# deeplearning-wisc/MCM

Hardware: AMD Instinct MI355X
Metric: images/sec MCM-scored (CLIP-B/16, 1000 prompts) (higher is better)
Workload: dtype fp16; 1 GPU; MCM scoring, CLIP-ViT-B/16 (12L vision tower, random-init weights), K=1000 prompts pre-encoded, batch 512/GPU, fp32 NCHW pixels resident in HBM -> [B] scores; batch_per_gpu=512, prompts=1000, parallelism=image-sharded x1

## Files before the change

include/mcm.h:

```cpp
#ifndef MCM_H_
#define MCM_H_

#include <stdint.h>

#ifdef __cplusplus
extern "C" {
#endif

#define MCM_ABI_VERSION 5

#define MCM_OK 0
#define MCM_EINVAL (-1)
#define MCM_ENOMEM (-2)
#define MCM_EHIP (-3)
#define MCM_ENOWEIGHT (-4)
#define MCM_ENAME (-5)
#define MCM_ESHAPE (-6)
#define MCM_ERANGE (-7)

#define MCM_PREC_BF16 0
#define MCM_PREC_F32 1
#define MCM_PREC_F16 2

#define MCM_DT_F32 0
#define MCM_DT_F16 1
#define MCM_DT_BF16 2

#define MCM_WEIGHTS_AUTO 0
#define MCM_WEIGHTS_SINGLE 1
#define MCM_WEIGHTS_SPLIT 2

#define MCM_ACT_QUICK_GELU 0
#define MCM_ACT_GELU 1

#define MCM_SCORE_MCM 0
#define MCM_SCORE_MAX_LOGIT 1
#define MCM_SCORE_ENERGY 2
#define MCM_SCORE_ENTROPY 3
#define MCM_SCORE_VAR 4

typedef struct mcm_handle mcm_handle;

typedef struct mcm_config {
  int32_t abi_version;
  int32_t device;
  int32_t precision;
  int32_t image_size;
  int32_t patch_size;
  int32_t v_width;
  int32_t v_heads;
  int32_t v_layers;
  int32_t v_mlp;
  int32_t vocab_size;
  int32_t max_positions;
  int32_t t_width;
  int32_t t_heads;
  int32_t t_layers;
  int32_t t_mlp;
  int32_t proj_dim;
  float ln_eps;
  int32_t max_batch;
  int32_t max_prompt_tokens;
  int32_t weight_operands;
  int32_t x2_max_batch;
  int32_t v_hidden_act;
  int32_t t_hidden_act;
} mcm_config;

int mcm_abi_version(void);

int mcm_create(const mcm_config* cfg, mcm_handle** out);
void mcm_destroy(mcm_handle* h);
const char* mcm_last_error(const mcm_handle* h);

int mcm_set_weight(mcm_handle* h, const char* hf_name, const void* host_ptr, int32_t dtype,
                   const int64_t* shape, int32_t ndim);
int mcm_finalize_weights(mcm_handle* h);
int mcm_weights_operand_exact(mcm_handle* h, uint64_t* inexact_host, int32_t* split_host);

int mcm_encode_text(mcm_handle* h, const int32_t* ids_host, int32_t K, int32_t S,
                    float* out_dev, void* stream);

int mcm_encode_image(mcm_handle* h, const float* pixels_dev, int32_t B, float* out_dev,
                     void* stream);

#define MCM_PIXELS_F32_NCHW 0
#define MCM_PIXELS_U8_NHWC 1
int mcm_encode_image_ex(mcm_handle* h, const void* pixels_dev, int32_t pixel_format, int32_t B,
                        int32_t normalize, float* out_dev, void* stream);
int mcm_encode_text_ex(mcm_handle* h, const int32_t* ids_host, int32_t K, int32_t S, int32_t normalize,
                       float* out_dev, void* stream);

int mcm_score_features(mcm_handle* h, const float* img_feat_dev, int32_t B,
                       const float* text_feat_dev, int32_t K, float T, int32_t kind,
                       float* scores_dev, void* stream);

int mcm_score(mcm_handle* h, const float* pixels_dev, int32_t B, const float* text_feat_dev,
              int32_t K, float T, int32_t kind, float* scores_dev, void* stream);

#define MCM_TOPK_MAX 8
int mcm_score_features_topk(mcm_handle* h, const float* img_feat_dev, int32_t B, const float* text_feat_dev,
                            int32_t K, float T, int32_t kind, int32_t topk, float* scores_dev,
                            int32_t* idx_dev , float* prob_dev , void* stream);
int mcm_score_topk(mcm_handle* h, const void* pixels_dev, int32_t pixel_format, int32_t x2, int32_t B,
                   const float* text_feat_dev, int32_t K, float T, int32_t kind, int32_t topk, float* scores_dev,
                   int32_t* idx_dev, float* prob_dev, void* stream);

int mcm_encode_image_u8(mcm_handle* h, const uint8_t* pixels_dev, int32_t B, float* out_dev,
                        void* stream);
int mcm_score_u8(mcm_handle* h, const uint8_t* pixels_dev, int32_t B, const float* text_feat_dev,
                 int32_t K, float T, int32_t kind, float* scores_dev, void* stream);

int mcm_x2_max_batch(const mcm_handle* h);
int mcm_encode_image_x2(mcm_handle* h, const void* pixels_dev, int32_t pixel_format, int32_t B, int32_t normalize,
                        float* out_dev, void* stream);
int mcm_score_x2(mcm_handle* h, const void* pixels_dev, int32_t pixel_format, int32_t B, const float* text_feat_dev,
                 int32_t K, float T, int32_t kind, float* scores_dev, void* stream);

int mcm_resize_crop_u8(mcm_handle* h, const uint8_t* const* src_dev_ptrs, const int32_t* heights,
                       const int32_t* widths, int32_t B, uint8_t* dst_dev, void* stream);

int mcm_pack_u8(const uint8_t* const* srcs, const int64_t* sizes, const int64_t* offsets, int32_t n, uint8_t* dst,
                int64_t dst_bytes, int32_t threads);

typedef struct mcm_jpeg_image {
  int32_t status;
  int32_t width, height, ncomp;
  int32_t hs[3], vs[3];
  int32_t wb[3], hb[3];
  int64_t coef_off[3];
} mcm_jpeg_image;
int mcm_jpeg_entropy_decode(const char* const* paths, int32_t n, void* dst, int64_t dst_bytes, mcm_jpeg_image* meta,
                            uint16_t* quant, int32_t threads, int64_t* bytes_used);

int mcm_jpeg_reconstruct(mcm_handle* h, const void* coef_dev, const mcm_jpeg_image* meta, const uint16_t* quant, int32_t n,
                         uint8_t* rgb_dev, const int64_t* rgb_offsets, void* stream);

int mcm_reduce_bank(mcm_handle* h, const float* feats_dev, int32_t K, int32_t T, float* bank_dev,
                    void* stream);

int mcm_measures(mcm_handle* h, const float* pos_dev, int64_t n_pos, const float* neg_dev,
                 int64_t n_neg, int32_t negate, double recall_level, double* out_host, void* stream);

int mcm_score_histogram(mcm_handle* h, const float* scores_dev, int64_t n, const float* edges_dev,
                        int32_t n_bins, int64_t* counts_dev, void* stream);

int mcm_encode_image_raw(mcm_handle* h, const float* pixels_dev, int32_t B, float* out_dev, void* stream);
int mcm_maha_prepare(mcm_handle* h, const float* means_dev, const float* prec_dev, int32_t C,
                     double* w_dev, double* k_dev, void* stream);
int mcm_maha_score_features(mcm_handle* h, const float* feats_dev, int32_t B, const float* prec_dev,
                            const double* w_dev, const double* k_dev, int32_t C, float* scores_dev,
                            void* stream);
int mcm_maha_fit_accumulate(mcm_handle* h, const float* feats_dev , int32_t B,
                            const float* shift_dev , double* gram_dev, double* sum_dev,
                            void* stream);

#define MCM_KNN_MAX_K 1024
#define MCM_KNN_MAX_SPLITS 32
int mcm_knn_workspace_bytes(const mcm_handle* h, int32_t B, int64_t N, int32_t k, int32_t splits, int64_t* bytes_out);
int mcm_knn_score_features(mcm_handle* h, const float* feats_dev , int32_t B,
                           const float* bank_dev , int64_t N, int32_t k, int32_t splits,
                           void* work_dev, int64_t work_bytes, float* scores_dev ,
                           float* topv_dev , void* stream);

#define MCM_NEG_MAX_GROUPS 1024
int mcm_neglabel_workspace_bytes(const mcm_handle* h, int32_t B, int32_t K, int32_t G, int32_t gs, int32_t splits,
                                 int64_t* bytes_out);
int mcm_neglabel_score_features(mcm_handle* h, const float* feats_dev , int32_t B,
                                const float* bank_dev , int32_t K, int32_t G, int32_t gs,
                                float T, int32_t splits, void* work_dev, int64_t work_bytes,
                                float* scores_dev , float* group_dev , void* stream);

int mcm_local_workspace_bytes(const mcm_handle* h, int32_t B, int32_t R, int32_t K, int64_t* bytes_out);
int mcm_local_score_features(mcm_handle* h, const float* local_dev , int32_t B, int32_t R,
                             const float* text_dev , int32_t K, float T, void* work_dev,
                             int64_t work_bytes, float* local_scores_dev ,
                             float* patch_dev , void* stream);
int mcm_encode_image_local(mcm_handle* h, const void* pixels_dev, int32_t pixel_format, int32_t B,
                           float* global_dev ,
                           float* local_dev , void* stream);
int mcm_score_glmcm(mcm_handle* h, const void* pixels_dev, int32_t pixel_format, int32_t B, const float* text_dev ,
                    int32_t K, float T, float lambda, float* scores_dev ,
                    float* global_scores_dev , float* local_scores_dev ,
                    float* patch_dev , void* stream);

typedef struct mcm_tokenizer mcm_tokenizer;
int mcm_tokenizer_create(const char* vocab_json_path, const char* merges_txt_path, mcm_tokenizer** out);
void mcm_tokenizer_destroy(mcm_tokenizer* t);
const char* mcm_tokenizer_last_error(const mcm_tokenizer* t);
int32_t mcm_tokenizer_vocab_size(const mcm_tokenizer* t);
int mcm_tokenizer_encode(mcm_tokenizer* t, const char* const* texts, int32_t n, int32_t capacity,
                         int32_t* ids_out, int32_t* mask_out, int32_t* seq_len_out);

#define MCM_KC_PATCHIFY 0
#define MCM_KC_GEMM 1
#define MCM_KC_LAYERNORM 2
#define MCM_KC_ATTENTION 3
#define MCM_KC_POOL_PROJECT 4
#define MCM_KC_SCORE 5
#define MCM_KC_EMBED 6
#define MCM_KC_GEMM_QKV 7
#define MCM_KC_GEMM_OUTPROJ 8
#define MCM_KC_GEMM_FC1 9
#define MCM_KC_GEMM_FC2 10
#define MCM_KC_COUNT 11
int mcm_profile_enable(mcm_handle* h, int32_t on);
int mcm_profile_read(mcm_handle* h, double* ms_out, int64_t* launches_out, double* flops_out);


int mcm_op_linear(mcm_handle* h, int32_t prec, const void* x_dev, const void* w_dev,
                  const float* bias_dev, void* y_dev, float* resid_dev, int32_t M, int32_t N,
                  int32_t K, int32_t epi, void* stream);
#define MCM_LINEAR_SPLIT_W 1
#define MCM_LINEAR_SPLIT_X 2
#define MCM_LINEAR_SPLIT_OUT 4
#define MCM_LINEAR_ACT_GELU 8
int mcm_op_linear_ex(mcm_handle* h, int32_t prec, const void* x_dev, const void* w_dev,
                     const float* bias_dev, void* y_dev, float* resid_dev, int32_t M, int32_t N,
                     int32_t K, int32_t epi, int32_t flags, void* stream);
int mcm_op_split_weight(mcm_handle* h, int32_t prec, const float* w_dev, int32_t N, int32_t K,
                        void* out_dev, void* stream);
int mcm_op_layernorm(mcm_handle* h, int32_t prec, const float* x_dev, const float* gamma_dev,
                     const float* beta_dev, void* y_dev, int32_t M, int32_t D, float eps,
                     int32_t out_f32, void* stream);
int mcm_op_layernorm_split(mcm_handle* h, const float* x_dev, const float* gamma_dev, const float* beta_dev,
                           void* y_dev, int32_t M, int32_t D, float eps, void* stream);
int mcm_op_attention_split(mcm_handle* h, const void* qkv_dev, void* out_dev, int32_t nseq, int32_t seq_len,
                           int32_t heads, void* stream);
int mcm_op_attention(mcm_handle* h, int32_t prec, const void* qkv_dev, void* out_dev,
                     int32_t nseq, int32_t seq_len, int32_t heads, int32_t causal,
                     void* stream);

int mcm_saturation_check(mcm_handle* h, int32_t on);
int mcm_saturation_count(mcm_handle* h, int32_t reset, uint64_t* count_host, void* stream);

int mcm_kernel_faults(const mcm_handle* h);

#ifdef MCM_HARNESS
int mcm_debug_gemm_variant(int32_t variant);
int mcm_debug_op_act(mcm_handle* h, int32_t act, const float* x_dev, float* y_dev, int64_t n, void* stream);
int mcm_debug_attention_variant(int32_t variant);
int mcm_debug_attn_spin_budget(int64_t polls);
int mcm_debug_clear_faults(mcm_handle* h);
int mcm_debug_op_attention(mcm_handle* h, int32_t prec, const void* qkv_dev, void* out_dev, int32_t nseq, int32_t seq_len,
                           int32_t heads, int32_t causal, int32_t qrows, int32_t reverse, void* stream);
int mcm_debug_op_attention_split(mcm_handle* h, const void* qkv_dev, void* out_dev, int32_t nseq, int32_t seq_len,
                                 int32_t heads, int32_t qrows, int32_t reverse, void* stream);
int mcm_debug_op_attention_hd(mcm_handle* h, int32_t prec, const void* qkv_dev, void* out_dev, int32_t nseq, int32_t seq_len,
                              int32_t heads, int32_t head_dim, int32_t causal, int32_t qrows, int32_t reverse, void* stream);
int mcm_debug_op_attention_split_hd(mcm_handle* h, const void* qkv_dev, void* out_dev, int32_t nseq, int32_t seq_len,
                                    int32_t heads, int32_t head_dim, int32_t qrows, int32_t reverse, void* stream);
int mcm_debug_vision_front(mcm_handle* h, const void* pixels_dev, int32_t pixel_format, int32_t x2, int32_t B, int32_t stage,
                           int32_t poison, float* resid_out_dev, void* ln_out_dev, void* stream);
int mcm_debug_op_pool_project(mcm_handle* h, const float* x_dev, int64_t x_rows, const int32_t* row_idx_host, int32_t row_stride,
                              int32_t n, int32_t D, const float* gamma_dev, const float* beta_dev, float eps,
                              const float* proj_dev, int32_t P, float* out_dev, int32_t normalize, void* stream);
int mcm_debug_op_text_embed(mcm_handle* h, const int32_t* ids_host, int32_t vocab, const float* tok_dev, const float* pos_dev,
                            float* x_dev, int32_t K, int32_t S, int32_t D, void* stream);
int mcm_debug_gemm_dbg(int32_t bits);
int mcm_debug_qkv_chunks(int32_t n);
int mcm_debug_nsplit(int32_t n);
int mcm_debug_gemm_group_n(int32_t gn);
int mcm_debug_patch_fold(int32_t on);
int mcm_debug_resize_fused_only(int32_t on);
int mcm_debug_persistent_grid(int32_t n);
int mcm_debug_ln_fold(int32_t on);
int mcm_debug_qkv_head_major(int32_t on);
int mcm_debug_ln_tail(int32_t on);
int mcm_debug_ln_cluster(int32_t on);
int mcm_debug_ln_cluster_spin(int32_t polls);
int mcm_debug_ln_row(int32_t on);
int mcm_debug_ln_cluster_deferred(mcm_handle* h, uint64_t* count_host);
int mcm_debug_ln_tail_timeouts(mcm_handle* h, uint64_t* count_host);
#endif

#ifdef __cplusplus
}
#endif
#endif
```

mcm_amd/csrc/common.hpp:

```cpp
#pragma once
#include <hip/hip_runtime.h>
#include <stdint.h>

#include "../../include/mcm.h"

struct PerDeviceFlag {
  bool done[64] = {};
  static int dev() { int d = 0; return hipGetDevice(&d) == hipSuccess && d >= 0 && d < 64 ? d : -1; }
  bool get() const { const int d = dev(); return d >= 0 && done[d]; }
  void set() { const int d = dev(); if (d >= 0) done[d] = true; }
};

inline int device_cu_count() {
  static int cus[64] = {};
  int dev = 0;
  if (hipGetDevice(&dev) != hipSuccess || dev < 0) return 0;
  if (dev < 64 && cus[dev] > 0) return cus[dev];
  int n = 0;
  if (hipDeviceGetAttribute(&n, hipDeviceAttributeMultiprocessorCount, dev) != hipSuccess) return 0;
  if (dev < 64) cus[dev] = n;
  return n;
}

typedef __attribute__((ext_vector_type(8))) __bf16 bf16x8_t;
typedef __attribute__((ext_vector_type(8))) _Float16 f16x8_t;
typedef __attribute__((ext_vector_type(4))) float f32x4_t;
typedef __attribute__((address_space(1))) const void* gptr_t;
typedef __attribute__((address_space(3))) void* lptr_t;

__device__ __forceinline__ uint16_t f2bf(float f) {
  uint32_t u = __builtin_bit_cast(uint32_t, f);
  if ((u & 0x7fffffffu) > 0x7f800000u) return (uint16_t)((u >> 16) | 0x40u);
  u += 0x7fffu + ((u >> 16) & 1u);
  return (uint16_t)(u >> 16);
}
__device__ __forceinline__ float bf2f(uint16_t h) {
  return __builtin_bit_cast(float, (uint32_t)h << 16);
}
__device__ __forceinline__ uint32_t pack_bf2(float lo, float hi) {
  typedef __bf16 bf2_t __attribute__((ext_vector_type(2)));
  typedef float f2_t __attribute__((ext_vector_type(2)));
  const f2_t v = {lo, hi};
  return __builtin_bit_cast(uint32_t, __builtin_convertvector(v, bf2_t));
}

__device__ __forceinline__ void glds16(const void* gsrc, uint32_t lds_base) {
  uint32_t keep;
  asm volatile(
      "s_mov_b32 %0, m0\n\ts_mov_b32 m0, %2\n\ts_nop 0\n\tglobal_load_lds_dwordx4 %1, off\n\t"
      "s_mov_b32 m0, %0"
      : "=&s"(keep)
      : "v"(gsrc), "s"(lds_base)
      : "memory");
}
__device__ __forceinline__ uint32_t lds_addr(const void* p) {
  return (uint32_t)(uintptr_t)(__attribute__((address_space(3))) const void*)p;
}

__device__ __forceinline__ uint32_t pack_h2(float lo, float hi) {
  typedef _Float16 h2_t __attribute__((ext_vector_type(2)));
  typedef float f2_t __attribute__((ext_vector_type(2)));
  const f2_t v = {lo, hi};
  return __builtin_bit_cast(uint32_t, __builtin_convertvector(v, h2_t));
}
template <int PREC>
__device__ __forceinline__ void enter_precision_mode() {
  if constexpr (PREC == MCM_PREC_F16) asm volatile("s_setreg_imm32_b32 hwreg(HW_REG_MODE, 23, 1), 1");
}

template <int PREC>
__device__ __forceinline__ void sat_track(float& amax, float a, float b) {
#ifndef MCM_NO_SAT_TRACK
  if constexpr (PREC == MCM_PREC_F16) amax = fmaxf(fmaxf(__builtin_fabsf(a), __builtin_fabsf(b)), amax);
#endif
}
template <int PREC>
__device__ __forceinline__ void sat_report(float amax, unsigned int* counter) {
  if constexpr (PREC == MCM_PREC_F16) {
    if (counter != nullptr && __builtin_amdgcn_ballot_w64(amax >= 65520.0f) != 0) {
      if ((threadIdx.x & 63) == 0) {
        const unsigned int one = 1u;
        asm volatile("global_atomic_add %0, %1, off" ::"v"(counter), "v"(one) : "memory");
      }
    }
  }
}

template <int PREC>
__device__ __forceinline__ uint32_t pack2(float lo, float hi) {
  if constexpr (PREC == MCM_PREC_F16) return pack_h2(lo, hi);
  else return pack_bf2(lo, hi);
}
template <int PREC>
__device__ __forceinline__ f32x4_t mfma16(uint4 a, uint4 b, f32x4_t c) {
  if constexpr (PREC == MCM_PREC_F16)
    return __builtin_amdgcn_mfma_f32_16x16x32_f16(__builtin_bit_cast(f16x8_t, a),
                                                  __builtin_bit_cast(f16x8_t, b), c, 0, 0, 0);
  else
    return __builtin_amdgcn_mfma_f32_16x16x32_bf16(__builtin_bit_cast(bf16x8_t, a),
                                                   __builtin_bit_cast(bf16x8_t, b), c, 0, 0, 0);
}

__device__ __forceinline__ float quick_gelu(float x) { return x / (1.0f + __expf(-1.702f * x)); }
__device__ __forceinline__ float quick_gelu_fast(float x) {
  return x * __builtin_amdgcn_rcpf(1.0f + __builtin_amdgcn_exp2f(-1.702f * 1.4426950408889634f * x));
}
__device__ __forceinline__ float gelu_erf(float x) {
#pragma clang fp contract(off)
  const float ax = __builtin_fabsf(x);
  const float t = __builtin_amdgcn_rcpf(__builtin_fmaf(ax, 0.2757716477f, 1.0f));
  const float e = __builtin_amdgcn_exp2f((ax * ax) * -0.7213475204f);
  float h = -0.11376846582f;
  h = __builtin_fmaf(h, t, 0.44333177805f);
  h = __builtin_fmaf(h, t, -0.31769949198f);
  h = __builtin_fmaf(h, t, 0.32477918267f);
  h = __builtin_fmaf(h, t, 0.045694414526f);
  h = __builtin_fmaf(h, t, 0.11766257882f);
  h = (h * t) * e;
  return x * (x >= 0.0f ? 1.0f - h : h);
}

__device__ __forceinline__ float wave_sum(float v) {
#pragma unroll
  for (int o = 32; o > 0; o >>= 1) v += __shfl_xor(v, o, 64);
  return v;
}
__device__ __forceinline__ float wave_max(float v) {
#pragma unroll
  for (int o = 32; o > 0; o >>= 1) v = fmaxf(v, __shfl_xor(v, o, 64));
  return v;
}

template <int CTRL>
__device__ __forceinline__ float dpp_move(float x) {
  return __builtin_bit_cast(float, __builtin_amdgcn_update_dpp(0, __builtin_bit_cast(int, x), CTRL, 0xf, 0xf, true));
}
__device__ __forceinline__ float row16_sum(float v) {
#pragma clang fp contract(off)
  v = v + dpp_move<0xB1>(v);
  v = v + dpp_move<0x4E>(v);
  v = v + dpp_move<0x141>(v);
  v = v + dpp_move<0x140>(v);
  return v;
}
__device__ __forceinline__ void slot_moments(const f32x4_t& v, float& sum, float& m2) {
#pragma clang fp contract(off)
  sum = row16_sum((v[0] + v[1]) + (v[2] + v[3]));
  const float mean = sum * (1.0f / 64.0f);
  const float d0 = v[0] - mean, d1 = v[1] - mean, d2 = v[2] - mean, d3 = v[3] - mean;
  m2 = row16_sum((d0 * d0 + d1 * d1) + (d2 * d2 + d3 * d3));
}
__device__ __forceinline__ f32x4_t fold_scale(const f32x4_t& v, const f32x4_t& gamma) {
#pragma clang fp contract(off)
  return v * gamma;
}
__device__ __forceinline__ float fold_apply(float acc, float rstd, float mrstd, float c, float b) {
  return __builtin_fmaf(acc, rstd, __builtin_fmaf(-mrstd, c, b));
}

template <int PREC>
__device__ __forceinline__ void split2(float a, float b, uint32_t& hi, uint32_t& lo) {
  hi = pack2<PREC>(a, b);
  float ha, hb;
  if constexpr (PREC == MCM_PREC_F16) {
    typedef _Float16 h2_t __attribute__((ext_vector_type(2)));
    const h2_t h = __builtin_bit_cast(h2_t, hi);
    ha = (float)h[0];
    hb = (float)h[1];
  } else {
    ha = __builtin_bit_cast(float, hi << 16);
    hb = __builtin_bit_cast(float, hi & 0xffff0000u);
  }
  lo = pack2<PREC>(a - ha, b - hb);
}
__host__ __device__ constexpr size_t split_col(int n) { return (size_t)(n >> 6) * 128 + (n & 63); }

__host__ __device__ constexpr int prec_esize(int prec) { return prec == MCM_PREC_F32 ? 4 : 2; }


enum GemmEpi : int {
  EPI_STORE = 0,
  EPI_GELU = 1,
  EPI_RESID = 2,
  EPI_PATCH = 3,
  EPI_STORE_X2 = 4,
  EPI_GELU_X2 = 5,
  EPI_GELU_ERF = 6,
  EPI_GELU_ERF_X2 = 7,
};
__host__ __device__ constexpr bool epi_x2(int e) { return e == EPI_STORE_X2 || e == EPI_GELU_X2 || e == EPI_GELU_ERF_X2; }
__host__ __device__ constexpr bool epi_erf(int e) { return e == EPI_GELU_ERF || e == EPI_GELU_ERF_X2; }
__host__ __device__ constexpr bool epi_gelu(int e) { return e == EPI_GELU || e == EPI_GELU_X2 || epi_erf(e); }
__host__ __device__ constexpr bool epi_plain16(int e) { return e == EPI_STORE || e == EPI_GELU || e == EPI_GELU_ERF; }
__host__ __device__ constexpr bool epi_store16(int e) { return epi_plain16(e) || epi_x2(e); }

struct GemmArgs {
  const void* x;
  const void* w;
  const float* bias;
  void* out;
  float* resid;
  const float* pos;
  int M, N, K;
  int ldx;
  int ldo;
  int np;
  const float* px;
  int img, patch;
  int gn;
  int rev;
  int dbg;
  unsigned int* sat;
  int ksplit;
  int xsplit;
  void* fold_z;
  const float* fold_g;
  float2* fold_part;
  const float2* fold_rs;
  const float* fold_c;
  int hm;
  const float* ln_g;
  const float* ln_b;
  void* ln_y;
  float ln_eps;
  unsigned int* ln_state;
  int ln_rs, ln_cap8;
  int lnc;
  int lnc_spin;
  int wblk;
};
#ifdef MCM_HARNESS
#define MCM_HM(hm) (hm)
#else
#define MCM_HM(hm) 0
#endif
__device__ __forceinline__ size_t out16_off(const GemmArgs& a, int m, int n) {
  return MCM_HM(a.hm) ? ((size_t)(n >> 6) * a.hm + m) * 64 + (n & 63) : (size_t)m * a.ldo + n;
}
hipError_t launch_gemm(int prec, int epi, const GemmArgs& a, hipStream_t s);
int gemm_fold_kind(int epi, int M, int N);
bool gemm_patch_takes_pixels(int prec, int M, int N, int kpad, int patch, int image);
bool gemm_ln_tail_ok(int prec, int M, int N);
int gemm_persistent_grid();
#ifdef MCM_HARNESS
void gemm_set_persistent_grid(int n);
#endif
hipError_t launch_fold_prep(int prec, const void* w, const float* gamma, const float* beta, const float* bias,
                            float* c, float* bfold, int N, int K, hipStream_t s);
hipError_t launch_fold_rows(int prec, const float* x, const float* gamma, void* z, float2* part, int M, int D,
                            hipStream_t s, unsigned int* sat = nullptr);
hipError_t launch_fold_stats(const float2* part, int slots, int M, int D, float eps, float2* rs, hipStream_t s);
#ifdef MCM_HARNESS
hipError_t launch_lnc_cleanup(int prec, const float* x, const float* g, const float* b, void* y, const float2* part, int M, int D,
                              float eps, unsigned int* ln_state, int ln_rs, int ln_cap8, hipStream_t s, unsigned int* sat);
hipError_t launch_gemm_row64_ln(int prec, const GemmArgs& a, hipStream_t s, int stages);
hipError_t launch_row64_block_w(const void* w, void* blocked, int N, int K, hipStream_t s);
void gemm_set_group_n(int gn);
void gemm_set_dbg(int d);
void gemm_set_variant(int v);
void attention_set_variant(int v);
void attention_set_spin_budget(unsigned int polls);
#endif

hipError_t launch_layernorm(int prec, const float* x, const float* g, const float* b, void* y,
                            int M, int D, float eps, bool out_f32, hipStream_t s,
                            size_t x_stride = 0, size_t y_stride = 0, bool reverse = false,
                            unsigned int* sat = nullptr, bool split = false);

hipError_t launch_layernorm_pre(int prec, float* x, const float* g0, const float* b0, const float* g1,
                                const float* b1, void* y, int M, int D, float eps, hipStream_t s,
                                bool reverse = false, unsigned int* sat = nullptr, const float* cls = nullptr,
                                const float* pos0 = nullptr, int ntok = 0, bool split = false);

hipError_t launch_attention(int prec, const void* qkv, void* out, int nseq, int L, int heads, int head_dim,
                            bool causal, int qrows, hipStream_t s, bool reverse = false, int hm = 0, bool split = false,
                            unsigned int* fault = nullptr);

hipError_t launch_patchify(int prec, const float* pixels, void* patches, int B, int image,
                           int patch, int kpad, hipStream_t s, bool split = false);
hipError_t launch_patchify_u8(int prec, const uint8_t* pixels, void* patches, int B, int image,
                              int patch, int kpad, const float* mean, const float* stdv,
                              hipStream_t s, bool split = false);
hipError_t launch_bank_reduce(const float* feats, int K, int T, int P, float* bank, hipStream_t s);
hipError_t launch_text_embed(const int32_t* ids, const float* tok, const float* pos, float* x,
                             int K, int S, int D, hipStream_t s);
hipError_t launch_cvt_weight(int prec, const float* src, void* dst, int rows, int cols,
                             int cols_pad, hipStream_t s);
hipError_t launch_cvt_weight_split(int prec, const float* src, void* dst, int rows, int cols,
                                   int cols_pad, hipStream_t s);
hipError_t launch_count_inexact(int prec, const float* src, size_t n, unsigned long long* count, hipStream_t s);

hipError_t launch_pool_project(const float* x, const int32_t* row_idx, int row_stride, int n,
                               int D, const float* g, const float* b, float eps,
                               const float* proj, int P, float* out, hipStream_t s,
                               bool normalize = true);
hipError_t launch_maha_prepare(const float* means, const float* prec, int C, int P, double* w, double* c,
                               hipStream_t s);
hipError_t launch_maha_score(const float* feats, int B, const float* prec, const double* w, const double* c,
                             int C, int P, float* scores, hipStream_t s);
hipError_t launch_maha_fit(const float* feats, int B, int P, const float* shift, double* gram, double* sum,
                           hipStream_t s);

hipError_t launch_knn(const float* feats, int B, const float* bank, int64_t N, int P, int k, int S, float* work,
                      float* scores, float* topv, hipStream_t s);

int64_t neglabel_work_bytes(int B, int G, int S);
hipError_t launch_neglabel(const float* feats, int B, const float* bank, int K, int G, int gs, int P, float T, int S,
                           void* work, float* scores, float* group, hipStream_t s);

int64_t local_work_bytes(int B, int R);
hipError_t launch_local_score(const float* rows, int B, int R, const float* bank, int K, int P, float T, void* work,
                              float* scores, float* patch, hipStream_t s);
hipError_t launch_local_compact(const float* y, float* out, int B, int ntok, int P, hipStream_t s);
hipError_t launch_local_combine(const float* g, const float* l, float lambda, float* out, int B, hipStream_t s);

hipError_t launch_score(const float* img, int B, const float* text, int K, int P, float T,
                        int kind, float* scores, hipStream_t s);
bool score_shape_ok(int K, int P);
hipError_t launch_score_topk(const float* img, int B, const float* text, int K, int P, float T, int kind,
                             int topk, float* scores, int* idx, float* prob, hipStream_t s);

size_t measures_workspace_bytes(long n);
hipError_t launch_measures(const float* pos, long n_pos, const float* neg, long n_neg, int negate,
                           double level, void* workspace, double** out_dev, hipStream_t s);

hipError_t launch_histogram(const float* x, long n, const float* edges, int nb, unsigned long long* counts,
                            hipStream_t s);

struct PrepImage {
  const uint8_t* src;
  int32_t H, W;
  int32_t nh, nw;
  int32_t top, left;
};
struct JpegImageDev {
  int32_t width, height, ncomp;
  int32_t H, V;
  int32_t wb[3], hb[3];
  int64_t coef_off[3];
  int64_t plane_off[3];
  int64_t rgb_off;
};
hipError_t launch_jpeg_reconstruct(const JpegImageDev* meta_dev, const uint16_t* quant_dev, const void* coef_dev,
                                   uint8_t* planes_dev, uint8_t* rgb_dev, int n, int max_blocks, int max_pixels, hipStream_t s);
int prep_max_taps();
size_t prep_coef_bytes(int max_batch, int S);
hipError_t launch_resize_crop(const PrepImage* meta_dev, int32_t* coef_dev, int B, int S, uint8_t* dst, hipStream_t s,
                              bool fused_only = false);
```

mcm_amd/csrc/embed.hip:

```cpp
#include "common.hpp"

namespace {

template <int OUT, bool X2 = false>
__global__ __launch_bounds__(256) void patchify_kernel(const float* __restrict__ px, void* out,
                                                       int B, int S, int P, int kpad) {
  const int g = S / P, np = g * g, kreal = 3 * P * P;
  const size_t total = (size_t)B * np * kpad;
  for (size_t i = (size_t)blockIdx.x * 256 + threadIdx.x; i < total;
       i += (size_t)gridDim.x * 256) {
    const int k = (int)(i % kpad);
    const size_t m = i / kpad;
    float v = 0.f;
    if (k < kreal) {
      const int b = (int)(m / np), p = (int)(m % np);
      const int gy = p / g, gx = p % g;
      const int c = k / (P * P), rem = k % (P * P), py = rem / P, pxx = rem % P;
      v = px[(((size_t)b * 3 + c) * S + gy * P + py) * S + gx * P + pxx];
    }
    if constexpr (X2) {
      const _Float16 hi = (_Float16)v;
      _Float16* dst = (_Float16*)out + m * 2 * kpad + split_col(k);
      dst[0] = hi;
      dst[64] = (_Float16)(v - (float)hi);
    } else
    if constexpr (OUT == MCM_PREC_BF16) ((uint16_t*)out)[i] = f2bf(v);
    else if constexpr (OUT == MCM_PREC_F16) ((_Float16*)out)[i] = (_Float16)v;
    else ((float*)out)[i] = v;
  }
}

template <int OUT>
__global__ __launch_bounds__(256) void patchify8_kernel(const float* __restrict__ px, void* out,
                                                        int B, int S, int P, int kpad) {
  const int g = S / P, np = g * g, k8 = kpad / 8, p8 = P / 8;
  const size_t total = (size_t)B * np * k8;
  for (size_t i = (size_t)blockIdx.x * 256 + threadIdx.x; i < total;
       i += (size_t)gridDim.x * 256) {
    const int kq = (int)(i % k8);
    const size_t m = i / k8;
    const int b = (int)(m / np), p = (int)(m % np);
    const int gy = p / g, gx = p - gy * g;
    const int rowi = kq / p8, xq = kq - rowi * p8;
    const int c = rowi / P, py = rowi - c * P;
    const float* src = px + (((size_t)b * 3 + c) * S + gy * P + py) * S + gx * P + xq * 8;
    const float4 a = *(const float4*)src, d = *(const float4*)(src + 4);
    if constexpr (OUT != MCM_PREC_F32) {
      *(uint4*)((uint16_t*)out + i * 8) =
          make_uint4(pack2<OUT>(a.x, a.y), pack2<OUT>(a.z, a.w), pack2<OUT>(d.x, d.y), pack2<OUT>(d.z, d.w));
    } else {
      *(float4*)((float*)out + i * 8) = a;
      *(float4*)((float*)out + i * 8 + 4) = d;
    }
  }
}

template <int OUT, bool X2 = false>
__global__ __launch_bounds__(256) void patchify_u8_kernel(const uint8_t* __restrict__ px, void* out,
                                                          int B, int S, int P, int kpad, float m0,
                                                          float m1, float m2, float s0, float s1,
                                                          float s2) {
  const int g = S / P, np = g * g;
  const size_t total = (size_t)B * S * S;
  const float mean[3] = {m0, m1, m2}, stdv[3] = {s0, s1, s2};
  for (size_t i = (size_t)blockIdx.x * 256 + threadIdx.x; i < total; i += (size_t)gridDim.x * 256) {
    const int x = (int)(i % S), y = (int)((i / S) % S), b = (int)(i / ((size_t)S * S));
    const int gy = y / P, py = y - gy * P, gx = x / P, pxx = x - gx * P;
    const size_t row = ((size_t)b * np + gy * g + gx) * kpad;
#pragma unroll
    for (int c = 0; c < 3; ++c) {
      const float v = ((float)px[i * 3 + c] / 255.0f - mean[c]) / stdv[c];
      const size_t o = row + (size_t)(c * P + py) * P + pxx;
      if constexpr (X2) {
        const _Float16 hi = (_Float16)v;
        _Float16* dst = (_Float16*)out + 2 * row + split_col((c * P + py) * P + pxx);
        dst[0] = hi;
        dst[64] = (_Float16)(v - (float)hi);
      } else
      if constexpr (OUT == MCM_PREC_BF16) ((uint16_t*)out)[o] = f2bf(v);
      else if constexpr (OUT == MCM_PREC_F16) ((_Float16*)out)[o] = (_Float16)v;
      else ((float*)out)[o] = v;
    }
  }
}

__global__ __launch_bounds__(256) void bank_reduce_kernel(const float* __restrict__ feats, int K,
                                                          int T, int P, float* __restrict__ bank) {
  const int k = blockIdx.x * 4 + (threadIdx.x >> 6), lane = threadIdx.x & 63;
  if (k >= K) return;
  float sq = 0.f;
  for (int d = lane; d < P; d += 64) {
    float a = 0.f;
    for (int t = 0; t < T; ++t) a += feats[((size_t)k * T + t) * P + d];
    a /= (float)T;
    bank[(size_t)k * P + d] = a;
    sq += a * a;
  }
  const float rn = 1.0f / sqrtf(wave_sum(sq));
  for (int d = lane; d < P; d += 64) bank[(size_t)k * P + d] *= rn;
}

__global__ __launch_bounds__(256) void text_embed_kernel(const int32_t* __restrict__ ids,
                                                         const float* __restrict__ tok,
                                                         const float* __restrict__ pos, float* x,
                                                         int K, int S, int D) {
  const int row = blockIdx.x;
  const int s = row % S;
  const int id = ids[row];
  for (int d = threadIdx.x * 4; d < D; d += 1024) {
    const float4 a = *(const float4*)(tok + (size_t)id * D + d);
    const float4 p = *(const float4*)(pos + (size_t)s * D + d);
    *(float4*)(x + (size_t)row * D + d) = make_float4(a.x + p.x, a.y + p.y, a.z + p.z, a.w + p.w);
  }
}

template <int OUT>
__global__ __launch_bounds__(256) void cvt_weight_kernel(const float* __restrict__ src, void* dst,
                                                         int rows, int cols, int cols_pad) {
  const size_t total = (size_t)rows * cols_pad;
  for (size_t i = (size_t)blockIdx.x * 256 + threadIdx.x; i < total;
       i += (size_t)gridDim.x * 256) {
    const int c = (int)(i % cols_pad);
    const size_t r = i / cols_pad;
    const float v = c < cols ? src[r * cols + c] : 0.f;
    if constexpr (OUT == MCM_PREC_BF16) ((uint16_t*)dst)[i] = f2bf(v);
    else if constexpr (OUT == MCM_PREC_F16) ((_Float16*)dst)[i] = (_Float16)v;
    else ((float*)dst)[i] = v;
  }
}

template <int OUT>
__global__ __launch_bounds__(256) void cvt_weight_split_kernel(const float* __restrict__ src, void* dst,
                                                               int rows, int cols, int cols_pad) {
  const size_t total = (size_t)rows * cols_pad;
  for (size_t i = (size_t)blockIdx.x * 256 + threadIdx.x; i < total;
       i += (size_t)gridDim.x * 256) {
    const int c = (int)(i % cols_pad);
    const size_t r = i / cols_pad;
    const float v = c < cols ? src[r * cols + c] : 0.f;
    const size_t o = r * 2 * cols_pad + (size_t)(c >> 6) * 128 + (c & 63);
    if constexpr (OUT == MCM_PREC_BF16) {
      const uint16_t hi = f2bf(v);
      ((uint16_t*)dst)[o] = hi;
      ((uint16_t*)dst)[o + 64] = f2bf(v - bf2f(hi));
    } else {
      const float vc = fminf(fmaxf(v, -65504.0f), 65504.0f);
      const _Float16 hi = (_Float16)vc;
      ((_Float16*)dst)[o] = hi;
      ((_Float16*)dst)[o + 64] = (_Float16)fminf(fmaxf(v - (float)hi, -65504.0f), 65504.0f);
    }
  }
}

template <int OUT>
__global__ __launch_bounds__(256) void count_inexact_kernel(const float* __restrict__ src, size_t n,
                                                            unsigned long long* count) {
  unsigned int mine = 0;
  for (size_t i = (size_t)blockIdx.x * 256 + threadIdx.x; i < n; i += (size_t)gridDim.x * 256) {
    const float v = src[i];
    float back;
    if constexpr (OUT == MCM_PREC_BF16) back = bf2f(f2bf(v));
    else back = (float)(_Float16)v;
    mine += (back != v && v == v) ? 1u : 0u;
  }
#pragma unroll
  for (int o = 32; o > 0; o >>= 1) mine += __shfl_xor(mine, o, 64);
  if ((threadIdx.x & 63) == 0 && mine) atomicAdd(count, (unsigned long long)mine);
}

constexpr int NWP = 16;
constexpr int POOL_MAXD = 1280;
template <bool WIDE>
__global__ __launch_bounds__(NWP * 64) void pool_project_kernel(
    const float* __restrict__ x, const int32_t* __restrict__ row_idx, int row_stride, int D,
    const float* __restrict__ g, const float* __restrict__ b, float eps,
    const float* __restrict__ proj, int P, float* __restrict__ out, int normalize) {
  __shared__ float y[WIDE ? POOL_MAXD : 1024];
  __shared__ float o[1024];
  __shared__ float red[2 * NWP];
  const int n = blockIdx.x, tid = threadIdx.x, lane = tid & 63, wave = tid >> 6;
  const size_t row = row_idx ? (size_t)row_idx[n] : (size_t)n * row_stride;
  const float* xr = x + row * D;
  const int t2 = tid + NWP * 64;
  const float xv = tid < D ? xr[tid] : 0.f;
  float xw = 0.f;
  float s;
  if constexpr (WIDE) {
    if (t2 < D) xw = xr[t2];
    s = wave_sum(xv + xw);
  } else {
    s = wave_sum(xv);
  }
  if (lane == 0) red[wave] = s;
  __syncthreads();
  float tot = 0.f;
#pragma unroll
  for (int i = 0; i < NWP; ++i) tot += red[i];
  const float mean = tot / (float)D;
  const float c = tid < D ? xv - mean : 0.f;
  float cw = 0.f;
  float q;
  if constexpr (WIDE) {
    if (t2 < D) cw = xw - mean;
    q = wave_sum(fmaf(cw, cw, c * c));
  } else {
    q = wave_sum(c * c);
  }
  if (lane == 0) red[NWP + wave] = q;
  __syncthreads();
  tot = 0.f;
#pragma unroll
  for (int i = 0; i < NWP; ++i) tot += red[NWP + i];
  const float rstd = 1.0f / sqrtf(tot / (float)D + eps);
  if (tid < D) y[tid] = c * rstd * g[tid] + b[tid];
  if constexpr (WIDE) {
    if (t2 < D) y[t2] = cw * rstd * g[t2] + b[t2];
  }
  __syncthreads();
  float sq = 0.f;
  for (int p = wave; p < P; p += NWP) {
    const float* w = proj + (size_t)p * D;
    float a = 0.f;
    for (int d = lane * 4; d < D; d += 256) {
      const float4 wv = *(const float4*)(w + d);
      a = fmaf(wv.x, y[d], a);
      a = fmaf(wv.y, y[d + 1], a);
      a = fmaf(wv.z, y[d + 2], a);
      a = fmaf(wv.w, y[d + 3], a);
    }
    a = wave_sum(a);
    if (lane == 0) {
      o[p] = a;
      sq += a * a;
    }
  }
  __syncthreads();
  if (lane == 0) red[wave] = sq;
  __syncthreads();
  tot = 0.f;
#pragma unroll
  for (int i = 0; i < NWP; ++i) tot += red[i];
  const float rn = normalize ? 1.0f / sqrtf(tot) : 1.0f;
  for (int p = tid; p < P; p += NWP * 64) out[(size_t)n * P + p] = o[p] * rn;
}

inline int grid_for(size_t total) {
  size_t g = (total + 255) / 256;
  return (int)(g > 4096 ? 4096 : (g ? g : 1));
}

}

hipError_t launch_patchify(int prec, const float* pixels, void* patches, int B, int image,
                           int patch, int kpad, hipStream_t s, bool split) {
  const int g = image / patch;
  if (split) {
    if (prec != MCM_PREC_F16 || kpad % 64) return hipErrorInvalidValue;
    const size_t n = (size_t)B * g * g * kpad;
    hipLaunchKernelGGL((patchify_kernel<MCM_PREC_F16, true>), dim3(grid_for(n)), dim3(256), 0, s, pixels, patches, B, image, patch, kpad);
    return hipGetLastError();
  }
  const bool vec = patch % 8 == 0 && kpad == 3 * patch * patch && image % 4 == 0;
  const size_t total = (size_t)B * g * g * (vec ? kpad / 8 : kpad);
  const dim3 grid(grid_for(total)), block(256);
#define MCM_LAUNCH_BY_PREC(KERNEL, ...)                                                         \
  do {                                                                                           \
    if (prec == MCM_PREC_BF16) hipLaunchKernelGGL(KERNEL<MCM_PREC_BF16>, grid, block, 0, s, __VA_ARGS__); \
    else if (prec == MCM_PREC_F16) hipLaunchKernelGGL(KERNEL<MCM_PREC_F16>, grid, block, 0, s, __VA_ARGS__); \
    else hipLaunchKernelGGL(KERNEL<MCM_PREC_F32>, grid, block, 0, s, __VA_ARGS__);               \
  } while (0)
  if (vec) MCM_LAUNCH_BY_PREC(patchify8_kernel, pixels, patches, B, image, patch, kpad);
  else MCM_LAUNCH_BY_PREC(patchify_kernel, pixels, patches, B, image, patch, kpad);
  return hipGetLastError();
}

hipError_t launch_patchify_u8(int prec, const uint8_t* pixels, void* patches, int B, int image,
                              int patch, int kpad, const float* mean, const float* stdv,
                              hipStream_t s, bool split) {
  const size_t total = (size_t)B * image * image;
  const dim3 grid(grid_for(total)), block(256);
  if (split && (prec != MCM_PREC_F16 || kpad % 64)) return hipErrorInvalidValue;
  if (kpad != 3 * patch * patch) {
    hipError_t e = hipMemsetAsync(patches, 0, (size_t)B * (image / patch) * (image / patch) * kpad *
                                                   prec_esize(prec) * (split ? 2 : 1), s);
    if (e != hipSuccess) return e;
  }
  if (split) {
    hipLaunchKernelGGL((patchify_u8_kernel<MCM_PREC_F16, true>), grid, block, 0, s, pixels, patches, B, image, patch, kpad,
                       mean[0], mean[1], mean[2], stdv[0], stdv[1], stdv[2]);
    return hipGetLastError();
  }
  MCM_LAUNCH_BY_PREC(patchify_u8_kernel, pixels, patches, B, image, patch, kpad, mean[0], mean[1],
                     mean[2], stdv[0], stdv[1], stdv[2]);
  return hipGetLastError();
}

hipError_t launch_bank_reduce(const float* feats, int K, int T, int P, float* bank, hipStream_t s) {
  if (K <= 0 || T <= 0 || P <= 0) return hipErrorInvalidValue;
  hipLaunchKernelGGL(bank_reduce_kernel, dim3((K + 3) / 4), dim3(256), 0, s, feats, K, T, P, bank);
  return hipGetLastError();
}

hipError_t launch_text_embed(const int32_t* ids, const float* tok, const float* pos, float* x,
                             int K, int S, int D, hipStream_t s) {
  if (D % 4) return hipErrorInvalidValue;
  hipLaunchKernelGGL(text_embed_kernel, dim3(K * S), dim3(256), 0, s, ids, tok, pos, x, K, S, D);
  return hipGetLastError();
}

hipError_t launch_cvt_weight(int prec, const float* src, void* dst, int rows, int cols,
                             int cols_pad, hipStream_t s) {
  const size_t total = (size_t)rows * cols_pad;
  const dim3 grid(grid_for(total)), block(256);
  MCM_LAUNCH_BY_PREC(cvt_weight_kernel, src, dst, rows, cols, cols_pad);
  return hipGetLastError();
}

hipError_t launch_cvt_weight_split(int prec, const float* src, void* dst, int rows, int cols,
                                   int cols_pad, hipStream_t s) {
  if (prec == MCM_PREC_F32 || cols_pad % 64) return hipErrorInvalidValue;
  const size_t total = (size_t)rows * cols_pad;
  const dim3 grid(grid_for(total)), block(256);
  if (prec == MCM_PREC_BF16) hipLaunchKernelGGL(cvt_weight_split_kernel<MCM_PREC_BF16>, grid, block, 0, s, src, dst, rows, cols, cols_pad);
  else hipLaunchKernelGGL(cvt_weight_split_kernel<MCM_PREC_F16>, grid, block, 0, s, src, dst, rows, cols, cols_pad);
  return hipGetLastError();
}

hipError_t launch_count_inexact(int prec, const float* src, size_t n, unsigned long long* count, hipStream_t s) {
  if (prec == MCM_PREC_F32 || n == 0) return hipSuccess;
  const dim3 grid(grid_for(n)), block(256);
  if (prec == MCM_PREC_BF16) hipLaunchKernelGGL(count_inexact_kernel<MCM_PREC_BF16>, grid, block, 0, s, src, n, count);
  else hipLaunchKernelGGL(count_inexact_kernel<MCM_PREC_F16>, grid, block, 0, s, src, n, count);
  return hipGetLastError();
}

hipError_t launch_pool_project(const float* x, const int32_t* row_idx, int row_stride, int n,
                               int D, const float* g, const float* b, float eps,
                               const float* proj, int P, float* out, hipStream_t s, bool normalize) {
  if (n <= 0 || D > POOL_MAXD || D % 4 || P > 1024) return hipErrorInvalidValue;
  if (D > 1024 && D % 64) return hipErrorInvalidValue;
  if (D > 1024)
    hipLaunchKernelGGL(pool_project_kernel<true>, dim3(n), dim3(NWP * 64), 0, s, x, row_idx, row_stride, D, g, b,
                       eps, proj, P, out, normalize ? 1 : 0);
  else
    hipLaunchKernelGGL(pool_project_kernel<false>, dim3(n), dim3(NWP * 64), 0, s, x, row_idx, row_stride, D, g, b,
                       eps, proj, P, out, normalize ? 1 : 0);
  return hipGetLastError();
}
```

mcm_amd/csrc/gemm.hip:

```cpp
#include <type_traits>

#include "common.hpp"
#include "ln_row.hpp"

namespace {

constexpr int ROWB = 128;

__device__ __forceinline__ void kstep_off(const GemmArgs& a, int kt, size_t& kox, size_t& kow) {
  const int t = kt >> (a.ksplit + a.xsplit);
  kox = (size_t)((t << a.xsplit) | (kt & a.xsplit)) * ROWB;
  kow = (size_t)((t << a.ksplit) | ((kt >> a.xsplit) & a.ksplit)) * ROWB;
}
__device__ __forceinline__ int ksteps(const GemmArgs& a, int es) { return ((a.K * es) / ROWB) << a.xsplit; }

#if defined(MCM_HARNESS) || defined(MCM_LN_FOLD) || defined(MCM_LN_TAIL)
#define MCM_ARMS 1
#endif

__device__ __forceinline__ int frag_off(int fr, int g, int kk) {
  return (fr >> 1) * 256 + ((((fr & 1) << 3) | (((kk * 4 + g) ^ (fr >> 1)) & 7)) << 4);
}

template <int PREC, int MF>
// ... 179 lines not shown
                     pack2<PREC>(v[1][0], v[1][1]), pack2<PREC>(v[1][2], v[1][3]));
      *(uint4*)(w + (((g * 2 + 1) ^ sw) << 4)) =
          make_uint4(pack2<PREC>(v[2][0], v[2][1]), pack2<PREC>(v[2][2], v[2][3]),
                     pack2<PREC>(v[3][0], v[3][1]), pack2<PREC>(v[3][2], v[3][3]));
    };
    auto read_unit = [&](int u, uint4 (&r)[2]) {
#pragma unroll
      for (int t = 0; t < 2; ++t) {
        const int row = t * 8 + rrow;
        r[t] = *(const uint4*)(scratch + (u & 1) * 2048 + row * 128 + ((c8 ^ (row & 7)) << 4));
      }
    };
    const int ldo_e = MCM_HM(a.hm) ? 64 : a.ldo;
    const int lane_off = rrow * ldo_e + c8 * 8;
    const char* sp = (const char*)a.out + out16_off(a, mw, nw) * 2;
    const size_t sp_step = (size_t)ldo_e * 16;
    auto store_unit = [&](int u, const uint4 (&r)[2]) {
#pragma unroll
      for (int t = 0; t < 2; ++t) {
        if constexpr (INTERIOR) {
          store16_stream_s(sp, (uint32_t)lane_off * 2u, r[t]);
          sp += sp_step;
        } else {
          const int m = mw + u * 16 + t * 8 + rrow;
          if (m < a.M && n < a.N) store16_stream((uint16_t*)a.out + out16_off(a, m, n), r[t]);
        }
      }
    };
    write_unit(0);
#pragma unroll
    for (int u = 1; u < MF; ++u) {
      uint4 r[2];
      read_unit(u - 1, r);
      write_unit(u);
      store_unit(u - 1, r);
    }
    {
      uint4 r[2];
      read_unit(MF - 1, r);
      store_unit(MF - 1, r);
    }
  } else {
    const int rrow = lane >> 4, c16 = lane & 15;
    const int n = nw + c16 * 4;
    const bool ncol = n < a.N;
    f32x4_t rnext[4];
    auto row_ptr = [&](int c, int t, bool& ok) -> float* {
      const int m = mw + c * 16 + t * 4 + rrow;
      ok = ncol && m < a.M;
      if constexpr (EPI == EPI_PATCH) {
        const int mm = min(m, a.M - 1), b = mm / a.np, p = mm - b * a.np;
        return (float*)a.out + (size_t)(b * (a.np + 1) + 1 + p) * a.ldo + n;
      } else if constexpr (EPI == EPI_RESID) {
        return a.resid + (size_t)m * a.ldo + n;
      } else {
        return (float*)a.out + (size_t)m * a.ldo + n;
      }
    };
    auto prefetch = [&](int c) {
#pragma unroll
      for (int t = 0; t < 4; ++t) {
        bool ok;
        const float* ptr;
        if constexpr (EPI == EPI_PATCH) {
          const int m = min(mw + c * 16 + t * 4 + rrow, a.M - 1);
          const int p = m - (m / a.np) * a.np;
          ok = ncol;
          ptr = a.pos + (size_t)(1 + p) * a.N + n;
        } else {
          ptr = row_ptr(c, t, ok);
        }
        rnext[t] = ok ? *(const f32x4_t*)ptr : (f32x4_t){0.f, 0.f, 0.f, 0.f};
      }
    };
    constexpr bool ADD = (EPI == EPI_RESID || EPI == EPI_PATCH);
    if constexpr (ADD) prefetch(0);
#pragma unroll
    for (int c = 0; c < MF; ++c) {
      f32x4_t r[4];
      if constexpr (ADD) {
#pragma unroll
        for (int t = 0; t < 4; ++t) r[t] = rnext[t];
        if (c + 1 < MF) prefetch(c + 1);
      }
      const int sw = fr;
#pragma unroll
      for (int fj = 0; fj < 4; ++fj) {
        f32x4_t v = acc[fj][c] + bv[fj];
        if constexpr (epi_gelu(EPI)) {
#pragma unroll
          for (int t = 0; t < 4; ++t) v[t] = epi_erf(EPI) ? gelu_erf(v[t]) : quick_gelu(v[t]);
        }
        *(f32x4_t*)(scratch + fr * 256 + (((g * 4 + fj) ^ sw) << 4)) = v;
      }
#pragma unroll
      for (int t = 0; t < 4; ++t) {
        const int row = t * 4 + rrow;
        f32x4_t v = *(const f32x4_t*)(scratch + row * 256 + ((c16 ^ row) << 4));
        if constexpr (ADD) v += r[t];
        bool ok;
        float* dst = row_ptr(c, t, ok);
        if (ok) *(f32x4_t*)dst = v;
      }
    }
  }
}

__device__ __forceinline__ void load_bias(const GemmArgs& a, int n, f32x4_t (&bv)[4]) {
  const int nc = min(n, a.N - 16);
#pragma unroll
  for (int fj = 0; fj < 4; ++fj) {
    bv[fj] = a.bias ? *(const f32x4_t*)(a.bias + nc + fj * 4) : (f32x4_t){0.f, 0.f, 0.f, 0.f};
  }
#pragma unroll
  for (int fj = 0; fj < 4; ++fj) asm volatile("" : "+v"(bv[fj]));
}
__device__ __forceinline__ void load_bias_async(const GemmArgs& a, int n, f32x4_t (&bv)[4]) {
  const float* p = a.bias + min(n, a.N - 16);
#pragma unroll
  for (int fj = 0; fj < 4; ++fj)
    asm volatile("global_load_dwordx4 %0, %1, off" : "=v"(bv[fj]) : "v"(p + fj * 4) : "memory");
}

template <int MF>
__device__ __forceinline__ void zero_acc(f32x4_t (&acc)[4][MF]) {
#pragma unroll
  for (int i = 0; i < 4; ++i)
#pragma unroll
    for (int j = 0; j < MF; ++j) acc[i][j] = (f32x4_t){0.f, 0.f, 0.f, 0.f};
}

namespace tile {
constexpr int BM = 128, BN = 128;
constexpr int TILE_BYTES = BM * ROWB;
constexpr int STAGE_BYTES = 2 * TILE_BYTES;
constexpr int LDS_BYTES = 2 * STAGE_BYTES;
}

template <int PREC, int EPI>
__global__ __launch_bounds__(256, 2) void gemm_tile_kernel(const GemmArgs a) {
  using namespace tile;
  enter_precision_mode<PREC>();
  extern __shared__ __attribute__((aligned(16))) char smem[];
  constexpr int ES = prec_esize(PREC);
  const int lane = threadIdx.x & 63;
  const int wave = __builtin_amdgcn_readfirstlane(threadIdx.x >> 6);

  const int nbn = (a.N + BN - 1) / BN;
  const int nbm = (a.M + BM - 1) / BM;
  const int nwg = nbn * nbm;
  int lid;
  {
    const int bid = blockIdx.x, q = nwg >> 3, r = nwg & 7, xcd = bid & 7;
    lid = (xcd < r ? xcd * (q + 1) : r * (q + 1) + (xcd - r) * q) + (bid >> 3);
  }
  const int m0 = (lid / nbn) * BM;
  const int n0 = (lid % nbn) * BN;

  const char* gx[4];
  const char* gw[4];
#pragma unroll
  for (int i = 0; i < 4; ++i) {
    const int blk = i * 4 + wave;
    const int p = blk * 4 + (lane >> 4);
    const int s = lane & 15;
    const int row = 2 * p + (s >> 3);
    const int chunk = (s & 7) ^ (p & 7);
    const int mr = min(m0 + row, a.M - 1);
    const int nr = min(n0 + (row & 64) + perm_n(row & 63), a.N - 1);
    gx[i] = (const char*)a.x + ((size_t)mr * a.ldx) * ES + chunk * 16;
    gw[i] = (const char*)a.w + ((size_t)nr * a.K) * ES + chunk * 16;
  }
  const uint32_t lds0 = lds_addr(smem);
  auto stage = [&](int st, int kt) {
    const uint32_t base = lds0 + st * STAGE_BYTES;
    size_t kox, kow;
    kstep_off(a, kt, kox, kow);
#pragma unroll
    for (int i = 0; i < 4; ++i) {
      const int blk = i * 4 + wave;
      glds16(gx[i] + kox, __builtin_amdgcn_readfirstlane(base + blk * 1024));
      glds16(gw[i] + kow, __builtin_amdgcn_readfirstlane(base + TILE_BYTES + blk * 1024));
    }
  };

  const int wr = wave >> 1, wc = wave & 1;
  const int fr = lane & 15, g = lane >> 4;
  const int foff[2] = {frag_off(fr, g, 0), frag_off(fr, g, 1)};
  const int xbase = wr * 64 * ROWB;
  const int wbase = TILE_BYTES + wc * 64 * ROWB;

  f32x4_t acc[4][4];
  zero_acc(acc);
  const int nk = ksteps(a, ES);
  stage(0, 0);
  for (int kt = 0; kt < nk; ++kt) {
    asm volatile("s_waitcnt vmcnt(0)" ::: "memory");
    __syncthreads();
    if (kt + 1 < nk) stage((kt + 1) & 1, kt + 1);
    const char* sb = smem + (kt & 1) * STAGE_BYTES;
    wave_kstep<PREC, 4>(sb + xbase, sb + wbase, foff, acc);
  }
  f32x4_t bv[4];
  load_bias(a, n0 + wc * 64 + g * 16, bv);
  float amax = 0.f;
  wave_epilogue<PREC, EPI, 4>(a, acc, bv, m0 + wr * 64, n0 + wc * 64, fr, g, amax);
  sat_report<PREC>(amax, a.sat);
}

namespace tile64 {
constexpr int BM = 64, BN = 128;
constexpr int X_BYTES = BM * ROWB, W_BYTES = BN * ROWB;
constexpr int STAGE_BYTES = X_BYTES + W_BYTES;
constexpr int LDS_BYTES = 2 * STAGE_BYTES;
}

template <int PREC, int EPI>
__global__ __launch_bounds__(256, 2) void gemm_tile64_kernel(const GemmArgs a) {
  using namespace tile64;
  enter_precision_mode<PREC>();
  extern __shared__ __attribute__((aligned(16))) char smem[];
  constexpr int ES = prec_esize(PREC);
  const int lane = threadIdx.x & 63;
  const int wave = __builtin_amdgcn_readfirstlane(threadIdx.x >> 6);
  const int nbn = (a.N + BN - 1) / BN;
  const int nbm = (a.M + BM - 1) / BM;
  const int nwg = nbn * nbm;
  int lid;
  {
    const int bid = blockIdx.x, q = nwg >> 3, r = nwg & 7, xcd = bid & 7;
    lid = (xcd < r ? xcd * (q + 1) : r * (q + 1) + (xcd - r) * q) + (bid >> 3);
  }
  const int m0 = (lid / nbn) * BM;
  const int n0 = (lid % nbn) * BN;
  const char* gx[2];
  const char* gw[4];
#pragma unroll
  for (int i = 0; i < 4; ++i) {
    const int blk = i * 4 + wave;
    const int p = blk * 4 + (lane >> 4);
    const int sl = lane & 15;
    const int row = 2 * p + (sl >> 3);
    const int chunk = (sl & 7) ^ (p & 7);
    if (i < 2) gx[i] = (const char*)a.x + ((size_t)min(m0 + row, a.M - 1) * a.ldx) * ES + chunk * 16;
    const int nr = min(n0 + (row & 64) + perm_n(row & 63), a.N - 1);
    gw[i] = (const char*)a.w + ((size_t)nr * a.K) * ES + chunk * 16;
  }
  const uint32_t lds0 = lds_addr(smem);
  auto stage = [&](int st, int kt) {
    const uint32_t base = lds0 + st * STAGE_BYTES;
    size_t kox, kow;
    kstep_off(a, kt, kox, kow);
#pragma unroll
    for (int i = 0; i < 4; ++i) {
      const int blk = i * 4 + wave;
      if (i < 2) glds16(gx[i] + kox, __builtin_amdgcn_readfirstlane(base + blk * 1024));
      glds16(gw[i] + kow, __builtin_amdgcn_readfirstlane(base + X_BYTES + blk * 1024));
    }
  };
  const int wr = wave >> 1, wc = wave & 1;
  const int fr = lane & 15, g = lane >> 4;
  const int foff[2] = {frag_off(fr, g, 0), frag_off(fr, g, 1)};
  const int xbase = wr * 32 * ROWB;
  const int wbase = X_BYTES + wc * 64 * ROWB;
  f32x4_t acc[4][2];
  zero_acc(acc);
  const int nk = ksteps(a, ES);
  stage(0, 0);
  for (int kt = 0; kt < nk; ++kt) {
    asm volatile("s_waitcnt vmcnt(0)" ::: "memory");
    __syncthreads();
    if (kt + 1 < nk) stage((kt + 1) & 1, kt + 1);
    const char* sb = smem + (kt & 1) * STAGE_BYTES;
#pragma unroll
    for (int kk = 0; kk < 2; ++kk) {
      uint4 wf[4], xf[2];
#pragma unroll
      for (int f = 0; f < 4; ++f) wf[f] = *(const uint4*)(sb + wbase + f * 2048 + foff[kk]);
#pragma unroll
      for (int f = 0; f < 2; ++f) xf[f] = *(const uint4*)(sb + xbase + f * 2048 + foff[kk]);
#pragma unroll
      for (int fj = 0; fj < 4; ++fj)
#pragma unroll
        for (int fi = 0; fi < 2; ++fi) {
          if constexpr (PREC != MCM_PREC_F32) {
            acc[fj][fi] = mfma16<PREC>(wf[fj], xf[fi], acc[fj][fi]);
          } else {
            const f32x4_t wv = __builtin_bit_cast(f32x4_t, wf[fj]);
            const f32x4_t xv = __builtin_bit_cast(f32x4_t, xf[fi]);
#pragma unroll
            for (int t = 0; t < 4; ++t)
              acc[fj][fi] = __builtin_amdgcn_mfma_f32_16x16x4f32(wv[t], xv[t], acc[fj][fi], 0, 0, 0);
          }
        }
    }
  }
  f32x4_t bv[4];
  load_bias(a, n0 + wc * 64 + g * 16, bv);
  float amax = 0.f;
  wave_epilogue<PREC, EPI, 2>(a, acc, bv, m0 + wr * 32, n0 + wc * 64, fr, g, amax);
  sat_report<PREC>(amax, a.sat);
}

__device__ __forceinline__ void tile_of(int q, int nmt_x, int nbn, int gn, int& mtl, int& nt) {
  int start = 0, g0 = 0;
  for (;;) {
    const int gw = min(gn, nbn - g0), cnt = nmt_x * gw;
    if (q < start + cnt || g0 + gw >= nbn) {
      const int r = q - start;
      mtl = r / gw;
      nt = g0 + (r - mtl * gw);
      return;
    }
    start += cnt;
    g0 += gw;
  }
}

template <int N>
__device__ __forceinline__ void wait_vmcnt() {
  asm volatile("s_waitcnt vmcnt(%0)" ::"n"(N) : "memory");
}

namespace p256 {
constexpr int BM = 256, BN = 256;
constexpr int A_BYTES = BM * ROWB;
constexpr int W_BYTES = BN * ROWB;
constexpr int STAGE_BYTES = A_BYTES + W_BYTES;
constexpr int LDS_BYTES = 2 * STAGE_BYTES + 8 * 4096;
}

__device__ __forceinline__ void gload16(f32x4_t& dst, const void* sbase, uint32_t voff) {
  asm volatile("global_load_dwordx4 %0, %1, %2" : "=v"(dst) : "v"(voff), "s"(sbase) : "memory");
}
__device__ __forceinline__ void gstore16(const void* sbase, uint32_t voff, const f32x4_t& v) {
  asm volatile("global_store_dwordx4 %0, %1, %2\n\ts_nop 1" ::"v"(voff), "v"(v), "s"(sbase) : "memory");
}

template <int PREC, int EPI, bool COUNT_STORES, bool PXF = false>
__global__ __launch_bounds__(512, 2) void gemm_p256_kernel(const GemmArgs a) {
  static_assert(!PXF || EPI == EPI_PATCH, "pixel gathering: the patch embedding only");
  using namespace p256;
  enter_precision_mode<PREC>();
  extern __shared__ __attribute__((aligned(16))) char smem[];
  constexpr int ES = prec_esize(PREC);
  constexpr int STORES_PER_EPI = (PREC != MCM_PREC_F32 && epi_plain16(EPI)) ? 16 : 32;
  const int lane = threadIdx.x & 63;
  const int wave = __builtin_amdgcn_readfirstlane(threadIdx.x >> 6);

  const int nbn = (a.N + BN - 1) / BN;
  const int nbm = (a.M + BM - 1) / BM;
  const int G8 = gridDim.x >> 3;
  const int xcd = blockIdx.x & 7, jx = blockIdx.x >> 3;
  const int nmt_x = (nbm - xcd + 7) >> 3;
  const int ntl_x = nmt_x * nbn;
  const int ntl = jx < ntl_x ? (ntl_x - jx + G8 - 1) / G8 : 0;
  if (ntl == 0) return;
  const int nk = ksteps(a, ES);
  const int total = ntl * nk;

  const int r0 = wave * 8 + (lane >> 4) * 2 + ((lane & 15) >> 3);
  const int chunk = (lane & 7) ^ (((wave & 1) << 2) | (lane >> 4));
  const char* gx[4];
  const char* gw[4];
  int ji = 0, kti = 0;
  constexpr int EC = 16 / ES, KS = ROWB / ES;
  uint32_t pxoff[4] = {0u, 0u, 0u, 0u};
  f32x4_t xr[4][2];
  int xst = 0;
  const bool plain = a.gn >= nbn;
  const int dmt = G8 / nbn, dnt = G8 - dmt * nbn;
  struct Cursor { int mtl, nt; };
  auto cursor_init = [&](Cursor& c) { tile_of(jx, nmt_x, nbn, a.gn, c.mtl, c.nt); };
  auto cursor_next = [&](Cursor& c, int i) {
    if (plain) {
      c.mtl += dmt;
      c.nt += dnt;
      if (c.nt >= nbn) { c.nt -= nbn; ++c.mtl; }
    } else {
      tile_of(jx + i * G8, nmt_x, nbn, a.gn, c.mtl, c.nt);
    }
  };
  const size_t sx = (size_t)a.ldx * ES, sw = (size_t)a.K * ES;
  const char* xlane = (const char*)a.x + (size_t)r0 * sx + chunk * 16;
  const char* wlane = (const char*)a.w + (size_t)perm_n(r0) * sw + chunk * 16;
  auto mt_of = [&](int mtl) { return a.rev ? nmt_x - 1 - mtl : mtl; };
  Cursor ci;
  auto set_issue_tile = [&]() {
    const int m0 = (mt_of(ci.mtl) * 8 + xcd) * BM, n0 = ci.nt * BN;
    if (m0 + BM <= a.M && n0 + BN <= a.N) {
      const char* xb = xlane + (size_t)m0 * sx;
      const char* wb = wlane + (size_t)n0 * sw;
#pragma unroll
      for (int p = 0; p < 4; ++p) {
        if constexpr (!PXF) gx[p] = xb + (size_t)(p * 64) * sx;
        gw[p] = wb + (size_t)(p * 64) * sw;
      }
    } else {
#pragma unroll
      for (int p = 0; p < 4; ++p) {
        if constexpr (!PXF) gx[p] = (const char*)a.x + (size_t)min(m0 + p * 64 + r0, a.M - 1) * sx + chunk * 16;
        gw[p] = (const char*)a.w + (size_t)min(n0 + p * 64 + perm_n(r0), a.N - 1) * sw + chunk * 16;
      }
    }
    if constexpr (PXF) {
      {
        const int P = a.patch, S = a.img, gsz = S / P;
        const int e = chunk * EC, dpy = e / P, pxl = e - dpy * P;
#pragma unroll
        for (int p = 0; p < 4; ++p) {
          const int m = min(m0 + p * 64 + r0, a.M - 1);
          const int b = m / a.np, pp = m - b * a.np, gy = pp / gsz, gxx = pp - gy * gsz;
          pxoff[p] = (uint32_t)((((size_t)b * 3 * S + (size_t)gy * P + dpy) * S + (size_t)gxx * P + pxl) * 4);
        }
      }
    }
  };
  const uint32_t lds0 = lds_addr(smem);
  auto issue_px = [&](int st) {
    const int r = (kti >> a.ksplit) * (KS / a.patch), c = r / a.patch, py0 = r - c * a.patch;
    const char* kb = (const char*)a.px + ((size_t)c * a.img + py0) * a.img * 4;
#pragma unroll
    for (int p = 0; p < 4; ++p) {
      gload16(xr[p][0], kb, pxoff[p]);
      if constexpr (ES == 2) gload16(xr[p][1], kb, pxoff[p] + 16u);
    }
    xst = st;
  };
  auto issue = [&](int st) {
    const uint32_t base = lds0 + st * STAGE_BYTES;
    size_t ko, kox;
    kstep_off(a, kti, kox, ko);
    if constexpr (PXF) {
#pragma unroll
      for (int p = 0; p < 4; ++p)
        glds16(gw[p] + ko, __builtin_amdgcn_readfirstlane(base + A_BYTES + (p * 8 + wave) * 1024));
    } else {
#pragma unroll
      for (int p = 0; p < 4; ++p) {
        glds16(gx[p] + kox, __builtin_amdgcn_readfirstlane(base + (p * 8 + wave) * 1024));
        glds16(gw[p] + ko, __builtin_amdgcn_readfirstlane(base + A_BYTES + (p * 8 + wave) * 1024));
      }
    }
    if (++kti == nk) {
      kti = 0;
      if (++ji < ntl) {
        cursor_next(ci, ji);
        set_issue_tile();
      }
    }
  };

  const int wr = wave >> 2, wc = wave & 3;
  const bool late = wave >= 4;
  const int fr = lane & 15, g = lane >> 4;
  const int foff[2] = {frag_off(fr, g, 0), frag_off(fr, g, 1)};
  const int xbase = wr * 128 * ROWB;
  const int wbase = A_BYTES + wc * 64 * ROWB;

  f32x4_t acc[4][8];
  zero_acc<8>(acc);
  float amax = 0.f;
  f32x4_t bv[4];
#pragma unroll
  for (int fj = 0; fj < 4; ++fj) bv[fj] = (f32x4_t){0.f, 0.f, 0.f, 0.f};

  auto commit_x = [&]() {
    wait_vmcnt<0>();
#pragma unroll
    for (int p = 0; p < 4; ++p) {
      asm volatile("" : "+v"(xr[p][0]));
      if constexpr (ES == 2) asm volatile("" : "+v"(xr[p][1]));
    }
#pragma unroll
    for (int p = 0; p < 4; ++p) {
      char* dst = smem + xst * STAGE_BYTES + (p * 8 + wave) * 1024 + lane * 16;
      if constexpr (PREC != MCM_PREC_F32) {
        *(uint4*)dst = make_uint4(pack2<PREC>(xr[p][0][0], xr[p][0][1]), pack2<PREC>(xr[p][0][2], xr[p][0][3]),
                                  pack2<PREC>(xr[p][1][0], xr[p][1][1]), pack2<PREC>(xr[p][1][2], xr[p][1][3]));
      } else {
        *(f32x4_t*)dst = xr[p][0];
      }
    }
    asm volatile("s_waitcnt lgkmcnt(0)" ::: "memory");
  };

  cursor_init(ci);
  set_issue_tile();
  if constexpr (PXF) issue_px(0);
  issue(0);
  if constexpr (PXF) commit_x();
  int issued = 1;
  int jc = 0, ktc = 0;
  Cursor cc;
  cursor_init(cc);
  int cm0 = (mt_of(cc.mtl) * 8 + xcd) * BM, cn0 = cc.nt * BN;
  bool stores_pending = false;
  if (late) __builtin_amdgcn_s_setprio(1);
  for (int s = 0; s < total; ++s) {
    if (COUNT_STORES && stores_pending) wait_vmcnt<STORES_PER_EPI>();
    else wait_vmcnt<0>();
    stores_pending = false;
    __builtin_amdgcn_s_barrier();
    asm volatile("" ::: "memory");
    if constexpr (!PXF) {
      if (ktc == 0 && a.bias) load_bias_async(a, cn0 + wc * 64 + g * 16, bv);
    }
    const bool refill = issued < total;
    if constexpr (PXF) {
      if (refill) issue_px(issued & 1);
    }
    if (refill && !late) issue(issued & 1);
    const char* sb = smem + (s & 1) * STAGE_BYTES;
    wave_khalf<PREC, 8>(sb + xbase, sb + wbase, foff[0], acc);
    if (refill && late) issue(issued & 1);
    if (refill) ++issued;
    wave_khalf<PREC, 8>(sb + xbase, sb + wbase, foff[1], acc);
    if (++ktc == nk) {
      if constexpr (!PXF) {
        if (nk < 2) wait_vmcnt<0>();
#pragma unroll
        for (int fj = 0; fj < 4; ++fj) asm volatile("" : "+v"(bv[fj]));
      }
      wave_epilogue_lds<PREC, EPI, 8>(a, acc, bv, cm0 + wr * 128, cn0 + wc * 64, lane,
                                      smem + 2 * STAGE_BYTES + wave * 4096, amax);
      zero_acc<8>(acc);
      stores_pending = (cm0 + BM <= a.M && cn0 + BN <= a.N);
      ktc = 0;
      if (++jc < ntl) {
        cursor_next(cc, jc);
        cm0 = (mt_of(cc.mtl) * 8 + xcd) * BM;
        cn0 = cc.nt * BN;
      }
    }
    if constexpr (PXF) {
      if (refill) commit_x();
    }
  }
  sat_report<PREC>(amax, a.sat);
}

template <int N>
__device__ __forceinline__ void wait_vmcnt_pin(f32x4_t (&b)[4]) {
  asm volatile("s_waitcnt vmcnt(%4)" : "+v"(b[0]), "+v"(b[1]), "+v"(b[2]), "+v"(b[3]) : "n"(N) : "memory");
}
template <int EPI, int MF>
__device__ __forceinline__ void wave_epilogue_f32_interior(const GemmArgs& a, const f32x4_t (&acc)[4][MF],
                                                           const f32x4_t (&bv)[4], int mw, int nw, int lane,
                                                           char* scratch) {
  static_assert(EPI != EPI_PATCH, "patch rows are remapped: not an interior form");
  const int fr = lane & 15, g = lane >> 4;
  const int rrow = lane >> 4, c16 = lane & 15;
  const uint32_t voff = (uint32_t)(rrow * a.ldo + c16 * 4) * 4u;
  const char* base = (const char*)(EPI == EPI_RESID ? a.resid : (float*)a.out) + ((size_t)mw * a.ldo + nw) * 4;
  const size_t step = (size_t)a.ldo * 16;
  const char* lp = base;
  const char* sp = base;
  f32x4_t buf[2][4];
  f32x4_t bia = {0.f, 0.f, 0.f, 0.f};
  if constexpr (EPI == EPI_RESID) {
    if (a.bias) gload16(bia, a.bias + nw, (uint32_t)c16 * 16u);
#pragma unroll
    for (int t = 0; t < 4; ++t) {
      gload16(buf[0][t], lp, voff);
      lp += step;
    }
  }
#pragma unroll
  for (int c = 0; c < MF; ++c) {
    if constexpr (EPI == EPI_RESID) {
      if (c + 1 < MF) {
#pragma unroll
        for (int t = 0; t < 4; ++t) {
          gload16(buf[(c + 1) & 1][t], lp, voff);
          lp += step;
        }
      }
    }
#pragma unroll
    for (int fj = 0; fj < 4; ++fj) {
      f32x4_t v = acc[fj][c];
      if constexpr (EPI != EPI_RESID) v += bv[fj];
      if constexpr (epi_gelu(EPI)) {
#pragma unroll
        for (int t = 0; t < 4; ++t) v[t] = epi_erf(EPI) ? gelu_erf(v[t]) : quick_gelu(v[t]);
      }
      *(f32x4_t*)(scratch + fr * 256 + (((g * 4 + fj) ^ fr) << 4)) = v;
    }
    f32x4_t v[4];
#pragma unroll
    for (int t = 0; t < 4; ++t) {
      const int row = t * 4 + rrow;
      v[t] = *(const f32x4_t*)(scratch + row * 256 + ((c16 ^ row) << 4));
    }
    if constexpr (EPI == EPI_RESID) {
      if (c == 0 || c + 1 == MF) wait_vmcnt_pin<4>(buf[c & 1]);
      else wait_vmcnt_pin<8>(buf[c & 1]);
      if (c == 0) asm volatile("" : "+v"(bia));
#pragma unroll
      for (int t = 0; t < 4; ++t) v[t] = (v[t] + bia) + buf[c & 1][t];
    }
#pragma unroll
    for (int t = 0; t < 4; ++t) {
      gstore16(sp, voff, v[t]);
      sp += step;
    }
  }
}

__device__ __forceinline__ void glds16s(const void* sbase, uint32_t voff, uint32_t lds_base) {
  uint32_t keep;
  asm volatile(
      "s_mov_b32 %0, m0\n\ts_mov_b32 m0, %3\n\ts_nop 0\n\tglobal_load_lds_dwordx4 %1, %2\n\t"
      "s_mov_b32 m0, %0"
      : "=&s"(keep)
      : "v"(voff), "s"(sbase), "s"(lds_base)
      : "memory");
}

template <int PREC, int EPI>
__global__ __launch_bounds__(512, 2) void gemm_pp_kernel(const GemmArgs a) {
  using namespace p256;
  enter_precision_mode<PREC>();
  extern __shared__ __attribute__((aligned(16))) char smem[];
  constexpr int ES = prec_esize(PREC);
  const int lane = threadIdx.x & 63;
  const int wave = __builtin_amdgcn_readfirstlane(threadIdx.x >> 6);
  const int grp = wave >> 2, w4 = wave & 3;

  const int nbn = a.N / BN, nbm = a.M / BM;
  const int G8 = gridDim.x >> 3;
  const int xcd = blockIdx.x & 7, jx = blockIdx.x >> 3;
  const int nmt_x = (nbm - xcd + 7) >> 3;
  const int ntl_x = nmt_x * nbn;
  const int ntl = jx < ntl_x ? (ntl_x - jx + G8 - 1) / G8 : 0;
  if (ntl == 0) return;
  const int nk = ksteps(a, ES);
  const int total = ntl * nk;

  const int dmt = G8 / nbn, dnt = G8 - dmt * nbn;
  struct Cursor { int mtl, nt; };
  auto cursor_next = [&](Cursor& c) {
    c.mtl += dmt;
    c.nt += dnt;
    if (c.nt >= nbn) { c.nt -= nbn; ++c.mtl; }
  };
  auto mt_of = [&](int mtl) { return a.rev ? nmt_x - 1 - mtl : mtl; };
  const size_t sx = (size_t)a.ldx * ES, sw = (size_t)a.K * ES;

  struct LaneK { uint32_t voff_x, voff_w; int fo0, fo1; };
  auto lane_consts = [&]() {
    int l = lane;
    asm volatile("" : "+v"(l));
    const int rr = (l >> 4) * 2 + ((l & 15) >> 3);
    const int chunk = (l & 7) ^ (((w4 & 1) << 2) | (l >> 4));
    LaneK c;
    c.voff_x = (uint32_t)(rr * (uint32_t)sx + chunk * 16);
    c.voff_w = (uint32_t)(perm_n(w4 * 8 + rr) * (uint32_t)sw + chunk * 16);
    c.fo0 = frag_off(l & 15, l >> 4, 0);
    c.fo1 = frag_off(l & 15, l >> 4, 1);
    return c;
  };
  Cursor ci{jx / nbn, jx % nbn};
  int ji = 0, kti = 0;
  const char *tx, *tw;
  auto set_issue_tile = [&]() {
    const int m0 = (mt_of(ci.mtl) * 8 + xcd) * BM, n0 = ci.nt * BN;
    tx = (const char*)a.x + (size_t)(m0 + grp * 128 + w4 * 8) * sx;
    tw = (const char*)a.w + (size_t)n0 * sw;
  };
  const uint32_t lds0 = lds_addr(smem);
  auto piece = [&](const LaneK& lk, int st, int i) {
    const uint32_t base = lds0 + st * STAGE_BYTES + w4 * 1024;
    size_t ko, kox;
    kstep_off(a, kti, kox, ko);
    if (i < 4) {
      glds16s(tx + kox + (size_t)(i * 32) * sx, lk.voff_x, base + (grp * 16 + i * 4) * 1024);
    } else {
      const int q = i - 4;
      glds16s(tw + ko + (size_t)((q >> 1) * 64 + (q & 1) * 8) * sw, lk.voff_w, base + A_BYTES + q * 4096);
    }
  };
  constexpr int NP0 = 12;
  auto issue_done = [&]() {
    if (++kti == nk) {
      kti = 0;
      if (++ji < ntl) {
        cursor_next(ci);
        set_issue_tile();
      }
    }
  };

  const int wr = wave >> 2, wc = wave & 3;
  const int xbase = wr * 128 * ROWB;
  const int wbase = A_BYTES + wc * 64 * ROWB;
  typedef uint32_t u32x4_t __attribute__((ext_vector_type(4)));
  u32x4_t xf[8], wf[2][4];
  auto readf = [&](const LaneK& lk, int st, int i) {
    const char* sb = smem + st * STAGE_BYTES;
    if (i < 4) wf[0][i] = *(const u32x4_t*)(sb + wbase + i * 2048 + lk.fo0);
    else if (i < 12) xf[i - 4] = *(const u32x4_t*)(sb + xbase + (i - 4) * 2048 + lk.fo0);
    else wf[1][i - 12] = *(const u32x4_t*)(sb + wbase + (i - 12) * 2048 + lk.fo1);
  };
  auto pin_frags = [&]() {
    asm volatile("s_waitcnt lgkmcnt(0)" ::: "memory");
#pragma unroll
    for (int f = 0; f < 4; ++f) asm volatile("" : "+v"(wf[0][f]));
#pragma unroll
    for (int f = 0; f < 4; ++f) asm volatile("" : "+v"(wf[1][f]));
#pragma unroll
    for (int f = 0; f < 8; ++f) asm volatile("" : "+v"(xf[f]));
  };
  f32x4_t acc[4][8];
  zero_acc<8>(acc);
  float amax = 0.f;
  auto mfma_pair = [&](const u32x4_t& wv4, const u32x4_t& xv4, f32x4_t& c) {
    if constexpr (PREC != MCM_PREC_F32) {
      c = mfma16<PREC>(__builtin_bit_cast(uint4, wv4), __builtin_bit_cast(uint4, xv4), c);
    } else {
      const f32x4_t wv = __builtin_bit_cast(f32x4_t, wv4);
      const f32x4_t xv = __builtin_bit_cast(f32x4_t, xv4);
#pragma unroll
      for (int t = 0; t < 4; ++t) c = __builtin_amdgcn_mfma_f32_16x16x4f32(wv[t], xv[t], c, 0, 0, 0);
    }
  };
  auto compute = [&](int fo1, int st) {
    const char* sb = smem + st * STAGE_BYTES;
#pragma unroll
    for (int fi = 0; fi < 8; ++fi) {
#pragma unroll
      for (int fj = 0; fj < 4; ++fj) mfma_pair(wf[0][fj], xf[fi], acc[fj][fi]);
      xf[fi] = *(const u32x4_t*)(sb + xbase + fi * 2048 + fo1);
    }
#pragma unroll
    for (int fi = 0; fi < 8; ++fi)
#pragma unroll
      for (int fj = 0; fj < 4; ++fj) mfma_pair(wf[1][fj], xf[fi], acc[fj][fi]);
  };

  Cursor cc{jx / nbn, jx % nbn};
  int em0 = 0, en0 = 0;
  f32x4_t bv[4];
#pragma unroll
  for (int fj = 0; fj < 4; ++fj) bv[fj] = (f32x4_t){0.f, 0.f, 0.f, 0.f};
  auto epilogue = [&]() {
    int le = lane;
    asm volatile("" : "+v"(le));
    if constexpr (EPI != EPI_RESID) {
#pragma unroll
      for (int fj = 0; fj < 4; ++fj) asm volatile("" : "+v"(bv[fj]));
    }
    char* win = smem + 2 * STAGE_BYTES + wave * 4096;
    if constexpr (PREC != MCM_PREC_F32 && epi_store16(EPI))
      wave_epilogue_lds<PREC, EPI, 8, true>(a, acc, bv, em0 + wr * 128, en0 + wc * 64, le, win, amax);
    else
      wave_epilogue_f32_interior<EPI, 8>(a, acc, bv, em0 + wr * 128, en0 + wc * 64, le, win);
    zero_acc<8>(acc);
  };
  set_issue_tile();
  {
    const LaneK lk = lane_consts();
#pragma unroll
    for (int i = 0; i < NP0; ++i)
      if (i < 4 || !grp) piece(lk, 0, i);
  }
  issue_done();
  wait_vmcnt<0>();
  __builtin_amdgcn_s_barrier();
  asm volatile("" ::: "memory");
  if (grp) {
    __builtin_amdgcn_s_barrier();
    asm volatile("" ::: "memory");
  }
  int ktc = 0;
  bool pend = false;
  auto phase_barrier = [&]() {
    __builtin_amdgcn_sched_barrier(0);
    __builtin_amdgcn_s_barrier();
    asm volatile("" ::: "memory");
    __builtin_amdgcn_sched_barrier(0);
  };
  for (int s = 0; s < total; ++s) {
    const int sr = s & 1, si = sr ^ 1;
    const bool split = pend && !grp;
    int fo1;
    if (pend) {
      if (!grp) {
        const LaneK lk = lane_consts();
#pragma unroll
        for (int i = 0; i < NP0; ++i) piece(lk, si, i);
        issue_done();
        phase_barrier();
      }
      epilogue();
      if (!grp) {
        const LaneK lk = lane_consts();
        fo1 = lk.fo1;
#pragma unroll
        for (int i = 0; i < 16; ++i) readf(lk, sr, i);
      }
    }
    if (!split) {
      const LaneK lk = lane_consts();
      fo1 = lk.fo1;
      if (!grp) {
#pragma unroll
        for (int i = 0; i < NP0; ++i) {
          if (i < 8) {
            readf(lk, sr, 2 * i);
            readf(lk, sr, 2 * i + 1);
          }
          piece(lk, si, i);
        }
      } else {
#pragma unroll
        for (int i = 0; i < 4; ++i) {
#pragma unroll
          for (int j = 0; j < 4; ++j) readf(lk, sr, 4 * i + j);
          piece(lk, si, i);
        }
      }
      issue_done();
    }
    pin_frags();
    if (!split) phase_barrier();
    if (EPI == EPI_RESID) {
    } else if (ktc == nk - 1 && a.bias) {
      int le = lane;
      asm volatile("" : "+v"(le));
      load_bias_async(a, cc.nt * BN + wc * 64 + (le >> 4) * 16, bv);
    }
    __builtin_amdgcn_s_setprio(1);
    compute(fo1, sr);
    __builtin_amdgcn_s_setprio(0);
    wait_vmcnt<0>();
    phase_barrier();
    pend = false;
    if (++ktc == nk) {
      ktc = 0;
      pend = true;
      em0 = (mt_of(cc.mtl) * 8 + xcd) * BM;
      en0 = cc.nt * BN;
      cursor_next(cc);
    }
  }
  if (!grp) {
    __builtin_amdgcn_s_barrier();
    asm volatile("" ::: "memory");
  }
  if (pend) epilogue();
  if constexpr (epi_store16(EPI)) sat_report<PREC>(amax, a.sat);
}

#ifdef MCM_ARMS
int persistent_grid();
#include "gemm_arms.hpp"
#endif


#ifdef MCM_HARNESS
int g_variant = -1;
int variant() { return g_variant; }
#else
constexpr int variant() { return -1; }
#endif

#ifdef MCM_HARNESS
int g_grid_override = 0;
#endif
int persistent_grid() {
#ifdef MCM_HARNESS
  if (g_grid_override > 0) return g_grid_override;
#endif
  return device_cu_count() / 8 * 8;
}

template <int PREC, int EPI>
hipError_t launch_tile(const GemmArgs& a, hipStream_t s) {
  static PerDeviceFlag attr_set;
  if (!attr_set.get()) {
    hipError_t e = hipFuncSetAttribute((const void*)gemm_tile_kernel<PREC, EPI>,
                                       hipFuncAttributeMaxDynamicSharedMemorySize, tile::LDS_BYTES);
    if (e != hipSuccess) return e;
    attr_set.set();
  }
  const int nbn = (a.N + tile::BN - 1) / tile::BN, nbm = (a.M + tile::BM - 1) / tile::BM;
  hipLaunchKernelGGL((gemm_tile_kernel<PREC, EPI>), dim3(nbn * nbm), dim3(256), tile::LDS_BYTES, s, a);
  return hipGetLastError();
}

template <int PREC, int EPI>
hipError_t launch_tile64(const GemmArgs& a, hipStream_t s) {
  static PerDeviceFlag attr_set;
  if (!attr_set.get()) {
    hipError_t e = hipFuncSetAttribute((const void*)gemm_tile64_kernel<PREC, EPI>,
                                       hipFuncAttributeMaxDynamicSharedMemorySize, tile64::LDS_BYTES);
    if (e != hipSuccess) return e;
    attr_set.set();
  }
  const int nbn = (a.N + tile64::BN - 1) / tile64::BN, nbm = (a.M + tile64::BM - 1) / tile64::BM;
  hipLaunchKernelGGL((gemm_tile64_kernel<PREC, EPI>), dim3(nbn * nbm), dim3(256), tile64::LDS_BYTES, s, a);
  return hipGetLastError();
}

template <int PREC, int EPI, bool CS, bool PXF = false>
hipError_t launch_p256(const GemmArgs& a, hipStream_t s) {
  static PerDeviceFlag attr_set;
  if (!attr_set.get()) {
    hipError_t e = hipFuncSetAttribute((const void*)gemm_p256_kernel<PREC, EPI, CS, PXF>,
                                       hipFuncAttributeMaxDynamicSharedMemorySize, p256::LDS_BYTES);
    if (e != hipSuccess) return e;
    attr_set.set();
  }
  hipLaunchKernelGGL((gemm_p256_kernel<PREC, EPI, CS, PXF>), dim3(persistent_grid()), dim3(512), p256::LDS_BYTES, s, a);
  return hipGetLastError();
}

template <int PREC, int EPI>
hipError_t launch_pp(const GemmArgs& a, hipStream_t s) {
  static PerDeviceFlag attr_set;
  if (!attr_set.get()) {
    hipError_t e = hipFuncSetAttribute((const void*)gemm_pp_kernel<PREC, EPI>,
                                       hipFuncAttributeMaxDynamicSharedMemorySize, p256::LDS_BYTES);
    if (e != hipSuccess) return e;
    attr_set.set();
  }
  hipLaunchKernelGGL((gemm_pp_kernel<PREC, EPI>), dim3(persistent_grid()), dim3(512), p256::LDS_BYTES, s, a);
  return hipGetLastError();
}

int size_policy(int M, int N) {
  int v = variant();
  if (v < 0) {
    const long tiles = (long)((M + p256::BM - 1) / p256::BM) * ((N + p256::BN - 1) / p256::BN);
    v = 2 * tiles > persistent_grid() ? 5 : 0;
  }
  if (v != 0 && v != 11 && persistent_grid() < 8) v = 0;
  return v;
}

template <int PREC, int EPI>
hipError_t launch_one(const GemmArgs& a, hipStream_t s) {
  int v = size_policy(a.M, a.N);
#ifdef MCM_ARMS
  if constexpr (epi_erf(EPI)) {
    if (a.fold_z || a.fold_rs || a.ln_y || a.lnc || a.wblk || v == 9) return hipErrorInvalidValue;
  } else {
    hipError_t e;
    if (arms::route<PREC, EPI>(v, a, s, &e)) return e;
  }
#else
  if (a.fold_z || a.fold_rs || a.ln_y || a.lnc || a.wblk) return hipErrorInvalidValue;
#endif
  if constexpr (EPI == EPI_PATCH) {
    if (a.px) return launch_p256<PREC, EPI, false, true>(a, s);
  }
  if (v == 0 || v == 11) {
    const bool few = (long)((a.M + 127) / 128) * ((a.N + 127) / 128) < 2L * persistent_grid();
    if (v == 11 || (variant() < 0 && few && !MCM_HM(a.hm))) return launch_tile64<PREC, EPI>(a, s);
    return launch_tile<PREC, EPI>(a, s);
  }
#ifdef MCM_HARNESS
  if (v == 4) return launch_p256<PREC, EPI, true>(a, s);
#endif
  if (v == 5) {
    if constexpr (EPI != EPI_PATCH) {
      if (a.M % p256::BM == 0 && a.N % p256::BN == 0) return launch_pp<PREC, EPI>(a, s);
    }
  }
  return launch_p256<PREC, EPI, false>(a, s);
}

template <int PREC, int EPI>
hipError_t launch_one_x2(const GemmArgs& a, hipStream_t s) {
  if constexpr (PREC != MCM_PREC_F16) {
    return hipErrorInvalidValue;
  } else {
    const int v = size_policy(a.M, a.N);
    if (v == 0 || v == 11) {
      const bool few = (long)((a.M + 127) / 128) * ((a.N + 127) / 128) < 2L * persistent_grid();
      return few ? launch_tile64<PREC, EPI>(a, s) : launch_tile<PREC, EPI>(a, s);
    }
    if (a.M % p256::BM == 0 && a.N % p256::BN == 0) return launch_pp<PREC, EPI>(a, s);
    return launch_p256<PREC, EPI, false>(a, s);
  }
}

template <int PREC>
hipError_t launch_prec(int epi, const GemmArgs& a, hipStream_t s) {
  switch (epi) {
    case EPI_STORE_X2: return launch_one_x2<PREC, EPI_STORE_X2>(a, s);
    case EPI_GELU_X2: return launch_one_x2<PREC, EPI_GELU_X2>(a, s);
    case EPI_GELU_ERF_X2: return launch_one_x2<PREC, EPI_GELU_ERF_X2>(a, s);
    case EPI_STORE: return launch_one<PREC, EPI_STORE>(a, s);
    case EPI_GELU: return launch_one<PREC, EPI_GELU>(a, s);
    case EPI_GELU_ERF: return launch_one<PREC, EPI_GELU_ERF>(a, s);
    case EPI_RESID: return launch_one<PREC, EPI_RESID>(a, s);
    case EPI_PATCH: return launch_one<PREC, EPI_PATCH>(a, s);
  }
  return hipErrorInvalidValue;
}

}

#ifdef MCM_HARNESS
void gemm_set_variant(int v) { g_variant = v; }
int g_group_n = 0;
int g_dbg = 0;
void gemm_set_dbg(int d) { g_dbg = d; }
void gemm_set_group_n(int gn) { g_group_n = gn > 0 ? gn : 0; }
#else
constexpr int g_group_n = 0, g_dbg = 0;
#endif

#ifdef MCM_HARNESS
void gemm_set_persistent_grid(int n) { g_grid_override = n; }
hipError_t launch_lnc_cleanup(int prec, const float* x, const float* g, const float* b, void* y, const float2* part, int M, int D,
                              float eps, unsigned int* ln_state, int ln_rs, int ln_cap8, hipStream_t s, unsigned int* sat) {
  if (prec == MCM_PREC_F16) return arms::launch_lnc_cleanup_p<MCM_PREC_F16>(x, g, b, y, part, M, D, eps, ln_state, ln_rs, ln_cap8, s, sat);
  if (prec == MCM_PREC_BF16) return arms::launch_lnc_cleanup_p<MCM_PREC_BF16>(x, g, b, y, part, M, D, eps, ln_state, ln_rs, ln_cap8, s, sat);
  return hipErrorInvalidValue;
}
hipError_t launch_row64_block_w(const void* w, void* blocked, int N, int K, hipStream_t s) {
  if (N % 16 || K % 32) return hipErrorInvalidValue;
  const size_t nchunks = (size_t)N * K / 8;
  hipLaunchKernelGGL(arms::row64_block_w_kernel, dim3((unsigned)((nchunks + 255) / 256)), dim3(256), 0, s, (const uint4*)w, (uint4*)blocked, N, K);
  return hipGetLastError();
}
hipError_t launch_gemm_row64_ln(int prec, const GemmArgs& a, hipStream_t s, int stages) {
  if (prec == MCM_PREC_F16) return arms::launch_row64_ln_p<MCM_PREC_F16>(a, s, stages);
  if (prec == MCM_PREC_BF16) return arms::launch_row64_ln_p<MCM_PREC_BF16>(a, s, stages);
  return hipErrorInvalidValue;
}
#endif
int gemm_persistent_grid() { return persistent_grid(); }
bool gemm_ln_tail_ok(int prec, int M, int N) {
#if !defined(MCM_HARNESS) && !defined(MCM_LN_TAIL)
  return false;
#endif
  if (prec == MCM_PREC_F32 || M <= 0 || M % p256::BM || (N != 768 && N != 1024)) return false;
  return size_policy(M, N) == 5 && persistent_grid() >= 8;
}

bool gemm_patch_takes_pixels(int prec, int M, int N, int kpad, int patch, int image) {
  const int es = prec_esize(prec), ks = ROWB / es, ec = 16 / es;
  if (patch <= 0 || image % patch || patch % ec || ks % patch || kpad != 3 * patch * patch) return false;
  if ((size_t)M / ((size_t)(image / patch) * (image / patch)) * 3 * image * image * 4 >= (1ull << 32)) return false;
  return size_policy(M, N) != 0 && persistent_grid() >= 8;
}

int gemm_fold_kind(int epi, int M, int N) {
  if (epi == EPI_PATCH || epi_erf(epi) || M <= 0 || N <= 0) return 0;
  const int v = size_policy(M, N);
  if (v == 5 && M % p256::BM == 0 && N % p256::BN == 0) return 1;
  if (v == 0) return 2;
  return 0;
}

static hipError_t launch_gemm_one(int prec, int epi, const GemmArgs& a, hipStream_t s) {
  switch (prec) {
    case MCM_PREC_BF16: return launch_prec<MCM_PREC_BF16>(epi, a, s);
    case MCM_PREC_F16: return launch_prec<MCM_PREC_F16>(epi, a, s);
    case MCM_PREC_F32: return launch_prec<MCM_PREC_F32>(epi, a, s);
  }
  return hipErrorInvalidValue;
}

hipError_t launch_gemm(int prec, int epi, const GemmArgs& a_in, hipStream_t s) {
  GemmArgs a = a_in;
  const int es = prec_esize(prec);
  if (a.gn <= 0) {
    const int nbn = (a.N + 255) / 256;
    a.gn = g_group_n > 0 ? g_group_n : nbn;
  }
  a.dbg = g_dbg;
  if (a.M <= 0 || a.N <= 0 || a.K <= 0 || (a.K * es) % ROWB || a.N % 16 || (a.ldx * es) % 16 ||
      a.ldo % 4)
    return hipErrorInvalidValue;
  if (a.ksplit && (a.ksplit != 1 || prec == MCM_PREC_F32 || ((a.K * es) / ROWB) % 2 || a.fold_z || a.fold_rs || a.ln_y))
    return hipErrorInvalidValue;
  if ((a.xsplit || epi_x2(epi)) && (prec != MCM_PREC_F16 || (a.xsplit != 0 && a.xsplit != 1) || a.fold_z || a.fold_rs || a.ln_y ||
                                    a.hm || a.px || variant() >= 0))
    return hipErrorInvalidValue;
  if (a.xsplit && a.ldx % 128) return hipErrorInvalidValue;
  if (epi_x2(epi) && (a.N % 64 || a.ldo % 128)) return hipErrorInvalidValue;
  if (a.hm && (a.hm < a.M || a.N % 64 || !(epi == EPI_STORE || epi == EPI_GELU) || prec == MCM_PREC_F32)) return hipErrorInvalidValue;
#ifndef MCM_HARNESS
  if (a.hm) return hipErrorInvalidValue;
#endif
#ifndef MCM_NO_SLIVER_SPLIT
  {
    const int G = persistent_grid();
    const bool fold = a.fold_z != nullptr || a.fold_rs != nullptr;
    if (epi != EPI_PATCH && !fold && !a.ln_y && variant() < 0 && G >= 8 && a.M % p256::BM == 0 && a.N % p256::BN == 0 &&
        size_policy(a.M, a.N) == 5) {
      const long nbn = a.N / p256::BN, rt = a.M / p256::BM, T = rt * nbn, R = T / G, left = T - R * G;
      const long rt1 = 8 * ((R * (G / 8)) / nbn);
      const long rest_wgs = (rt - rt1) * 2 * (a.N / 128);
      if (R >= 1 && left > 0 && left * 4 <= G && rt1 >= 1 && rt1 < rt && rest_wgs * 2 >= G &&
          size_policy((int)(rt1 * p256::BM), a.N) == 5 && size_policy((int)((rt - rt1) * p256::BM), a.N) == 0) {
        GemmArgs m = a, r = a;
        const size_t row0 = (size_t)rt1 * p256::BM;
        m.M = (int)row0;
        r.M = a.M - (int)row0;
        r.x = (const char*)a.x + row0 * a.ldx * es;
        if (a.out) r.out = (char*)a.out + (a.hm ? row0 * 64 : row0 * a.ldo) * es;
        if (a.resid) r.resid = a.resid + row0 * a.ldo;
        hipError_t e = launch_gemm_one(prec, epi, m, s);
        return e != hipSuccess ? e : launch_gemm_one(prec, epi, r, s);
      }
    }
  }
#endif
  return launch_gemm_one(prec, epi, a, s);
}
```

mcm_amd/csrc/mcm_api.hip:

```cpp
#include <algorithm>
#include <map>
#include <string>
#include <vector>

#include <math.h>
#include <stdlib.h>
#include <string.h>

#include "bank_sim.hpp"
#include "common.hpp"

namespace {

thread_local std::string g_create_err;

struct Param {
  std::vector<int64_t> shape;
  int64_t numel = 0;
  float* dev = nullptr;
  bool set = false;
};

struct LayerW {
  void *wqkv = nullptr, *wo = nullptr, *w1 = nullptr, *w2 = nullptr;
// ... 1248 lines not shown
    h->ms_acc[k] = 0;
    h->launches[k] = 0;
    h->flops[k] = 0;
  }
  return MCM_OK;
}


int mcm_op_linear(mcm_handle* h, int32_t prec, const void* x_dev, const void* w_dev, const float* bias_dev,
                  void* y_dev, float* resid_dev, int32_t M, int32_t N, int32_t K, int32_t epi,
                  void* stream) {
  return mcm_op_linear_ex(h, prec, x_dev, w_dev, bias_dev, y_dev, resid_dev, M, N, K, epi, 0, stream);
}

int mcm_op_linear_ex(mcm_handle* h, int32_t prec, const void* x_dev, const void* w_dev, const float* bias_dev,
                     void* y_dev, float* resid_dev, int32_t M, int32_t N, int32_t K, int32_t epi, int32_t flags,
                     void* stream) {
  if (!h) return MCM_EINVAL;
  if (epi < EPI_STORE || epi > EPI_RESID) return fail(h, MCM_EINVAL, "bad epilogue");
  const bool split = (flags & MCM_LINEAR_SPLIT_W) != 0, xs = (flags & MCM_LINEAR_SPLIT_X) != 0, os = (flags & MCM_LINEAR_SPLIT_OUT) != 0;
  const bool erf = (flags & MCM_LINEAR_ACT_GELU) != 0;
  if ((flags & ~(MCM_LINEAR_SPLIT_W | MCM_LINEAR_SPLIT_X | MCM_LINEAR_SPLIT_OUT | MCM_LINEAR_ACT_GELU)) ||
      (split && (prec == MCM_PREC_F32 || K % 64)))
    return fail(h, MCM_EINVAL, "bad flags (split weights: 16-bit modes, K % 64 == 0)");
  if (erf && epi != EPI_GELU) return fail(h, MCM_EINVAL, "bad flags (MCM_LINEAR_ACT_GELU: epilogue 1 only)");
  if ((xs || os) && (prec != MCM_PREC_F16 || K % 64 || (os && (epi == EPI_RESID || N % 64))))
    return fail(h, MCM_EINVAL, "bad flags (split activations / outputs: fp16 mode, K % 64 == 0; outputs: epilogues 0 / 1, N % 64 == 0)");
  GemmArgs a{};
  a.x = x_dev; a.w = w_dev; a.bias = bias_dev; a.out = y_dev; a.resid = resid_dev;
  a.M = M; a.N = N; a.K = split ? 2 * K : K; a.ldx = xs ? 2 * K : K; a.ldo = os ? 2 * N : N; a.ksplit = split ? 1 : 0;
  a.xsplit = xs ? 1 : 0;
  if (os) epi = epi == EPI_STORE ? EPI_STORE_X2 : erf ? EPI_GELU_ERF_X2 : EPI_GELU_X2;
  else if (erf) epi = EPI_GELU_ERF;
  a.sat = h->sat_on ? h->sat_dev : nullptr;
  HIP_TRY(h, launch_gemm(prec, epi, a, (hipStream_t)stream));
  return MCM_OK;
}

int mcm_op_split_weight(mcm_handle* h, int32_t prec, const float* w_dev, int32_t N, int32_t K, void* out_dev,
                        void* stream) {
  if (!h) return MCM_EINVAL;
  if (!w_dev || !out_dev || N <= 0 || K <= 0 || K % 64 || prec == MCM_PREC_F32)
    return fail(h, MCM_EINVAL, "split weights: 16-bit modes, K % 64 == 0");
  HIP_TRY(h, launch_cvt_weight_split(prec, w_dev, out_dev, N, K, K, (hipStream_t)stream));
  return MCM_OK;
}

int mcm_op_layernorm(mcm_handle* h, int32_t prec, const float* x_dev, const float* gamma_dev,
                     const float* beta_dev, void* y_dev, int32_t M, int32_t D, float eps, int32_t out_f32,
                     void* stream) {
  if (!h) return MCM_EINVAL;
  HIP_TRY(h, launch_layernorm(prec, x_dev, gamma_dev, beta_dev, y_dev, M, D, eps, out_f32 != 0,
                              (hipStream_t)stream, 0, 0, false, h->sat_on ? h->sat_dev : nullptr));
  return MCM_OK;
}

int mcm_op_layernorm_split(mcm_handle* h, const float* x_dev, const float* gamma_dev, const float* beta_dev,
                           void* y_dev, int32_t M, int32_t D, float eps, void* stream) {
  if (!h) return MCM_EINVAL;
  HIP_TRY(h, launch_layernorm(MCM_PREC_F16, x_dev, gamma_dev, beta_dev, y_dev, M, D, eps, false, (hipStream_t)stream, 0, 0,
                              false, h->sat_on ? h->sat_dev : nullptr, true));
  return MCM_OK;
}

int mcm_op_attention_split(mcm_handle* h, const void* qkv_dev, void* out_dev, int32_t nseq, int32_t seq_len,
                           int32_t heads, void* stream) {
  if (!h) return MCM_EINVAL;
  HIP_TRY(h, launch_attention(MCM_PREC_F16, qkv_dev, out_dev, nseq, seq_len, heads, 64, false, 0, (hipStream_t)stream, false, 0, true));
  return MCM_OK;
}

int mcm_op_attention(mcm_handle* h, int32_t prec, const void* qkv_dev, void* out_dev, int32_t nseq,
                     int32_t seq_len, int32_t heads, int32_t causal, void* stream) {
  if (!h) return MCM_EINVAL;
  HIP_TRY(h, launch_attention(prec, qkv_dev, out_dev, nseq, seq_len, heads, 64, causal != 0, 0,
                              (hipStream_t)stream, false, 0, false, h->fault_dev));
  return MCM_OK;
}

#ifdef MCM_HARNESS
__global__ void act_kernel(const float* __restrict__ x, float* __restrict__ y, size_t n, int act) {
  const size_t stride = (size_t)gridDim.x * blockDim.x;
  for (size_t i = (size_t)blockIdx.x * blockDim.x + threadIdx.x; i < n; i += stride)
    y[i] = act == 2 ? gelu_erf(x[i]) : act == 1 ? quick_gelu_fast(x[i]) : quick_gelu(x[i]);
}
int mcm_debug_op_act(mcm_handle* h, int32_t act, const float* x_dev, float* y_dev, int64_t n, void* stream) {
  if (!h) return MCM_EINVAL;
  if (act < 0 || act > 2 || !x_dev || !y_dev || n <= 0) return fail(h, MCM_EINVAL, "act 0 ... 2, n > 0, device pointers");
  const size_t blocks = ((size_t)n + 255) / 256;
  hipLaunchKernelGGL(act_kernel, dim3((unsigned)(blocks < 4096 ? blocks : 4096)), dim3(256), 0, (hipStream_t)stream, x_dev, y_dev,
                     (size_t)n, (int)act);
  HIP_TRY(h, hipGetLastError());
  return MCM_OK;
}

int mcm_debug_attention_variant(int32_t variant) {
  if (variant != 0 && variant != 1 && variant != 10 && variant != 11 && variant != 21 && variant != 36) return MCM_EINVAL;
  attention_set_variant(variant);
  return MCM_OK;
}

int mcm_debug_attn_spin_budget(int64_t polls) {
  if (polls < 0 || polls > 0xffffffffLL) return MCM_EINVAL;
  attention_set_spin_budget((unsigned int)polls);
  return MCM_OK;
}

int mcm_debug_clear_faults(mcm_handle* h) {
  if (!h || !h->fault_pin) return MCM_EINVAL;
  (void)hipDeviceSynchronize();
  *(volatile unsigned int*)h->fault_pin = 0u;
  return MCM_OK;
}

int mcm_debug_op_attention(mcm_handle* h, int32_t prec, const void* qkv_dev, void* out_dev, int32_t nseq, int32_t seq_len,
                           int32_t heads, int32_t causal, int32_t qrows, int32_t reverse, void* stream) {
  if (!h) return MCM_EINVAL;
  HIP_TRY(h, launch_attention(prec, qkv_dev, out_dev, nseq, seq_len, heads, 64, causal != 0, qrows, (hipStream_t)stream, reverse != 0, 0, false,
                              h->fault_dev));
  return MCM_OK;
}

int mcm_debug_op_attention_hd(mcm_handle* h, int32_t prec, const void* qkv_dev, void* out_dev, int32_t nseq, int32_t seq_len,
                              int32_t heads, int32_t head_dim, int32_t causal, int32_t qrows, int32_t reverse, void* stream) {
  if (!h) return MCM_EINVAL;
  HIP_TRY(h, launch_attention(prec, qkv_dev, out_dev, nseq, seq_len, heads, head_dim, causal != 0, qrows, (hipStream_t)stream,
                              reverse != 0, 0, false, h->fault_dev));
  return MCM_OK;
}

int mcm_debug_op_attention_split(mcm_handle* h, const void* qkv_dev, void* out_dev, int32_t nseq, int32_t seq_len,
                                 int32_t heads, int32_t qrows, int32_t reverse, void* stream) {
  if (!h) return MCM_EINVAL;
  HIP_TRY(h, launch_attention(MCM_PREC_F16, qkv_dev, out_dev, nseq, seq_len, heads, 64, false, qrows, (hipStream_t)stream,
                              reverse != 0, 0, true));
  return MCM_OK;
}

int mcm_debug_op_attention_split_hd(mcm_handle* h, const void* qkv_dev, void* out_dev, int32_t nseq, int32_t seq_len,
                                    int32_t heads, int32_t head_dim, int32_t qrows, int32_t reverse, void* stream) {
  if (!h) return MCM_EINVAL;
  HIP_TRY(h, launch_attention(MCM_PREC_F16, qkv_dev, out_dev, nseq, seq_len, heads, head_dim, false, qrows, (hipStream_t)stream,
                              reverse != 0, 0, true));
  return MCM_OK;
}

int mcm_debug_vision_front(mcm_handle* h, const void* pixels_dev, int32_t pixel_format, int32_t x2, int32_t B, int32_t stage,
                           int32_t poison, float* resid_out_dev, void* ln_out_dev, void* stream) {
  if (pixel_format != MCM_PIXELS_F32_NCHW && pixel_format != MCM_PIXELS_U8_NHWC) return fail(h, MCM_EINVAL, "unknown pixel_format");
  int rc = check_image_call(h, pixels_dev, resid_out_dev, B, x2 != 0);
  if (rc) return rc;
  if (stage < 0 || stage > 1 || (stage == 1 && !ln_out_dev)) return fail(h, MCM_EINVAL, "stage 0 or 1; stage 1 needs ln_out_dev");
  hipStream_t s = (hipStream_t)stream;
  const size_t es = (size_t)prec_esize(h->cfg.precision) * (x2 ? 2 : 1), rows = (size_t)B * h->ntok, D = (size_t)h->cfg.v_width;
  if (poison) {
    HIP_TRY(h, hipMemsetAsync(h->patches, 0xFF, (size_t)B * h->np * h->kpad * es, s));
    HIP_TRY(h, hipMemsetAsync(h->x, 0xFF, rows * D * sizeof(float), s));
  }
  if ((rc = vision_front(h, s, pixels_dev, pixel_format == MCM_PIXELS_U8_NHWC, B, x2 != 0, stage))) return rc;
  HIP_TRY(h, hipMemcpyAsync(resid_out_dev, h->x, rows * D * sizeof(float), hipMemcpyDeviceToDevice, s));
  if (stage == 1) HIP_TRY(h, hipMemcpyAsync(ln_out_dev, h->ln, rows * D * es, hipMemcpyDeviceToDevice, s));
  return MCM_OK;
}

int mcm_debug_op_pool_project(mcm_handle* h, const float* x_dev, int64_t x_rows, const int32_t* row_idx_host, int32_t row_stride,
                              int32_t n, int32_t D, const float* gamma_dev, const float* beta_dev, float eps,
                              const float* proj_dev, int32_t P, float* out_dev, int32_t normalize, void* stream) {
  if (!h) return MCM_EINVAL;
  if (!x_dev || !gamma_dev || !beta_dev || !proj_dev || !out_dev || n <= 0 || D <= 0 || P <= 0 || x_rows <= 0 || row_stride < 0)
    return fail(h, MCM_EINVAL, "bad argument");
  if (row_idx_host) {
    for (int32_t i = 0; i < n; ++i)
      if (row_idx_host[i] < 0 || row_idx_host[i] >= x_rows) return fail(h, MCM_EINVAL, "row index outside x");
  } else if ((int64_t)(n - 1) * row_stride >= x_rows) {
    return fail(h, MCM_EINVAL, "strided rows outside x");
  }
  hipStream_t s = (hipStream_t)stream;
  int32_t* idx_dev = nullptr;
  if (row_idx_host) {
    HIP_TRY(h, hipMalloc((void**)&idx_dev, (size_t)n * sizeof(int32_t)));
    hipError_t e = hipMemcpy(idx_dev, row_idx_host, (size_t)n * sizeof(int32_t), hipMemcpyHostToDevice);
    if (e != hipSuccess) {
      (void)hipFree(idx_dev);
      HIP_TRY(h, e);
    }
  }
  hipError_t e = launch_pool_project(x_dev, idx_dev, row_stride, n, D, gamma_dev, beta_dev, eps, proj_dev, P, out_dev, s,
                                     normalize != 0);
  const bool refused = e == hipErrorInvalidValue;
  if (e == hipSuccess) e = hipStreamSynchronize(s);
  if (idx_dev) (void)hipFree(idx_dev);
  if (refused) return fail(h, MCM_EINVAL, "launch_pool_project refused the shape (D <= 1280, D % 4 == 0 — D % 64 == 0 past 1024 —, P <= 1024)");
  HIP_TRY(h, e);
  return MCM_OK;
}

int mcm_debug_op_text_embed(mcm_handle* h, const int32_t* ids_host, int32_t vocab, const float* tok_dev, const float* pos_dev,
                            float* x_dev, int32_t K, int32_t S, int32_t D, void* stream) {
  if (!h) return MCM_EINVAL;
  if (!ids_host || !tok_dev || !pos_dev || !x_dev || K <= 0 || S <= 0 || D <= 0 || vocab <= 0) return fail(h, MCM_EINVAL, "bad argument");
  const size_t nid = (size_t)K * S;
  for (size_t i = 0; i < nid; ++i)
    if (ids_host[i] < 0 || ids_host[i] >= vocab) return fail(h, MCM_EINVAL, "token id out of range");
  hipStream_t s = (hipStream_t)stream;
  int32_t* ids_dev = nullptr;
  HIP_TRY(h, hipMalloc((void**)&ids_dev, nid * sizeof(int32_t)));
  hipError_t e = hipMemcpy(ids_dev, ids_host, nid * sizeof(int32_t), hipMemcpyHostToDevice);
  bool refused = false;
  if (e == hipSuccess) {
    e = launch_text_embed(ids_dev, tok_dev, pos_dev, x_dev, K, S, D, s);
    refused = e == hipErrorInvalidValue;
  }
  if (e == hipSuccess) e = hipStreamSynchronize(s);
  (void)hipFree(ids_dev);
  if (refused) return fail(h, MCM_EINVAL, "launch_text_embed refused the shape (D % 4 == 0)");
  HIP_TRY(h, e);
  return MCM_OK;
}

int mcm_debug_gemm_dbg(int32_t bits) {
  gemm_set_dbg(bits);
  return MCM_OK;
}

int mcm_debug_ln_fold(int32_t on) {
  g_ln_fold = on ? 1 : 0;
  return MCM_OK;
}

int mcm_debug_ln_tail(int32_t on) {
  g_ln_tail = on ? 1 : 0;
  return MCM_OK;
}
int mcm_debug_ln_cluster(int32_t on) {
  g_ln_cluster = on ? 1 : 0;
  return MCM_OK;
}
int mcm_debug_ln_row(int32_t on) {
  g_ln_row = (on >= 1 && on <= 4) ? on : 0;
  return MCM_OK;
}
int mcm_debug_ln_cluster_spin(int32_t polls) {
  g_lnc_spin = polls < 0 ? -1 : polls;
  return MCM_OK;
}
int mcm_debug_ln_cluster_deferred(mcm_handle* h, uint64_t* count_host) {
  if (!h || !count_host) return MCM_EINVAL;
  *count_host = 0;
  if (!h->ln_state) return MCM_OK;
  HIP_TRY(h, hipDeviceSynchronize());
  for (int x = 0; x < 8; ++x) {
    unsigned int v = 0;
    HIP_TRY(h, hipMemcpy(&v, h->ln_state + (size_t)x * h->ln_rs + 2 * h->ln_cap8 + 3, sizeof(v), hipMemcpyDeviceToHost));
    *count_host += v;
  }
  return MCM_OK;
}
int mcm_debug_ln_tail_timeouts(mcm_handle* h, uint64_t* count_host) {
  if (!h || !count_host) return MCM_EINVAL;
  *count_host = 0;
  if (!h->ln_state) return MCM_OK;
  HIP_TRY(h, hipDeviceSynchronize());
  for (int x = 0; x < 8; ++x) {
    unsigned int v = 0;
    HIP_TRY(h, hipMemcpy(&v, h->ln_state + (size_t)x * h->ln_rs + h->ln_cap8 + 2, sizeof(v), hipMemcpyDeviceToHost));
    *count_host += v;
  }
  return MCM_OK;
}
int mcm_debug_qkv_head_major(int32_t on) {
  g_qkv_head_major = on ? 1 : 0;
  return MCM_OK;
}
int mcm_debug_patch_fold(int32_t on) {
  g_patch_fold = on ? 1 : 0;
  return MCM_OK;
}
int mcm_debug_persistent_grid(int32_t n) {
  if (n < 0 || n % 8 != 0) return MCM_EINVAL;
  gemm_set_persistent_grid(n);
  return MCM_OK;
}
int mcm_debug_resize_fused_only(int32_t on) {
  g_resize_fused_only = on ? 1 : 0;
  return MCM_OK;
}
int mcm_debug_gemm_group_n(int32_t gn) {
  if (gn < 0 || gn > 64) return MCM_EINVAL;
  gemm_set_group_n(gn);
  return MCM_OK;
}
int mcm_debug_nsplit(int32_t n) {
  if (n < 1 || n > 4) return MCM_EINVAL;
  g_nsplit = n;
  return MCM_OK;
}
int mcm_debug_qkv_chunks(int32_t n) {
  if (n < 1 || n > 16) return MCM_EINVAL;
  g_qkv_chunks = n;
  return MCM_OK;
}

int mcm_debug_gemm_variant(int32_t variant) {
  if (variant != -1 && variant != 0 && variant != 3 && variant != 4 && variant != 5 && variant != 9 && variant != 11) return MCM_EINVAL;
  gemm_set_variant(variant);
  return MCM_OK;
}

#endif

}
```

mcm_amd/csrc/score.hip:

```cpp
#include "common.hpp"

namespace {

__device__ __forceinline__ double wave_sum_d(double v) {
#pragma unroll
  for (int o = 32; o > 0; o >>= 1) v += __shfl_xor(v, o, 64);
  return v;
}

constexpr int NWV = 16;

__device__ __forceinline__ double block_sum_d(double v, double* red, int lane, int wave) {
  v = wave_sum_d(v);
  __syncthreads();
  if (lane == 0) red[wave] = v;
  __syncthreads();
  double t = 0.0;
#pragma unroll
  for (int i = 0; i < NWV; ++i) t += red[i];
  return t;
}

__device__ __forceinline__ void pair_better(float& v, int& i, float ov, int oi) {
  if (oi >= 0 && (i < 0 || ov > v || (ov == v && oi < i))) {
    v = ov;
    i = oi;
  }
}

template <bool TOPK>
__global__ __launch_bounds__(NWV * 64) void score_kernel(const float* __restrict__ img,
                                                    const float* __restrict__ text, int K, int P,
                                                    float T, int kind, float* __restrict__ scores,
                                                    int topk, int* __restrict__ idx,
                                                    float* __restrict__ prob) {
  extern __shared__ __attribute__((aligned(16))) char smem[];
  float* f = (float*)smem;
  float* sim = f + P;
  __shared__ double red[NWV];
  __shared__ float redf[NWV];
  const int b = blockIdx.x, tid = threadIdx.x, lane = tid & 63, wave = tid >> 6;
  for (int d = tid; d < P; d += NWV * 64) f[d] = img[(size_t)b * P + d];
  __syncthreads();
  for (int k = wave; k < K; k += NWV) {
    const float* t = text + (size_t)k * P;
    float a = 0.f;
    for (int d = lane * 4; d < P; d += 256) {
      const float4 tv = *(const float4*)(t + d);
      const float4 fv = *(const float4*)(f + d);
      a = fmaf(tv.x, fv.x, a);
      a = fmaf(tv.y, fv.y, a);
      a = fmaf(tv.z, fv.z, a);
      a = fmaf(tv.w, fv.w, a);
    }
    a = wave_sum(a);
    if (lane == 0) sim[k] = a;
  }
  __syncthreads();
  float m = -INFINITY;
  for (int k = tid; k < K; k += NWV * 64) m = fmaxf(m, sim[k]);
  m = wave_max(m);
  if (lane == 0) redf[wave] = m;
  __syncthreads();
  m = redf[0];
#pragma unroll
  for (int i = 1; i < NWV; ++i) m = fmaxf(m, redf[i]);
  float selv = 0.f;
  int seli = -1;
  if constexpr (TOPK) {
    __shared__ float stv[2][NWV];
    __shared__ int sti[2][NWV];
    float pv = INFINITY;
    int pi = -1;
    for (int r = 0; r < topk; ++r) {
      float bv = 0.f;
      int bi = -1;
      for (int k = tid; k < K; k += NWV * 64) {
        const float v = sim[k];
        if ((v < pv || (v == pv && k > pi)) && (bi < 0 || v > bv)) {
          bv = v;
          bi = k;
        }
      }
#pragma unroll
      for (int o = 32; o > 0; o >>= 1) {
        const float ov = __shfl_xor(bv, o, 64);
        const int oi = __shfl_xor(bi, o, 64);
        pair_better(bv, bi, ov, oi);
      }
      if (lane == 0) {
        stv[r & 1][wave] = bv;
        sti[r & 1][wave] = bi;
      }
      __syncthreads();
      bv = stv[r & 1][0];
      bi = sti[r & 1][0];
#pragma unroll
      for (int i = 1; i < NWV; ++i) pair_better(bv, bi, stv[r & 1][i], sti[r & 1][i]);
      if (bi < 0) break;
      if (tid == r) {
        selv = bv;
        seli = bi;
      }
      pv = bv;
      pi = bi;
    }
    if (tid < topk) idx[(size_t)b * topk + tid] = seli;
  }
  if (kind == MCM_SCORE_MAX_LOGIT) {
    if (tid == 0) scores[b] = -m;
    if constexpr (TOPK) {
      if (!prob) return;
    } else {
      return;
    }
  }
  const float mt = m / T;
  double z = 0.0, ez = 0.0;
  for (int k = tid; k < K; k += NWV * 64) {
    const float u = sim[k] / T - mt;
    const float e = expf(u);
    sim[k] = e;
    z += (double)e;
    ez += (double)e * (double)u;
  }
  z = block_sum_d(z, red, lane, wave);
  if constexpr (TOPK) {
    if (prob && tid < topk)
      prob[(size_t)b * topk + tid] = seli < 0 ? NAN : (float)((double)expf(selv / T - mt) / z);
    if (kind == MCM_SCORE_MAX_LOGIT) return;
  }
  if (kind == MCM_SCORE_MCM) {
    if (tid == 0) scores[b] = -(float)(1.0 / z);
  } else if (kind == MCM_SCORE_ENERGY) {
    if (tid == 0) scores[b] = -(T * (mt + (float)log(z)));
  } else if (kind == MCM_SCORE_ENTROPY) {
    ez = block_sum_d(ez, red, lane, wave);
    if (tid == 0) scores[b] = (float)(log(z) - ez / z);
  } else {
    const float rz = (float)(1.0 / z);
    double s1 = 0.0;
    for (int k = tid; k < K; k += NWV * 64) {
      const float p = sim[k] * rz;
      sim[k] = p;
      s1 += (double)p;
    }
    const double mean = block_sum_d(s1, red, lane, wave) / (double)K;
    double s2 = 0.0;
    for (int k = tid; k < K; k += NWV * 64) {
      const double c = (double)sim[k] - mean;
      s2 += c * c;
    }
    s2 = block_sum_d(s2, red, lane, wave);
    if (tid == 0) scores[b] = (float)(-(s2 / (double)K));
  }
}

__global__ __launch_bounds__(256) void maha_prepare_kernel(const float* __restrict__ means,
                                                           const float* __restrict__ prec, int P,
                                                           double* __restrict__ w, double* __restrict__ k) {
  extern __shared__ __attribute__((aligned(16))) char smem[];
  double* mu = (double*)smem;
  __shared__ double red[4];
  const int c = blockIdx.x, tid = threadIdx.x;
  for (int j = tid; j < P; j += 256) mu[j] = (double)means[(size_t)c * P + j];
  __syncthreads();
  double kc = 0.0;
  for (int p = tid; p < P; p += 256) {
    double a = 0.0, b = 0.0;
    for (int j = 0; j < P; ++j) {
      a += (double)prec[(size_t)p * P + j] * mu[j];
      b += (double)prec[(size_t)j * P + p] * mu[j];
    }
    w[(size_t)c * P + p] = a + b;
    kc += mu[p] * a;
  }
  kc = wave_sum_d(kc);
  if ((tid & 63) == 0) red[tid >> 6] = kc;
  __syncthreads();
  if (tid == 0) k[c] = (red[0] + red[1]) + (red[2] + red[3]);
}

__global__ __launch_bounds__(NWV * 64) void maha_score_kernel(const float* __restrict__ feats,
                                                              const float* __restrict__ prec,
                                                              const double* __restrict__ w,
                                                              const double* __restrict__ k, int C, int P,
                                                              float* __restrict__ scores) {
  extern __shared__ __attribute__((aligned(16))) char smem[];
  double* f = (double*)smem;
  __shared__ double red[NWV];
  const int b = blockIdx.x, tid = threadIdx.x, lane = tid & 63, wave = tid >> 6;
  for (int j = tid; j < P; j += NWV * 64) f[j] = (double)feats[(size_t)b * P + j];
  __syncthreads();
  double qa = 0.0;
  for (int p = wave; p < P; p += NWV) {
    double a = 0.0;
    for (int j = lane; j < P; j += 64) a += (double)prec[(size_t)p * P + j] * f[j];
    a = wave_sum_d(a);
    if (lane == 0) qa += f[p] * a;
  }
  const double q = block_sum_d(lane == 0 ? qa : 0.0, red, lane, wave);
  double best = INFINITY;
  for (int c = wave; c < C; c += NWV) {
    double a = 0.0;
    for (int j = lane; j < P; j += 64) a += w[(size_t)c * P + j] * f[j];
    a = wave_sum_d(a);
    best = fmin(best, q - a + k[c]);
  }
  __syncthreads();
  if (lane == 0) red[wave] = best;
  __syncthreads();
  if (tid == 0) {
    double m = red[0];
    for (int i = 1; i < NWV; ++i) m = fmin(m, red[i]);
    scores[b] = (float)(0.5 * m);
  }
}

constexpr int FT = 64;
constexpr int FK = 32;

__global__ __launch_bounds__(256) void maha_fit_kernel(const float* __restrict__ feats, int B, int P,
                                                       const float* __restrict__ shift, double* __restrict__ gram,
                                                       double* __restrict__ sum) {
  __shared__ double xs[2][FK][FT];
  const int nt = (P + FT - 1) / FT;
  int idx = blockIdx.x, ti = 0;
  while (idx >= nt - ti) {
    idx -= nt - ti;
    ++ti;
  }
  const int tj = ti + idx;
  const bool diag = ti == tj;
  const int tid = threadIdx.x, tx = tid & 15, ty = tid >> 4;
  const int sc = tid & 63, sr = tid >> 6;
  const int ci = ti * FT + sc, cj = tj * FT + sc;
  const double shi = (shift && ci < P) ? (double)shift[ci] : 0.0;
  const double shj = (shift && cj < P) ? (double)shift[cj] : 0.0;
  const double(*xi)[FT] = xs[0];
  const double(*xj)[FT] = diag ? xs[0] : xs[1];

  double acc[4][4];
#pragma unroll
  for (int r = 0; r < 4; ++r)
#pragma unroll
    for (int c = 0; c < 4; ++c) {
      const int i = ti * FT + ty + 16 * r, j = tj * FT + tx + 16 * c;
      acc[r][c] = (i < P && j < P && i <= j) ? gram[(size_t)i * P + j] : 0.0;
    }
  const bool sums = diag && tid < FT;
  double s = (sums && ci < P) ? sum[ci] : 0.0;

  float ri[FK / 4], rj[FK / 4];
  auto fetch = [&](int b0) {
#pragma unroll
    for (int m = 0; m < FK / 4; ++m) {
      const int b = b0 + sr + 4 * m;
      ri[m] = (b < B && ci < P) ? feats[(size_t)b * P + ci] : 0.f;
      rj[m] = (!diag && b < B && cj < P) ? feats[(size_t)b * P + cj] : 0.f;
    }
  };
  fetch(0);
  for (int b0 = 0; b0 < B; b0 += FK) {
    __syncthreads();
#pragma unroll
    for (int m = 0; m < FK / 4; ++m) {
      xs[0][sr + 4 * m][sc] = ci < P ? (double)ri[m] - shi : 0.0;
      if (!diag) xs[1][sr + 4 * m][sc] = cj < P ? (double)rj[m] - shj : 0.0;
    }
    __syncthreads();
    if (b0 + FK < B) fetch(b0 + FK);
    const int kmax = min(FK, B - b0);
    for (int k = 0; k < kmax; ++k) {
      double a[4], b[4];
#pragma unroll
      for (int r = 0; r < 4; ++r) a[r] = xi[k][ty + 16 * r];
#pragma unroll
      for (int c = 0; c < 4; ++c) b[c] = xj[k][tx + 16 * c];
#pragma unroll
      for (int r = 0; r < 4; ++r)
#pragma unroll
        for (int c = 0; c < 4; ++c) acc[r][c] = fma(a[r], b[c], acc[r][c]);
    }
    if (sums)
      for (int k = 0; k < kmax; ++k) s += xi[k][sc];
  }
#pragma unroll
  for (int r = 0; r < 4; ++r)
#pragma unroll
    for (int c = 0; c < 4; ++c) {
      const int i = ti * FT + ty + 16 * r, j = tj * FT + tx + 16 * c;
      if (i < P && j < P && i <= j) {
        gram[(size_t)i * P + j] = acc[r][c];
        if (i != j) gram[(size_t)j * P + i] = acc[r][c];
      }
    }
  if (sums && ci < P) sum[ci] = s;
}

}

hipError_t launch_maha_fit(const float* feats, int B, int P, const float* shift, double* gram, double* sum,
                           hipStream_t s) {
  if (B <= 0 || P <= 0 || P > 4096 || !feats || !gram || !sum) return hipErrorInvalidValue;
  const int nt = (P + FT - 1) / FT;
  hipLaunchKernelGGL(maha_fit_kernel, dim3(nt * (nt + 1) / 2), dim3(256), 0, s, feats, B, P, shift, gram, sum);
  return hipGetLastError();
}

hipError_t launch_maha_prepare(const float* means, const float* prec, int C, int P, double* w, double* c,
                               hipStream_t s) {
  if (C <= 0 || P <= 0 || P > 4096) return hipErrorInvalidValue;
  hipLaunchKernelGGL(maha_prepare_kernel, dim3(C), dim3(256), P * sizeof(double), s, means, prec, P, w, c);
  return hipGetLastError();
}

hipError_t launch_maha_score(const float* feats, int B, const float* prec, const double* w, const double* c,
                             int C, int P, float* scores, hipStream_t s) {
  if (B <= 0 || C <= 0 || P <= 0 || P > 4096) return hipErrorInvalidValue;
  hipLaunchKernelGGL(maha_score_kernel, dim3(B), dim3(NWV * 64), P * sizeof(double), s, feats, prec, w, c, C,
                     P, scores);
  return hipGetLastError();
}

hipError_t launch_score(const float* img, int B, const float* text, int K, int P, float T, int kind,
                        float* scores, hipStream_t s) {
  if (B <= 0 || K <= 0 || P % 4 || kind < 0 || kind > MCM_SCORE_VAR || !(T > 0.f))
    return hipErrorInvalidValue;
  const int lds = (P + K) * (int)sizeof(float);
  if (lds > 150 * 1024) return hipErrorInvalidValue;
  static PerDeviceFlag attr_set;
  if (!attr_set.get()) {
    hipError_t e = hipFuncSetAttribute((const void*)score_kernel<false>,
                                       hipFuncAttributeMaxDynamicSharedMemorySize, 150 * 1024);
    if (e != hipSuccess) return e;
    attr_set.set();
  }
  hipLaunchKernelGGL(score_kernel<false>, dim3(B), dim3(NWV * 64), lds, s, img, text, K, P, T, kind, scores,
                     0, (int*)nullptr, (float*)nullptr);
  return hipGetLastError();
}

bool score_shape_ok(int K, int P) { return K > 0 && P > 0 && P % 4 == 0 && (int64_t)(P + (int64_t)K) * 4 <= 150 * 1024; }

hipError_t launch_score_topk(const float* img, int B, const float* text, int K, int P, float T, int kind,
                             int topk, float* scores, int* idx, float* prob, hipStream_t s) {
  if (B <= 0 || !score_shape_ok(K, P) || kind < 0 || kind > MCM_SCORE_VAR || !(T > 0.f) || topk < 1 ||
      topk > MCM_TOPK_MAX || !scores || !idx)
    return hipErrorInvalidValue;
  const int lds = (P + K) * (int)sizeof(float);
  static PerDeviceFlag attr_set;
  if (!attr_set.get()) {
    hipError_t e = hipFuncSetAttribute((const void*)score_kernel<true>,
                                       hipFuncAttributeMaxDynamicSharedMemorySize, 150 * 1024);
    if (e != hipSuccess) return e;
    attr_set.set();
  }
  hipLaunchKernelGGL(score_kernel<true>, dim3(B), dim3(NWV * 64), lds, s, img, text, K, P, T, kind, scores,
                     topk, idx, prob);
  return hipGetLastError();
}
```

mcm_amd/engine.py:

```python
from __future__ import annotations

import ctypes
import os
from typing import Dict, Optional

import numpy as np

from .config import (ABI_VERSION, CConfig, ClipGeometry, DT_BF16, DT_F16, DT_F32, PREC_BF16, PREC_F16, PREC_F32,
                     SCORE_KINDS, WEIGHT_OPERANDS, geometry)

_HERE = os.path.dirname(os.path.abspath(__file__))
LIB_PATH = os.path.join(_HERE, "libmcm_hip.so")
HARNESS_LIB_PATH = os.path.join(_HERE, "libmcm_hip_harness.so")
KERNEL_CLASSES = ["patchify", "gemm", "layernorm", "attention", "pool_project", "score", "embed",
                  "gemm_qkv", "gemm_outproj", "gemm_fc1", "gemm_fc2"]

TOPK_MAX = 8

_libs = {}


class NativeLibraryMissing(RuntimeError):
    pass


def load_library(harness: bool = False):
    if harness in _libs:
        return _libs[harness]
    path = HARNESS_LIB_PATH if harness else LIB_PATH
    if not os.path.exists(path):
        raise NativeLibraryMissing(
            f"{path} not found: build it with `python -c 'import __graft_entry__ as g; g.build()'` "
            "(make -C mcm_amd/csrc).  mcm_amd has no CPU fallback.")
    try:
        import torch
    except ImportError:
        pass
    L = ctypes.CDLL(path)
    vp, i32, f32 = ctypes.c_void_p, ctypes.c_int32, ctypes.c_float
    L.mcm_abi_version.restype = i32
    L.mcm_create.argtypes = [ctypes.POINTER(CConfig), ctypes.POINTER(vp)]
    L.mcm_destroy.argtypes = [vp]
    L.mcm_destroy.restype = None
    L.mcm_last_error.argtypes = [vp]
    L.mcm_last_error.restype = ctypes.c_char_p
    L.mcm_set_weight.argtypes = [vp, ctypes.c_char_p, vp, i32, ctypes.POINTER(ctypes.c_int64), i32]
    L.mcm_weights_operand_exact.argtypes = [vp, ctypes.POINTER(ctypes.c_uint64), ctypes.POINTER(i32)]
    L.mcm_finalize_weights.argtypes = [vp]
    L.mcm_encode_text.argtypes = [vp, vp, i32, i32, vp, vp]
    L.mcm_encode_image.argtypes = [vp, vp, i32, vp, vp]
    L.mcm_score_features.argtypes = [vp, vp, i32, vp, i32, f32, i32, vp, vp]
    L.mcm_score.argtypes = [vp, vp, i32, vp, i32, f32, i32, vp, vp]
    L.mcm_score_features_topk.argtypes = [vp, vp, i32, vp, i32, f32, i32, i32, vp, vp, vp, vp]
    L.mcm_score_topk.argtypes = [vp, vp, i32, i32, i32, vp, i32, f32, i32, i32, vp, vp, vp, vp]
    L.mcm_profile_enable.argtypes = [vp, i32]
    L.mcm_profile_read.argtypes = [vp, ctypes.POINTER(ctypes.c_double),
                                   ctypes.POINTER(ctypes.c_int64), ctypes.POINTER(ctypes.c_double)]
    L.mcm_op_linear.argtypes = [vp, i32, vp, vp, vp, vp, vp, i32, i32, i32, i32, vp]
    L.mcm_op_linear_ex.argtypes = [vp, i32, vp, vp, vp, vp, vp, i32, i32, i32, i32, i32, vp]
    L.mcm_op_split_weight.argtypes = [vp, i32, vp, i32, i32, vp, vp]
    L.mcm_op_layernorm.argtypes = [vp, i32, vp, vp, vp, vp, i32, i32, f32, i32, vp]
    L.mcm_op_attention.argtypes = [vp, i32, vp, vp, i32, i32, i32, i32, vp]
    L.mcm_op_layernorm_split.argtypes = [vp, vp, vp, vp, vp, i32, i32, f32, vp]
    L.mcm_op_attention_split.argtypes = [vp, vp, vp, i32, i32, i32, vp]
    L.mcm_x2_max_batch.argtypes = [vp]
    L.mcm_x2_max_batch.restype = i32
    L.mcm_kernel_faults.argtypes = [vp]
    L.mcm_kernel_faults.restype = i32
    L.mcm_encode_image_x2.argtypes = [vp, vp, i32, i32, i32, vp, vp]
    L.mcm_score_x2.argtypes = [vp, vp, i32, i32, vp, i32, f32, i32, vp, vp]
    if harness:
        L.mcm_debug_gemm_variant.argtypes = [i32]
        L.mcm_debug_op_act.argtypes = [vp, i32, vp, vp, ctypes.c_int64, vp]
        L.mcm_debug_attention_variant.argtypes = [i32]
        L.mcm_debug_attn_spin_budget.argtypes = [ctypes.c_int64]
        L.mcm_debug_clear_faults.argtypes = [vp]
        L.mcm_debug_qkv_chunks.argtypes = [i32]
        L.mcm_debug_ln_fold.argtypes = [i32]
        L.mcm_debug_qkv_head_major.argtypes = [i32]
        L.mcm_debug_ln_tail.argtypes = [i32]
        L.mcm_debug_ln_cluster.argtypes = [i32]
        L.mcm_debug_ln_cluster_spin.argtypes = [i32]
        L.mcm_debug_ln_row.argtypes = [i32]
        L.mcm_debug_ln_cluster_deferred.argtypes = [vp, vp]
        L.mcm_debug_ln_tail_timeouts.argtypes = [vp, vp]
        L.mcm_debug_gemm_dbg.argtypes = [i32]
        L.mcm_debug_nsplit.argtypes = [i32]
        L.mcm_debug_gemm_group_n.argtypes = [i32]
        L.mcm_debug_patch_fold.argtypes = [i32]
        L.mcm_debug_resize_fused_only.argtypes = [i32]
        L.mcm_debug_persistent_grid.argtypes = [i32]
        L.mcm_debug_op_attention.argtypes = [vp, i32, vp, vp, i32, i32, i32, i32, i32, i32, vp]
        L.mcm_debug_op_attention_split.argtypes = [vp, vp, vp, i32, i32, i32, i32, i32, vp]
        L.mcm_debug_op_attention_hd.argtypes = [vp, i32, vp, vp, i32, i32, i32, i32, i32, i32, i32, vp]
        L.mcm_debug_op_attention_split_hd.argtypes = [vp, vp, vp, i32, i32, i32, i32, i32, i32, vp]
        L.mcm_debug_vision_front.argtypes = [vp, vp, i32, i32, i32, i32, i32, vp, vp, vp]
        L.mcm_debug_op_pool_project.argtypes = [vp, vp, ctypes.c_int64, vp, i32, i32, i32, vp, vp, f32, vp, i32, vp, i32, vp]
        L.mcm_debug_op_text_embed.argtypes = [vp, vp, i32, vp, vp, vp, i32, i32, i32, vp]
    L.mcm_encode_image_u8.argtypes = [vp, vp, i32, vp, vp]
    L.mcm_score_u8.argtypes = [vp, vp, i32, vp, i32, f32, i32, vp, vp]
    L.mcm_reduce_bank.argtypes = [vp, vp, i32, i32, vp, vp]
    L.mcm_resize_crop_u8.argtypes = [vp, ctypes.POINTER(vp), ctypes.POINTER(i32), ctypes.POINTER(i32), i32, vp, vp]
    L.mcm_jpeg_reconstruct.argtypes = [vp, vp, vp, vp, i32, vp, ctypes.POINTER(ctypes.c_int64), vp]
    L.mcm_jpeg_entropy_decode.argtypes = [ctypes.POINTER(ctypes.c_char_p), i32, vp, ctypes.c_int64, vp, vp, i32,
                                          ctypes.POINTER(ctypes.c_int64)]
    L.mcm_pack_u8.argtypes = [ctypes.POINTER(vp), ctypes.POINTER(ctypes.c_int64), ctypes.POINTER(ctypes.c_int64), i32, vp,
                              ctypes.c_int64, i32]
    L.mcm_tokenizer_create.argtypes = [ctypes.c_char_p, ctypes.c_char_p, ctypes.POINTER(vp)]
    L.mcm_tokenizer_destroy.argtypes = [vp]
    L.mcm_tokenizer_destroy.restype = None
    L.mcm_tokenizer_last_error.argtypes = [vp]
    L.mcm_tokenizer_last_error.restype = ctypes.c_char_p
    L.mcm_tokenizer_vocab_size.argtypes = [vp]
    L.mcm_tokenizer_vocab_size.restype = i32
    L.mcm_tokenizer_encode.argtypes = [vp, ctypes.POINTER(ctypes.c_char_p), i32, i32, vp, vp, ctypes.POINTER(i32)]
    L.mcm_encode_image_raw.argtypes = [vp, vp, i32, vp, vp]
    L.mcm_encode_image_ex.argtypes = [vp, vp, i32, i32, i32, vp, vp]
    L.mcm_encode_text_ex.argtypes = [vp, vp, i32, i32, i32, vp, vp]
    L.mcm_score_histogram.argtypes = [vp, vp, ctypes.c_int64, vp, i32, vp, vp]
    L.mcm_maha_prepare.argtypes = [vp, vp, vp, i32, vp, vp, vp]
    L.mcm_maha_score_features.argtypes = [vp, vp, i32, vp, vp, vp, i32, vp, vp]
    L.mcm_maha_fit_accumulate.argtypes = [vp, vp, i32, vp, vp, vp, vp]
    L.mcm_knn_workspace_bytes.argtypes = [vp, i32, ctypes.c_int64, i32, i32, ctypes.POINTER(ctypes.c_int64)]
    L.mcm_knn_score_features.argtypes = [vp, vp, i32, vp, ctypes.c_int64, i32, i32, vp, ctypes.c_int64, vp, vp, vp]
    L.mcm_neglabel_workspace_bytes.argtypes = [vp, i32, i32, i32, i32, i32, ctypes.POINTER(ctypes.c_int64)]
    L.mcm_neglabel_score_features.argtypes = [vp, vp, i32, vp, i32, i32, i32, ctypes.c_float, i32, vp, ctypes.c_int64, vp, vp, vp]
    L.mcm_local_workspace_bytes.argtypes = [vp, i32, i32, i32, ctypes.POINTER(ctypes.c_int64)]
    L.mcm_local_score_features.argtypes = [vp, vp, i32, i32, vp, i32, ctypes.c_float, vp, ctypes.c_int64, vp, vp, vp]
    L.mcm_encode_image_local.argtypes = [vp, vp, i32, i32, vp, vp, vp]
    L.mcm_score_glmcm.argtypes = [vp, vp, i32, i32, vp, i32, ctypes.c_float, ctypes.c_float, vp, vp, vp, vp, vp]
    L.mcm_measures.argtypes = [vp, vp, ctypes.c_int64, vp, ctypes.c_int64, i32, ctypes.c_double,
                               ctypes.POINTER(ctypes.c_double), vp]
    L.mcm_saturation_check.argtypes = [vp, i32]
    L.mcm_saturation_count.argtypes = [vp, i32, ctypes.POINTER(ctypes.c_uint64), vp]
    if L.mcm_abi_version() != ABI_VERSION:
        raise RuntimeError(f"{path}: ABI version {L.mcm_abi_version()}, this package speaks {ABI_VERSION} — rebuild (make -C mcm_amd/csrc)")
    _libs[harness] = L
    return L


EXPORTED_SYMBOLS = [
    "mcm_abi_version", "mcm_create", "mcm_destroy", "mcm_last_error", "mcm_set_weight",
    "mcm_finalize_weights", "mcm_encode_text", "mcm_encode_image", "mcm_score_features",
    "mcm_score", "mcm_profile_enable", "mcm_profile_read", "mcm_op_linear", "mcm_op_layernorm",
    "mcm_op_attention", "mcm_encode_image_u8", "mcm_score_u8",
    "mcm_reduce_bank", "mcm_measures", "mcm_resize_crop_u8", "mcm_tokenizer_create",
    "mcm_tokenizer_destroy", "mcm_tokenizer_last_error", "mcm_tokenizer_vocab_size", "mcm_tokenizer_encode",
    "mcm_encode_image_raw", "mcm_maha_prepare", "mcm_maha_score_features",
    "mcm_encode_image_ex", "mcm_encode_text_ex", "mcm_score_histogram",
    "mcm_saturation_check", "mcm_saturation_count",
    "mcm_weights_operand_exact", "mcm_op_linear_ex", "mcm_op_split_weight", "mcm_pack_u8",
    "mcm_jpeg_entropy_decode", "mcm_jpeg_reconstruct",
    "mcm_x2_max_batch", "mcm_encode_image_x2", "mcm_score_x2", "mcm_op_layernorm_split", "mcm_op_attention_split",
    "mcm_kernel_faults",
    "mcm_score_features_topk", "mcm_score_topk",
    "mcm_maha_fit_accumulate",
    "mcm_knn_workspace_bytes", "mcm_knn_score_features",
    "mcm_neglabel_workspace_bytes", "mcm_neglabel_score_features",
    "mcm_local_workspace_bytes", "mcm_local_score_features", "mcm_encode_image_local", "mcm_score_glmcm",
]
HARNESS_ONLY_SYMBOLS = ["mcm_debug_gemm_variant", "mcm_debug_attention_variant", "mcm_debug_qkv_chunks",
                        "mcm_debug_gemm_dbg", "mcm_debug_ln_fold", "mcm_debug_qkv_head_major",
                        "mcm_debug_ln_tail", "mcm_debug_ln_tail_timeouts", "mcm_debug_nsplit",
                        "mcm_debug_gemm_group_n", "mcm_debug_patch_fold", "mcm_debug_resize_fused_only",
                        "mcm_debug_persistent_grid", "mcm_debug_op_attention", "mcm_debug_attn_spin_budget",
                        "mcm_debug_clear_faults", "mcm_debug_ln_cluster", "mcm_debug_ln_cluster_spin",
                        "mcm_debug_ln_cluster_deferred", "mcm_debug_ln_row", "mcm_debug_op_attention_split",
                        "mcm_debug_vision_front", "mcm_debug_op_pool_project", "mcm_debug_op_text_embed",
                        "mcm_debug_op_act", "mcm_debug_op_attention_hd", "mcm_debug_op_attention_split_hd"]


def _stream_ptr():
    import torch

    return ctypes.c_void_p(torch.cuda.current_stream().cuda_stream)


class NativeCLIP:

    def __init__(self, geo: ClipGeometry | str, state_dict: Dict[str, np.ndarray], *,
                 device: int = 0, precision: str = "fp16", max_batch: int = 512,
                 max_prompt_tokens: int = 1024 * 77, synthetic_weights: Optional[bool] = None,
                 harness: bool = False, weight_operands: str = "auto", x2_max_batch: Optional[int] = None):
        import torch

        if not torch.cuda.is_available():
            raise RuntimeError("NativeCLIP needs a HIP device (no CPU fallback)")
        self.geo = geometry(geo) if isinstance(geo, str) else geo
        self.device = torch.device("cuda", device)
        self.x2_default = precision == "fp16x2"
        self.precision = {"bf16": PREC_BF16, "fp32": PREC_F32, "f32": PREC_F32, "fp16": PREC_F16,
                          "f16": PREC_F16, "fp16x2": PREC_F16}[precision]
        self.max_batch = int(max_batch)
        self.synthetic_weights = synthetic_weights
        self._lib = load_library(harness)
        torch.cuda.set_device(self.device)
        torch.cuda.init()
        self._cfg = self.geo.to_c(device=device, precision=self.precision, max_batch=max_batch,
                                  max_prompt_tokens=max_prompt_tokens,
                                  weight_operands=WEIGHT_OPERANDS[weight_operands],
                                  x2_max_batch=int(x2_max_batch or 0))
        self._h = ctypes.c_void_p()
        rc = self._lib.mcm_create(ctypes.byref(self._cfg), ctypes.byref(self._h))
        if rc:
            raise RuntimeError(f"mcm_create rc={rc}: {self._lib.mcm_last_error(None).decode()}")
        for name, arr in state_dict.items():
            if name == "logit_scale" or name.endswith("position_ids"):
                continue
            arr = np.asarray(arr)
            if arr.dtype == np.float16:
                a, dt = np.ascontiguousarray(arr), DT_F16
            elif str(arr.dtype) == "bfloat16":
                a, dt = np.ascontiguousarray(arr).view(np.uint16), DT_BF16
            else:
                a, dt = np.ascontiguousarray(arr, dtype=np.float32), DT_F32
            shape = (ctypes.c_int64 * max(a.ndim, 1))(*a.shape)
            self._check(self._lib.mcm_set_weight(self._h, name.encode(), a.ctypes.data_as(ctypes.c_void_p), dt,
                                                 shape, a.ndim))
        self._check(self._lib.mcm_finalize_weights(self._h))
        n, sp = ctypes.c_uint64(0), ctypes.c_int32(0)
        self._check(self._lib.mcm_weights_operand_exact(self._h, ctypes.byref(n), ctypes.byref(sp)))
        self.weights_inexact, self.split_weights = int(n.value), bool(sp.value)

    def _check(self, rc: int):
        if rc:
            raise RuntimeError(f"libmcm_hip rc={rc}: {self._lib.mcm_last_error(self._h).decode()}")

    def close(self):
        if getattr(self, "_h", None):
            self._lib.mcm_destroy(self._h)
            self._h = None

    def __del__(self):
        try:
            self.close()
        except Exception:
            pass

    def eval(self):
        return self

    def _pixels(self, pixel_values):
        import torch

        S = self.geo.image_size
        if pixel_values.dtype == torch.uint8:
            if pixel_values.dim() != 4 or tuple(pixel_values.shape[1:]) != (S, S, 3):
                raise ValueError(f"uint8 input must be [b,{S},{S},3] NHWC, got {tuple(pixel_values.shape)}")
            return pixel_values.to(device=self.device).contiguous()
        if pixel_values.dim() != 4 or tuple(pixel_values.shape[1:]) != (3, S, S):
            raise ValueError(f"Input image size {tuple(pixel_values.shape)} doesn't match model (3x{S}x{S}).")
        return pixel_values.to(device=self.device, dtype=torch.float32).contiguous()

    def get_image_features(self, pixel_values, normalize: bool = False):
        import torch

        if self.x2_default:
            return self.get_image_features_x2(pixel_values, normalize=normalize)
        px = self._pixels(pixel_values)
        fmt = 1 if px.dtype == torch.uint8 else 0
        out = torch.empty((px.shape[0], self.geo.proj_dim), device=self.device, dtype=torch.float32)
        for s in range(0, px.shape[0], self.max_batch):
            n = min(self.max_batch, px.shape[0] - s)
            self._check(self._lib.mcm_encode_image_ex(self._h, px[s:s + n].data_ptr(), fmt, n, int(bool(normalize)),
                                                      out[s:s + n].data_ptr(), _stream_ptr()))
        return out

    def get_image_features_raw(self, pixel_values):
        return self.get_image_features(pixel_values, normalize=False)

    def maha_prepare(self, classwise_mean, precision):
        import torch

        mu = classwise_mean.to(device=self.device, dtype=torch.float32).contiguous()
        pr = precision.to(device=self.device, dtype=torch.float32).contiguous()
        C, P = mu.shape
        assert P == self.geo.proj_dim and pr.shape == (P, P)
        w = torch.empty((C, P), device=self.device, dtype=torch.float64)
        k = torch.empty((C,), device=self.device, dtype=torch.float64)
        self._check(self._lib.mcm_maha_prepare(self._h, mu.data_ptr(), pr.data_ptr(), C, w.data_ptr(),
                                               k.data_ptr(), _stream_ptr()))
        return {"prec": pr, "w": w, "k": k, "C": C}

    def maha_scores(self, features, state):
        import torch

        f = features.to(device=self.device, dtype=torch.float32).contiguous()
        out = torch.empty(f.shape[0], device=self.device, dtype=torch.float32)
        self._check(self._lib.mcm_maha_score_features(self._h, f.data_ptr(), f.shape[0], state["prec"].data_ptr(),
                                                      state["w"].data_ptr(), state["k"].data_ptr(), state["C"],
                                                      out.data_ptr(), _stream_ptr()))
        return out

    def maha_fit_state(self, shift=None):
        import torch

        P = self.geo.proj_dim
        sh = (torch.zeros(P, device=self.device, dtype=torch.float32) if shift is None
              else shift.to(device=self.device, dtype=torch.float32).reshape(-1).contiguous())
        if sh.shape != (P,):
            raise ValueError(f"shift must hold proj_dim = {P} values, got {tuple(sh.shape)}")
        return {"gram": torch.zeros((P, P), device=self.device, dtype=torch.float64),
                "sum": torch.zeros(P, device=self.device, dtype=torch.float64), "shift": sh, "n": 0}

    def maha_fit_accumulate(self, features, state):
        import torch

        f = features.to(device=self.device, dtype=torch.float32).contiguous()
        if f.dim() != 2 or f.shape[1] != self.geo.proj_dim:
            raise ValueError(f"features must be [B, {self.geo.proj_dim}], got {tuple(f.shape)}")
        self._check(self._lib.mcm_maha_fit_accumulate(self._h, f.data_ptr(), f.shape[0], state["shift"].data_ptr(),
                                                      state["gram"].data_ptr(), state["sum"].data_ptr(), _stream_ptr()))
        state["n"] += int(f.shape[0])
        return state

    def knn_scores(self, features, bank, k, splits: int = 0, return_values: bool = False):
        import torch

        f, bk = self._bank_operands(features, bank)
        k, splits = int(k), int(splits)
        B, N = int(f.shape[0]), int(bk.shape[0])
        scores = torch.empty(B, device=self.device, dtype=torch.float32)
        topv = torch.empty((B, max(k, 0)), device=self.device, dtype=torch.float32) if return_values else None
        for s, n, work in self._bank_blocks(B, getattr(self, "_knn_work", None), lambda n, need: self._check_knn(
                self._lib.mcm_knn_workspace_bytes(self._h, n, N, k, splits, need), n, N, k, splits)):
            self._knn_work = work
            self._check(self._lib.mcm_knn_score_features(
                self._h, f[s:s + n].data_ptr(), n, bk.data_ptr(), N, k, splits, work.data_ptr(), work.numel() * 4,
                scores[s:s + n].data_ptr(), topv[s:s + n].data_ptr() if return_values else None, _stream_ptr()))
        return (scores, topv) if return_values else scores

    def _bank_operands(self, features, bank):
        import torch

        f = features.to(device=self.device, dtype=torch.float32).contiguous()
        bk = bank.to(device=self.device, dtype=torch.float32).contiguous()
        P = self.geo.proj_dim
        if f.dim() != 2 or f.shape[1] != P or bk.dim() != 2 or bk.shape[1] != P:
            raise ValueError(f"features and bank must be [*, {P}], got {tuple(f.shape)} and {tuple(bk.shape)}")
        return f, bk

    def _bank_blocks(self, B, work, workspace_bytes):
        import torch

        for s in range(0, max(B, 1), 4096):
            n = min(4096, B - s)
            need = ctypes.c_int64(0)
            workspace_bytes(n, ctypes.byref(need))
            if work is None or work.numel() * 4 < need.value:
                work = torch.empty((need.value + 3) // 4, device=self.device, dtype=torch.float32)
            yield s, n, work

    def _check_knn(self, rc, B, N, k, splits):
        if rc:
            raise ValueError(f"knn_scores: refused (rc={rc}) for B={B}, N={N}, k={k}, splits={splits}: B >= 1, N >= 1, "
                             "1 <= k <= 1024, 0 <= splits <= 32 and proj_dim % 4 == 0 are required")

    def neglabel_scores(self, features, bank, n_id, groups, group_size, T: float = 0.01, splits: int = 0,
                        return_groups: bool = False):
        import torch

        f, bk = self._bank_operands(features, bank)
        K, G, gs, splits, T = int(n_id), int(groups), int(group_size), int(splits), float(T)
        if K < 1 or G < 1 or gs < 1 or bk.shape[0] != K + G * gs:
            raise ValueError(f"neglabel_scores: the bank has {bk.shape[0]} rows, n_id + groups * group_size = {K} + {G} * {gs}")
        B = int(f.shape[0])
        scores = torch.empty(B, device=self.device, dtype=torch.float32)
        grp = torch.empty((B, G), device=self.device, dtype=torch.float32) if return_groups else None
        for s, n, work in self._bank_blocks(B, getattr(self, "_neg_work", None), lambda n, need: self._check_neglabel(
                self._lib.mcm_neglabel_workspace_bytes(self._h, n, K, G, gs, splits, need), n, K, G, gs, T, splits)):
            self._neg_work = work
            self._check_neglabel(self._lib.mcm_neglabel_score_features(
                self._h, f[s:s + n].data_ptr(), n, bk.data_ptr(), K, G, gs, T, splits, work.data_ptr(), work.numel() * 4,
                scores[s:s + n].data_ptr(), grp[s:s + n].data_ptr() if return_groups else None, _stream_ptr()),
                n, K, G, gs, T, splits)
        return (scores, grp) if return_groups else scores

    def _check_neglabel(self, rc, B, K, G, gs, T, splits):
        if rc == -1:
            raise ValueError(f"neglabel_scores: refused (rc={rc}) for B={B}, n_id={K}, groups={G}, group_size={gs}, T={T}, "
                             f"splits={splits}: B, n_id, group_size >= 1, 1 <= groups <= 1024, T > 0 and finite, "
                             "0 <= splits <= 32 and proj_dim % 4 == 0 are required")
        self._check(rc)

    @property
    def local_rows(self) -> int:
        return (self.geo.image_size // self.geo.patch_size) ** 2

    def _no_x2_local(self, what):
        if self.x2_default:
            raise ValueError(f"{what}: the split-activation arm (precision='fp16x2') has no local pass")

    def get_local_features(self, pixel_values):
        import torch

        self._no_x2_local("get_local_features")
        px = self._pixels(pixel_values)
        fmt = 1 if px.dtype == torch.uint8 else 0
        b, R, P = px.shape[0], self.local_rows, self.geo.proj_dim
        glob = torch.empty((b, P), device=self.device, dtype=torch.float32)
        loc = torch.empty((b, R, P), device=self.device, dtype=torch.float32)
        for s in range(0, b, self.max_batch):
            n = min(self.max_batch, b - s)
            self._check(self._lib.mcm_encode_image_local(self._h, px[s:s + n].data_ptr(), fmt, n, glob[s:s + n].data_ptr(),
                                                         loc[s:s + n].data_ptr(), _stream_ptr()))
        return glob, loc

    def local_scores(self, local, text_features, T: float = 1.0, return_patches: bool = False):
        import torch

        loc = local.to(device=self.device, dtype=torch.float32).contiguous()
        t = self._bank(text_features)
        if loc.dim() != 3 or loc.shape[2] != self.geo.proj_dim or loc.shape[0] == 0 or loc.shape[1] == 0:
            raise ValueError(f"local must be [B,R,{self.geo.proj_dim}] with B, R >= 1, got {tuple(loc.shape)}")
        B, R, K, T = int(loc.shape[0]), int(loc.shape[1]), int(t.shape[0]), float(T)
        need = ctypes.c_int64(0)
        self._check_local(self._lib.mcm_local_workspace_bytes(self._h, B, R, K, ctypes.byref(need)), B, R, K, T)
        work = getattr(self, "_local_work", None)
        if work is None or work.numel() * 4 < need.value:
            work = self._local_work = torch.empty((need.value + 3) // 4, device=self.device, dtype=torch.float32)
        scores = torch.empty(B, device=self.device, dtype=torch.float32)
        patch = torch.empty((B, R), device=self.device, dtype=torch.float32) if return_patches else None
        self._check_local(self._lib.mcm_local_score_features(
            self._h, loc.data_ptr(), B, R, t.data_ptr(), K, T, work.data_ptr(), work.numel() * 4, scores.data_ptr(),
            patch.data_ptr() if return_patches else None, _stream_ptr()), B, R, K, T)
        return (scores, patch) if return_patches else scores

    def _check_local(self, rc, B, R, K, T):
        if rc == -1:
            raise ValueError(f"local_scores: refused (rc={rc}) for B={B}, R={R}, K={K}, T={T}: B, R, K >= 1, B R < 2^31, "
                             "T > 0 and finite and proj_dim % 4 == 0 are required")
        self._check(rc)

    def score_images_glmcm(self, pixel_values, text_features, T: float = 1.0, lam: float = 1.0, return_parts: bool = False):
        import torch

        self._no_x2_local("score_images_glmcm")
        px = self._pixels(pixel_values)
        fmt = 1 if px.dtype == torch.uint8 else 0
        t = self._bank(text_features)
        b, R = px.shape[0], self.local_rows
        out = torch.empty(b, device=self.device, dtype=torch.float32)
        gs = torch.empty(b, device=self.device, dtype=torch.float32) if return_parts else None
        ls = torch.empty(b, device=self.device, dtype=torch.float32) if return_parts else None
        patch = torch.empty((b, R), device=self.device, dtype=torch.float32) if return_parts else None
        for s in range(0, b, self.max_batch):
            n = min(self.max_batch, b - s)
            self._check(self._lib.mcm_score_glmcm(
                self._h, px[s:s + n].data_ptr(), fmt, n, t.data_ptr(), t.shape[0], float(T), float(lam), out[s:s + n].data_ptr(),
                gs[s:s + n].data_ptr() if return_parts else None, ls[s:s + n].data_ptr() if return_parts else None,
                patch[s:s + n].data_ptr() if return_parts else None, _stream_ptr()))
        return (out, gs, ls, patch) if return_parts else out

    def get_text_features(self, input_ids, attention_mask=None, normalize: bool = False):
        import torch

        ids = np.ascontiguousarray(input_ids.detach().cpu().numpy() if hasattr(input_ids, "detach")
                                   else np.asarray(input_ids), dtype=np.int32)
        if ids.ndim != 2:
            raise ValueError("input_ids must be [K,S]")
        K, S = ids.shape
        if S > self.geo.max_positions:
            raise ValueError(f"Sequence length must be less than max_position_embeddings (got {S})")
        out = torch.empty((K, self.geo.proj_dim), device=self.device, dtype=torch.float32)
# ... 271 lines not shown
```

Measured before the change: 26030 images/sec.

## Add multi-row pool-project, multi-row score kernels and skinny GEMM path

Adds a skinny 32x64-tile GEMM kernel with a 6-stage LDS pipeline for small-M problems. Rewrites pool_project and MCM score as multi-row kernels that keep the activation rows in registers, prefetch projection and text rows, and reduce partial dot products with permlane-swap scatter reductions. Each weight or text row fetch is then shared across G rows. The aim is to cut the redundant weight and text-bank traffic and the reduction overhead in the tail stages, at the cost of more registers and more template variants.

```diff
diff --git a/include/mcm.h b/include/mcm.h
--- a/include/mcm.h
+++ b/include/mcm.h
@@ -238,6 +238,11 @@
 
 #ifdef MCM_HARNESS
 int mcm_debug_gemm_variant(int32_t variant);
+int mcm_debug_gemm_last_kernel(void);
+int mcm_debug_tail_kernels(int32_t pool_project, int32_t score);
+int mcm_debug_op_linear_strided(mcm_handle* h, int32_t prec, const void* x_dev, const void* w_dev, const float* bias_dev, void* y_dev,
+                                float* resid_dev, int32_t M, int32_t N, int32_t K, int32_t epi, int32_t flags, int32_t ldx, int32_t ldo,
+                                void* stream);
 int mcm_debug_op_act(mcm_handle* h, int32_t act, const float* x_dev, float* y_dev, int64_t n, void* stream);
 int mcm_debug_attention_variant(int32_t variant);
 int mcm_debug_attn_spin_budget(int64_t polls);
diff --git a/mcm_amd/csrc/common.hpp b/mcm_amd/csrc/common.hpp
--- a/mcm_amd/csrc/common.hpp
+++ b/mcm_amd/csrc/common.hpp
@@ -124,6 +124,56 @@
 #pragma unroll
   for (int o = 32; o > 0; o >>= 1) v += __shfl_xor(v, o, 64);
   return v;
+}
+template <int CTRL>
+__device__ __forceinline__ float wave_dpp(float x) {
+  return __builtin_bit_cast(float, __builtin_amdgcn_update_dpp(0, __builtin_bit_cast(int, x), CTRL, 0xf, 0xf, true));
+}
+__device__ __forceinline__ float swap32_sum(float x, float y) {
+  asm("s_nop 1\n\tv_permlane32_swap_b32 %0, %1\n\ts_nop 1" : "+v"(x), "+v"(y));
+  return x + y;
+}
+__device__ __forceinline__ float swap16_sum(float x, float y) {
+  asm("s_nop 1\n\tv_permlane16_swap_b32 %0, %1\n\ts_nop 1" : "+v"(x), "+v"(y));
+  return x + y;
+}
+template <int R>
+__device__ __forceinline__ void wave_sum_scatter(float (&a)[R], int lane) {
+  static_assert(R == 1 || R == 2 || R == 4 || R == 8, "R values over the xor-32, -16, -8 steps");
+  if constexpr (R >= 2) {
+#pragma unroll
+    for (int r = 0; r < R / 2; ++r) a[r] = swap32_sum(a[r], a[r + R / 2]);
+  }
+  if constexpr (R >= 4) {
+#pragma unroll
+    for (int r = 0; r < R / 4; ++r) a[r] = swap16_sum(a[r], a[r + R / 4]);
+  }
+  if constexpr (R >= 8) {
+    const bool up = (lane & 8) != 0;
+    const float keep = up ? a[1] : a[0];
+    const float send = up ? a[0] : a[1];
+    a[0] = keep + wave_dpp<0x128>(send);
+  }
+  if constexpr (R < 2) a[0] += __shfl_xor(a[0], 32, 64);
+  if constexpr (R < 4) a[0] += __shfl_xor(a[0], 16, 64);
+  if constexpr (R < 8) a[0] += wave_dpp<0x128>(a[0]);
+  a[0] += __shfl_xor(a[0], 4, 64);
+  a[0] += wave_dpp<0x4E>(a[0]);
+  a[0] += wave_dpp<0xB1>(a[0]);
+}
+template <int R>
+__device__ __forceinline__ int wave_sum_scatter_index(int lane) {
+  int v = 0, o = 32;
+#pragma unroll
+  for (int n = R; n > 1; n >>= 1, o >>= 1) v += (lane & o) ? n / 2 : 0;
+  return v;
+}
+template <int R>
+__host__ __device__ constexpr int wave_sum_scatter_lane(int v) {
+  int l = 0, o = 32;
+  for (int n = R; n > 1; n >>= 1, o >>= 1)
+    if (v >= n / 2) { l += o; v -= n / 2; }
+  return l;
 }
 __device__ __forceinline__ float wave_max(float v) {
 #pragma unroll
@@ -258,6 +308,9 @@
 void gemm_set_group_n(int gn);
 void gemm_set_dbg(int d);
 void gemm_set_variant(int v);
+int gemm_last_kernel();
+void pool_project_set_mode(int m);
+void score_set_mode(int m);
 void attention_set_variant(int v);
 void attention_set_spin_budget(unsigned int polls);
 #endif
diff --git a/mcm_amd/csrc/embed.hip b/mcm_amd/csrc/embed.hip
--- a/mcm_amd/csrc/embed.hip
+++ b/mcm_amd/csrc/embed.hip
@@ -171,16 +171,10 @@
 constexpr int NWP = 16;
 constexpr int POOL_MAXD = 1280;
 template <bool WIDE>
-__global__ __launch_bounds__(NWP * 64) void pool_project_kernel(
-    const float* __restrict__ x, const int32_t* __restrict__ row_idx, int row_stride, int D,
-    const float* __restrict__ g, const float* __restrict__ b, float eps,
-    const float* __restrict__ proj, int P, float* __restrict__ out, int normalize) {
-  __shared__ float y[WIDE ? POOL_MAXD : 1024];
-  __shared__ float o[1024];
-  __shared__ float red[2 * NWP];
-  const int n = blockIdx.x, tid = threadIdx.x, lane = tid & 63, wave = tid >> 6;
-  const size_t row = row_idx ? (size_t)row_idx[n] : (size_t)n * row_stride;
-  const float* xr = x + row * D;
+__device__ __forceinline__ void pool_ln_row(const float* __restrict__ xr, int D, const float* __restrict__ g,
+                                            const float* __restrict__ b, float eps, float* __restrict__ y,
+                                            float* __restrict__ red) {
+  const int tid = threadIdx.x, lane = tid & 63, wave = tid >> 6;
   const int t2 = tid + NWP * 64;
   const float xv = tid < D ? xr[tid] : 0.f;
   float xw = 0.f;
@@ -217,6 +211,20 @@
     if (t2 < D) y[t2] = cw * rstd * g[t2] + b[t2];
   }
   __syncthreads();
+}
+
+template <bool WIDE>
+__global__ __launch_bounds__(NWP * 64) void pool_project_kernel(
+    const float* __restrict__ x, const int32_t* __restrict__ row_idx, int row_stride, int D,
+    const float* __restrict__ g, const float* __restrict__ b, float eps,
+    const float* __restrict__ proj, int P, float* __restrict__ out, int normalize) {
+  __shared__ float y[WIDE ? POOL_MAXD : 1024];
+  __shared__ float o[1024];
+  __shared__ float red[2 * NWP];
+  const int n = blockIdx.x, tid = threadIdx.x, lane = tid & 63, wave = tid >> 6;
+  const size_t row = row_idx ? (size_t)row_idx[n] : (size_t)n * row_stride;
+  pool_ln_row<WIDE>(x + row * D, D, g, b, eps, y, red);
+  float tot;
   float sq = 0.f;
   for (int p = wave; p < P; p += NWP) {
     const float* w = proj + (size_t)p * D;
@@ -242,6 +250,104 @@
   for (int i = 0; i < NWP; ++i) tot += red[i];
   const float rn = normalize ? 1.0f / sqrtf(tot) : 1.0f;
   for (int p = tid; p < P; p += NWP * 64) out[(size_t)n * P + p] = o[p] * rn;
+}
+
+template <bool WIDE, int G, int NJ, int KB, int PF>
+__global__ __launch_bounds__(NWP * 64) void pool_project_multi_kernel(
+    const float* __restrict__ x, const int32_t* __restrict__ row_idx, int row_stride, int n_rows, int D,
+    const float* __restrict__ g, const float* __restrict__ b, float eps,
+    const float* __restrict__ proj, int P, float* __restrict__ out, int normalize) {
+  static_assert(NJ * 256 <= (WIDE ? POOL_MAXD : 1024), "NJ float4 per lane and row: D <= NJ * 256");
+  constexpr int R = G * KB;
+  __shared__ __attribute__((aligned(16))) float y[G][WIDE ? POOL_MAXD : 1024];
+  __shared__ float o[G][1024];
+  __shared__ float red[2 * NWP];
+  const int n0 = blockIdx.x * G, tid = threadIdx.x, lane = tid & 63;
+  const int wave = __builtin_amdgcn_readfirstlane(tid >> 6);
+  const int nb = min(G, n_rows - n0);
+  for (int r = 0; r < nb; ++r) {
+    const size_t row = row_idx ? (size_t)row_idx[n0 + r] : (size_t)(n0 + r) * row_stride;
+    pool_ln_row<WIDE>(x + row * D, D, g, b, eps, y[r], red);
+  }
+  float4 yv[G][NJ];
+#pragma unroll
+  for (int r = 0; r < G; ++r)
+#pragma unroll
+    for (int j = 0; j < NJ; ++j) {
+      const int d = lane * 4 + 256 * j;
+      yv[r][j] = (r < nb && d < D) ? *(const float4*)(&y[r][d]) : make_float4(0.f, 0.f, 0.f, 0.f);
+    }
+  const int npw = wave < P ? (P - wave + NWP - 1) / NWP : 0;
+  float4 wv[PF][KB][NJ];
+  auto fetch = [&](float4 (&dst)[KB][NJ], int i0) {
+#pragma unroll
+    for (int kb = 0; kb < KB; ++kb) {
+      const float* w = proj + (size_t)(wave + NWP * min(i0 + kb, npw - 1)) * D;
+#pragma unroll
+      for (int j = 0; j < NJ; ++j) {
+        const int d = lane * 4 + 256 * j;
+        dst[kb][j] = *(const float4*)(w + (d < D ? (unsigned)d : 0u));
+      }
+    }
+  };
+#pragma unroll
+  for (int s = 0; s < PF; ++s)
+    if (s * KB < npw) fetch(wv[s], s * KB);
+  float sq[G];
+#pragma unroll
+  for (int r = 0; r < G; ++r) sq[r] = 0.f;
+  for (int ib = 0; ib < npw; ib += PF * KB) {
+#pragma unroll
+    for (int s = 0; s < PF; ++s) {
+      const int i0 = ib + s * KB;
+      if (i0 < npw) {
+        float a[R];
+#pragma unroll
+        for (int v = 0; v < R; ++v) a[v] = 0.f;
+#pragma unroll
+        for (int j = 0; j < NJ; ++j)
+          if (lane * 4 + 256 * j < D) {
+#pragma unroll
+            for (int r = 0; r < G; ++r)
+#pragma unroll
+              for (int kb = 0; kb < KB; ++kb) {
+                float& t = a[r * KB + kb];
+                t = fmaf(wv[s][kb][j].x, yv[r][j].x, t);
+                t = fmaf(wv[s][kb][j].y, yv[r][j].y, t);
+                t = fmaf(wv[s][kb][j].z, yv[r][j].z, t);
+                t = fmaf(wv[s][kb][j].w, yv[r][j].w, t);
+              }
+          }
+        __builtin_amdgcn_sched_barrier(0);
+        if (i0 + PF * KB < npw) fetch(wv[s], i0 + PF * KB);
+        wave_sum_scatter<R>(a, lane);
+#pragma unroll
+        for (int r = 0; r < G; ++r)
+#pragma unroll
+          for (int kb = 0; kb < KB; ++kb) {
+            const float t = __builtin_bit_cast(float, __builtin_amdgcn_readlane(__builtin_bit_cast(int, a[0]),
+                                                                                wave_sum_scatter_lane<R>(r * KB + kb)));
+            if (i0 + kb < npw) {
+              if (lane == 0) o[r][wave + NWP * (i0 + kb)] = t;
+              sq[r] += t * t;
+            }
+          }
+      }
+    }
+  }
+#pragma unroll
+  for (int r = 0; r < G; ++r) {
+    if (r < nb) {
+      __syncthreads();
+      if (lane == 0) red[wave] = sq[r];
+      __syncthreads();
+      float tot = 0.f;
+#pragma unroll
+      for (int i = 0; i < NWP; ++i) tot += red[i];
+      const float rn = normalize ? 1.0f / sqrtf(tot) : 1.0f;
+      for (int p = tid; p < P; p += NWP * 64) out[(size_t)(n0 + r) * P + p] = o[r][p] * rn;
+    }
+  }
 }
 
 inline int grid_for(size_t total) {
@@ -334,16 +440,44 @@
   return hipGetLastError();
 }
 
+#ifdef MCM_HARNESS
+int g_pool_mode = 0;
+void pool_project_set_mode(int m) { g_pool_mode = m; }
+static int pool_mode() { return g_pool_mode; }
+#else
+static constexpr int pool_mode() { return 0; }
+#endif
+
 hipError_t launch_pool_project(const float* x, const int32_t* row_idx, int row_stride, int n,
                                int D, const float* g, const float* b, float eps,
                                const float* proj, int P, float* out, hipStream_t s, bool normalize) {
   if (n <= 0 || D > POOL_MAXD || D % 4 || P > 1024) return hipErrorInvalidValue;
   if (D > 1024 && D % 64) return hipErrorInvalidValue;
-  if (D > 1024)
-    hipLaunchKernelGGL(pool_project_kernel<true>, dim3(n), dim3(NWP * 64), 0, s, x, row_idx, row_stride, D, g, b,
-                       eps, proj, P, out, normalize ? 1 : 0);
-  else
-    hipLaunchKernelGGL(pool_project_kernel<false>, dim3(n), dim3(NWP * 64), 0, s, x, row_idx, row_stride, D, g, b,
-                       eps, proj, P, out, normalize ? 1 : 0);
-  return hipGetLastError();
-}
+  const int mode = pool_mode(), nz = normalize ? 1 : 0;
+  const dim3 block(NWP * 64);
+#ifdef MCM_HARNESS
+  if (mode == 1) {
+    if (D > 1024)
+      hipLaunchKernelGGL(pool_project_kernel<true>, dim3(n), block, 0, s, x, row_idx, row_stride, D, g, b, eps, proj, P, out, nz);
+    else
+      hipLaunchKernelGGL(pool_project_kernel<false>, dim3(n), block, 0, s, x, row_idx, row_stride, D, g, b, eps, proj, P, out, nz);
+    return hipGetLastError();
+  }
+#endif
+  const bool two = mode == 3 || (mode == 0 && (n + 1) / 2 >= device_cu_count());
+#define MCM_POOL_LAUNCH(WIDE, G, NJ, KB, PF)                                                                                                \
+  hipLaunchKernelGGL((pool_project_multi_kernel<WIDE, G, NJ, KB, PF>), dim3((n + G - 1) / G), block, 0, s, x, row_idx, row_stride, n, D, g, \
+                     b, eps, proj, P, out, nz)
+  if (D > 1024) {
+    if (two) MCM_POOL_LAUNCH(true, 2, 5, 2, 1);
+    else MCM_POOL_LAUNCH(true, 1, 5, 2, 2);
+  } else if (D > 768) {
+    if (two) MCM_POOL_LAUNCH(false, 2, 4, 2, 1);
+    else MCM_POOL_LAUNCH(false, 1, 4, 2, 2);
+  } else {
+    if (two) MCM_POOL_LAUNCH(false, 2, 3, 2, 2);
+    else MCM_POOL_LAUNCH(false, 1, 3, 2, 2);
+  }
+#undef MCM_POOL_LAUNCH
+  return hipGetLastError();
+}
diff --git a/mcm_amd/csrc/gemm.hip b/mcm_amd/csrc/gemm.hip
--- a/mcm_amd/csrc/gemm.hip
+++ b/mcm_amd/csrc/gemm.hip
@@ -505,6 +505,107 @@
   sat_report<PREC>(amax, a.sat);
 }
 
+template <int N>
+__device__ __forceinline__ void wait_vmcnt() {
+  asm volatile("s_waitcnt vmcnt(%0)" ::"n"(N) : "memory");
+}
+
+namespace skinny {
+constexpr int BM = 32, BN = 64;
+constexpr int NS = 6;
+constexpr int X_BYTES = BM * ROWB, W_BYTES = BN * ROWB;
+constexpr int STAGE_BYTES = X_BYTES + W_BYTES;
+constexpr int LDS_BYTES = NS * STAGE_BYTES;
+constexpr int WAVE_LOADS = 6;
+}
+
+template <int PREC, int EPI>
+__global__ __launch_bounds__(128) void gemm_skinny_kernel(const GemmArgs a) {
+  using namespace skinny;
+  enter_precision_mode<PREC>();
+  extern __shared__ __attribute__((aligned(16))) char smem[];
+  constexpr int ES = prec_esize(PREC);
+  const int lane = threadIdx.x & 63;
+  const int wave = __builtin_amdgcn_readfirstlane(threadIdx.x >> 6);
+  const int nbn = (a.N + BN - 1) / BN;
+  const int nbm = (a.M + BM - 1) / BM;
+  const int nwg = nbn * nbm;
+  int lid;
+  {
+    const int bid = blockIdx.x, q = nwg >> 3, r = nwg & 7, xcd = bid & 7;
+    lid = (xcd < r ? xcd * (q + 1) : r * (q + 1) + (xcd - r) * q) + (bid >> 3);
+  }
+  const int m0 = (lid / nbn) * BM;
+  const int n0 = (lid % nbn) * BN;
+  const char* gx[2];
+  const char* gw[4];
+#pragma unroll
+  for (int i = 0; i < 4; ++i) {
+    const int blk = i * 2 + wave;
+    const int p = blk * 4 + (lane >> 4);
+    const int sl = lane & 15;
+    const int row = 2 * p + (sl >> 3);
+    const int chunk = (sl & 7) ^ (p & 7);
+    if (i < 2) gx[i] = (const char*)a.x + ((size_t)min(m0 + row, a.M - 1) * a.ldx) * ES + chunk * 16;
+    const int nr = min(n0 + perm_n(row), a.N - 1);
+    gw[i] = (const char*)a.w + ((size_t)nr * a.K) * ES + chunk * 16;
+  }
+  const uint32_t lds0 = lds_addr(smem);
+  auto stage = [&](int st, int kt) {
+    const uint32_t base = lds0 + st * STAGE_BYTES;
+    size_t kox, kow;
+    kstep_off(a, kt, kox, kow);
+#pragma unroll
+    for (int i = 0; i < 4; ++i) {
+      const int blk = i * 2 + wave;
+      if (i < 2) glds16(gx[i] + kox, __builtin_amdgcn_readfirstlane(base + blk * 1024));
+      glds16(gw[i] + kow, __builtin_amdgcn_readfirstlane(base + X_BYTES + blk * 1024));
+    }
+  };
+  const int fr = lane & 15, g = lane >> 4;
+  const int foff[2] = {frag_off(fr, g, 0), frag_off(fr, g, 1)};
+  const int xbase = wave * 16 * ROWB;
+  f32x4_t acc[4][1];
+  zero_acc(acc);
+  const int nk = ksteps(a, ES);
+#pragma unroll
+  for (int st = 0; st < NS - 1; ++st)
+    if (st < nk) stage(st, st);
+  int cur = 0;
+  for (int kt = 0; kt < nk; ++kt) {
+    if (kt + NS - 1 <= nk) wait_vmcnt<(NS - 2) * WAVE_LOADS>();
+    else wait_vmcnt<0>();
+    __syncthreads();
+    if (kt + NS - 1 < nk) stage(cur == 0 ? NS - 1 : cur - 1, kt + NS - 1);
+    const char* sb = smem + cur * STAGE_BYTES;
+#pragma unroll
+    for (int kk = 0; kk < 2; ++kk) {
+      uint4 wf[4];
+#pragma unroll
+      for (int f = 0; f < 4; ++f) wf[f] = *(const uint4*)(sb + X_BYTES + f * 2048 + foff[kk]);
+      const uint4 xf = *(const uint4*)(sb + xbase + foff[kk]);
+#pragma unroll
+      for (int fj = 0; fj < 4; ++fj) {
+        if constexpr (PREC != MCM_PREC_F32) {
+          acc[fj][0] = mfma16<PREC>(wf[fj], xf, acc[fj][0]);
+        } else {
+          const f32x4_t wv = __builtin_bit_cast(f32x4_t, wf[fj]);
+          const f32x4_t xv = __builtin_bit_cast(f32x4_t, xf);
+#pragma unroll
+          for (int t = 0; t < 4; ++t)
+            acc[fj][0] = __builtin_amdgcn_mfma_f32_16x16x4f32(wv[t], xv[t], acc[fj][0], 0, 0, 0);
+        }
+      }
+    }
+    cur = cur == NS - 1 ? 0 : cur + 1;
+  }
+  f32x4_t bv[4];
+  load_bias(a, n0 + g * 16, bv);
+  float amax = 0.f;
+  wave_epilogue<PREC, EPI, 1>(a, acc, bv, m0 + wave * 16, n0, fr, g, amax);
+  sat_report<PREC>(amax, a.sat);
+}
+
 __device__ __forceinline__ void tile_of(int q, int nmt_x, int nbn, int gn, int& mtl, int& nt) {
   int start = 0, g0 = 0;
   for (;;) {
@@ -518,11 +619,6 @@
     start += cnt;
     g0 += gw;
   }
-}
-
-template <int N>
-__device__ __forceinline__ void wait_vmcnt() {
-  asm volatile("s_waitcnt vmcnt(%0)" ::"n"(N) : "memory");
 }
 
 namespace p256 {
@@ -1065,7 +1161,10 @@
 #ifdef MCM_HARNESS
 int g_variant = -1;
 int variant() { return g_variant; }
+int g_last_kernel = -1;
+inline void note_kernel(int k) { g_last_kernel = k; }
 #else
+inline void note_kernel(int) {}
 constexpr int variant() { return -1; }
 #endif
 
@@ -1107,6 +1206,30 @@
   return hipGetLastError();
 }
 
+template <int PREC, int EPI>
+hipError_t launch_skinny(const GemmArgs& a, hipStream_t s) {
+  static PerDeviceFlag attr_set;
+  if (!attr_set.get()) {
+    hipError_t e = hipFuncSetAttribute((const void*)gemm_skinny_kernel<PREC, EPI>,
+                                       hipFuncAttributeMaxDynamicSharedMemorySize, skinny::LDS_BYTES);
+    if (e != hipSuccess) return e;
+    attr_set.set();
+  }
+  const int nbn = (a.N + skinny::BN - 1) / skinny::BN, nbm = (a.M + skinny::BM - 1) / skinny::BM;
+  hipLaunchKernelGGL((gemm_skinny_kernel<PREC, EPI>), dim3(nbn * nbm), dim3(128), skinny::LDS_BYTES, s, a);
+  return hipGetLastError();
+}
+
+template <int EPI>
+constexpr bool skinny_epi() { return EPI == EPI_STORE || EPI == EPI_GELU || EPI == EPI_GELU_ERF || EPI == EPI_RESID; }
+constexpr int SKINNY_LONG_K = 32;
+inline bool skinny_problem(const GemmArgs& a, int es) {
+  const int G = persistent_grid();
+  if (a.xsplit || MCM_HM(a.hm) || G < 8) return false;
+  const long wg64 = (long)((a.M + tile64::BM - 1) / tile64::BM) * ((a.N + tile64::BN - 1) / tile64::BN);
+  return 2 * wg64 < G && (4 * wg64 <= G || (a.K * es) / ROWB >= SKINNY_LONG_K);
+}
+
 template <int PREC, int EPI, bool CS, bool PXF = false>
 hipError_t launch_p256(const GemmArgs& a, hipStream_t s) {
   static PerDeviceFlag attr_set;
@@ -1139,7 +1262,7 @@
     const long tiles = (long)((M + p256::BM - 1) / p256::BM) * ((N + p256::BN - 1) / p256::BN);
     v = 2 * tiles > persistent_grid() ? 5 : 0;
   }
-  if (v != 0 && v != 11 && persistent_grid() < 8) v = 0;
+  if (v != 0 && v != 11 && v != 12 && persistent_grid() < 8) v = 0;
   return v;
 }
 
@@ -1159,6 +1282,14 @@
   if constexpr (EPI == EPI_PATCH) {
     if (a.px) return launch_p256<PREC, EPI, false, true>(a, s);
   }
+  if constexpr (skinny_epi<EPI>()) {
+    if ((v == 0 && variant() < 0 && skinny_problem(a, prec_esize(PREC))) || (v == 12 && !a.xsplit && !MCM_HM(a.hm))) {
+      note_kernel(12);
+      return launch_skinny<PREC, EPI>(a, s);
+    }
+  }
+  if (v == 12) v = 11;
+  note_kernel(v == 0 || v == 11 ? 0 : v == 5 && EPI != EPI_PATCH && a.M % p256::BM == 0 && a.N % p256::BN == 0 ? 5 : 3);
   if (v == 0 || v == 11) {
     const bool few = (long)((a.M + 127) / 128) * ((a.N + 127) / 128) < 2L * persistent_grid();
     if (v == 11 || (variant() < 0 && few && !MCM_HM(a.hm))) return launch_tile64<PREC, EPI>(a, s);
@@ -1209,6 +1340,7 @@
 
 #ifdef MCM_HARNESS
 void gemm_set_variant(int v) { g_variant = v; }
+int gemm_last_kernel() { return g_last_kernel; }
 int g_group_n = 0;
 int g_dbg = 0;
 void gemm_set_dbg(int d) { g_dbg = d; }
diff --git a/mcm_amd/csrc/mcm_api.hip b/mcm_amd/csrc/mcm_api.hip
--- a/mcm_amd/csrc/mcm_api.hip
+++ b/mcm_amd/csrc/mcm_api.hip
@@ -1574,10 +1574,33 @@
 }
 
 int mcm_debug_gemm_variant(int32_t variant) {
-  if (variant != -1 && variant != 0 && variant != 3 && variant != 4 && variant != 5 && variant != 9 && variant != 11) return MCM_EINVAL;
+  if (variant != -1 && variant != 0 && variant != 3 && variant != 4 && variant != 5 && variant != 9 && variant != 11 && variant != 12)
+    return MCM_EINVAL;
   gemm_set_variant(variant);
   return MCM_OK;
 }
+int mcm_debug_gemm_last_kernel(void) { return gemm_last_kernel(); }
+int mcm_debug_tail_kernels(int32_t pool_project, int32_t score) {
+  if (pool_project < 0 || pool_project > 3 || score < 0 || score > 3) return MCM_EINVAL;
+  pool_project_set_mode(pool_project);
+  score_set_mode(score);
+  return MCM_OK;
+}
+int mcm_debug_op_linear_strided(mcm_handle* h, int32_t prec, const void* x_dev, const void* w_dev, const float* bias_dev, void* y_dev,
+                                float* resid_dev, int32_t M, int32_t N, int32_t K, int32_t epi, int32_t flags, int32_t ldx, int32_t ldo,
+                                void* stream) {
+  if (!h) return MCM_EINVAL;
+  const bool split = (flags & MCM_LINEAR_SPLIT_W) != 0, erf = (flags & MCM_LINEAR_ACT_GELU) != 0;
+  if (epi < EPI_STORE || epi > EPI_RESID || (flags & ~(MCM_LINEAR_SPLIT_W | MCM_LINEAR_ACT_GELU)) || (erf && epi != EPI_GELU) ||
+      (split && (prec == MCM_PREC_F32 || K % 64)) || ldx < K || ldo < N)
+    return fail(h, MCM_EINVAL, "bad argument");
+  GemmArgs a{};
+  a.x = x_dev; a.w = w_dev; a.bias = bias_dev; a.out = y_dev; a.resid = resid_dev;
+  a.M = M; a.N = N; a.K = split ? 2 * K : K; a.ldx = ldx; a.ldo = ldo; a.ksplit = split ? 1 : 0;
+  a.sat = h->sat_on ? h->sat_dev : nullptr;
+  HIP_TRY(h, launch_gemm(prec, erf ? EPI_GELU_ERF : epi, a, (hipStream_t)stream));
+  return MCM_OK;
+}
 
 #endif
 
diff --git a/mcm_amd/csrc/score.hip b/mcm_amd/csrc/score.hip
--- a/mcm_amd/csrc/score.hip
+++ b/mcm_amd/csrc/score.hip
@@ -29,34 +29,12 @@
 }
 
 template <bool TOPK>
-__global__ __launch_bounds__(NWV * 64) void score_kernel(const float* __restrict__ img,
-                                                    const float* __restrict__ text, int K, int P,
-                                                    float T, int kind, float* __restrict__ scores,
-                                                    int topk, int* __restrict__ idx,
-                                                    float* __restrict__ prob) {
-  extern __shared__ __attribute__((aligned(16))) char smem[];
-  float* f = (float*)smem;
-  float* sim = f + P;
+__device__ __forceinline__ void score_row_tail(float* __restrict__ sim, int b, int K, float T, int kind,
+                                               float* __restrict__ scores, int topk, int* __restrict__ idx,
+                                               float* __restrict__ prob) {
   __shared__ double red[NWV];
   __shared__ float redf[NWV];
-  const int b = blockIdx.x, tid = threadIdx.x, lane = tid & 63, wave = tid >> 6;
-  for (int d = tid; d < P; d += NWV * 64) f[d] = img[(size_t)b * P + d];
-  __syncthreads();
-  for (int k = wave; k < K; k += NWV) {
-    const float* t = text + (size_t)k * P;
-    float a = 0.f;
-    for (int d = lane * 4; d < P; d += 256) {
-      const float4 tv = *(const float4*)(t + d);
-      const float4 fv = *(const float4*)(f + d);
-      a = fmaf(tv.x, fv.x, a);
-      a = fmaf(tv.y, fv.y, a);
-      a = fmaf(tv.z, fv.z, a);
-      a = fmaf(tv.w, fv.w, a);
-    }
-    a = wave_sum(a);
-    if (lane == 0) sim[k] = a;
-  }
-  __syncthreads();
+  const int tid = threadIdx.x, lane = tid & 63, wave = tid >> 6;
   float m = -INFINITY;
   for (int k = tid; k < K; k += NWV * 64) m = fmaxf(m, sim[k]);
   m = wave_max(m);
@@ -156,6 +134,113 @@
   }
 }
 
+template <bool TOPK>
+__global__ __launch_bounds__(NWV * 64) void score_kernel(const float* __restrict__ img,
+                                                    const float* __restrict__ text, int K, int P,
+                                                    float T, int kind, float* __restrict__ scores,
+                                                    int topk, int* __restrict__ idx,
+                                                    float* __restrict__ prob) {
+  extern __shared__ __attribute__((aligned(16))) char smem[];
+  float* f = (float*)smem;
+  float* sim = f + P;
+  const int b = blockIdx.x, tid = threadIdx.x, lane = tid & 63, wave = tid >> 6;
+  for (int d = tid; d < P; d += NWV * 64) f[d] = img[(size_t)b * P + d];
+  __syncthreads();
+  for (int k = wave; k < K; k += NWV) {
+    const float* t = text + (size_t)k * P;
+    float a = 0.f;
+    for (int d = lane * 4; d < P; d += 256) {
+      const float4 tv = *(const float4*)(t + d);
+      const float4 fv = *(const float4*)(f + d);
+      a = fmaf(tv.x, fv.x, a);
+      a = fmaf(tv.y, fv.y, a);
+      a = fmaf(tv.z, fv.z, a);
+      a = fmaf(tv.w, fv.w, a);
+    }
+    a = wave_sum(a);
+    if (lane == 0) sim[k] = a;
+  }
+  __syncthreads();
+  score_row_tail<TOPK>(sim, b, K, T, kind, scores, topk, idx, prob);
+}
+
+template <bool TOPK, int G, int NJ, int KB, int PF>
+__global__ __launch_bounds__(NWV * 64) void score_multi_kernel(const float* __restrict__ img, int B,
+                                                               const float* __restrict__ text, int K, int P,
+                                                               float T, int kind, float* __restrict__ scores,
+                                                               int topk, int* __restrict__ idx,
+                                                               float* __restrict__ prob) {
+  constexpr int R = G * KB;
+  extern __shared__ __attribute__((aligned(16))) char smem[];
+  float* sim = (float*)smem;
+  const int b0 = blockIdx.x * G, tid = threadIdx.x, lane = tid & 63;
+  const int wave = __builtin_amdgcn_readfirstlane(tid >> 6);
+  const int nb = min(G, B - b0);
+  float4 fv[G][NJ];
+#pragma unroll
+  for (int g = 0; g < G; ++g)
+#pragma unroll
+    for (int j = 0; j < NJ; ++j) {
+      const int d = lane * 4 + 256 * j;
+      fv[g][j] = make_float4(0.f, 0.f, 0.f, 0.f);
+      if (g < nb && d < P) {
+        const float* f = img + (size_t)(b0 + g) * P + d;
+        fv[g][j] = make_float4(f[0], f[1], f[2], f[3]);
+      }
+    }
+  const int nkw = wave < K ? (K - wave + NWV - 1) / NWV : 0;
+  float4 tv[PF][KB][NJ];
+  auto fetch = [&](float4 (&dst)[KB][NJ], int i0) {
+#pragma unroll
+    for (int kb = 0; kb < KB; ++kb) {
+      const float* t = text + (size_t)(wave + NWV * min(i0 + kb, nkw - 1)) * P;
+#pragma unroll
+      for (int j = 0; j < NJ; ++j) {
+        const int d = lane * 4 + 256 * j;
+        dst[kb][j] = *(const float4*)(t + (d < P ? (unsigned)d : 0u));
+      }
+    }
+  };
+#pragma unroll
+  for (int s = 0; s < PF; ++s)
+    if (s * KB < nkw) fetch(tv[s], s * KB);
+  const int mine = wave_sum_scatter_index<R>(lane), mg = mine / KB, mkb = mine % KB;
+  const bool leader = (lane & (64 / R - 1)) == 0;
+  for (int ib = 0; ib < nkw; ib += PF * KB) {
+#pragma unroll
+    for (int s = 0; s < PF; ++s) {
+      const int i0 = ib + s * KB;
+      if (i0 < nkw) {
+        float a[R];
+#pragma unroll
+        for (int r = 0; r < R; ++r) a[r] = 0.f;
+#pragma unroll
+        for (int j = 0; j < NJ; ++j)
+          if (lane * 4 + 256 * j < P) {
+#pragma unroll
+            for (int g = 0; g < G; ++g)
+#pragma unroll
+              for (int kb = 0; kb < KB; ++kb) {
+                float& c = a[g * KB + kb];
+                c = fmaf(tv[s][kb][j].x, fv[g][j].x, c);
+                c = fmaf(tv[s][kb][j].y, fv[g][j].y, c);
+                c = fmaf(tv[s][kb][j].z, fv[g][j].z, c);
+                c = fmaf(tv[s][kb][j].w, fv[g][j].w, c);
+              }
+          }
+        __builtin_amdgcn_sched_barrier(0);
+        if (i0 + PF * KB < nkw) fetch(tv[s], i0 + PF * KB);
+        wave_sum_scatter<R>(a, lane);
+        if (leader && i0 + mkb < nkw) sim[(size_t)mg * K + wave + NWV * (i0 + mkb)] = a[0];
+      }
+    }
+  }
+  for (int g = 0; g < nb; ++g) {
+    __syncthreads();
+    score_row_tail<TOPK>(sim + (size_t)g * K, b0 + g, K, T, kind, scores, topk, idx, prob);
+  }
+}
+
 __global__ __launch_bounds__(256) void maha_prepare_kernel(const float* __restrict__ means,
                                                            const float* __restrict__ prec, int P,
                                                            double* __restrict__ w, double* __restrict__ k) {
@@ -323,22 +408,60 @@
   return hipGetLastError();
 }
 
+#ifdef MCM_HARNESS
+int g_score_mode = 0;
+void score_set_mode(int m) { g_score_mode = m; }
+static int score_mode() { return g_score_mode; }
+#else
+static constexpr int score_mode() { return 0; }
+#endif
+
+template <bool TOPK, int G, int NJ, int KB, int PF>
+static hipError_t launch_score_multi(const float* img, int B, const float* text, int K, int P, float T, int kind,
+                                     float* scores, int topk, int* idx, float* prob, hipStream_t s) {
+  static PerDeviceFlag attr_set;
+  if (!attr_set.get()) {
+    hipError_t e = hipFuncSetAttribute((const void*)score_multi_kernel<TOPK, G, NJ, KB, PF>,
+                                       hipFuncAttributeMaxDynamicSharedMemorySize, 150 * 1024);
+    if (e != hipSuccess) return e;
+    attr_set.set();
+  }
+  hipLaunchKernelGGL((score_multi_kernel<TOPK, G, NJ, KB, PF>), dim3((B + G - 1) / G), dim3(NWV * 64), G * K * (int)sizeof(float), s,
+                     img, B, text, K, P, T, kind, scores, topk, idx, prob);
+  return hipGetLastError();
+}
+
+template <bool TOPK>
+static hipError_t launch_score_any(const float* img, int B, const float* text, int K, int P, float T, int kind,
+                                   float* scores, int topk, int* idx, float* prob, hipStream_t s) {
+  const int mode = score_mode();
+  if (mode != 1 && P > 0 && P <= 1024) {
+    const bool two = mode == 3 || (mode == 0 && (B + 1) / 2 >= device_cu_count());
+    if (two && (int64_t)2 * K * 4 <= 150 * 1024) {
+      if (P <= 512) return launch_score_multi<TOPK, 2, 2, 4, 2>(img, B, text, K, P, T, kind, scores, topk, idx, prob, s);
+      return launch_score_multi<TOPK, 2, 4, 2, 1>(img, B, text, K, P, T, kind, scores, topk, idx, prob, s);
+    }
+    if (P <= 512) return launch_score_multi<TOPK, 1, 2, 4, 2>(img, B, text, K, P, T, kind, scores, topk, idx, prob, s);
+    return launch_score_multi<TOPK, 1, 4, 2, 2>(img, B, text, K, P, T, kind, scores, topk, idx, prob, s);
+  }
+  const int lds = (P + K) * (int)sizeof(float);
+  static PerDeviceFlag attr_set;
+  if (!attr_set.get()) {
+    hipError_t e = hipFuncSetAttribute((const void*)score_kernel<TOPK>, hipFuncAttributeMaxDynamicSharedMemorySize, 150 * 1024);
+    if (e != hipSuccess) return e;
+    attr_set.set();
+  }
+  hipLaunchKernelGGL(score_kernel<TOPK>, dim3(B), dim3(NWV * 64), lds, s, img, text, K, P, T, kind, scores, topk, idx, prob);
+  return hipGetLastError();
+}
+
 hipError_t launch_score(const float* img, int B, const float* text, int K, int P, float T, int kind,
                         float* scores, hipStream_t s) {
   if (B <= 0 || K <= 0 || P % 4 || kind < 0 || kind > MCM_SCORE_VAR || !(T > 0.f))
     return hipErrorInvalidValue;
   const int lds = (P + K) * (int)sizeof(float);
   if (lds > 150 * 1024) return hipErrorInvalidValue;
-  static PerDeviceFlag attr_set;
-  if (!attr_set.get()) {
-    hipError_t e = hipFuncSetAttribute((const void*)score_kernel<false>,
-                                       hipFuncAttributeMaxDynamicSharedMemorySize, 150 * 1024);
-    if (e != hipSuccess) return e;
-    attr_set.set();
-  }
-  hipLaunchKernelGGL(score_kernel<false>, dim3(B), dim3(NWV * 64), lds, s, img, text, K, P, T, kind, scores,
-                     0, (int*)nullptr, (float*)nullptr);
-  return hipGetLastError();
+  return launch_score_any<false>(img, B, text, K, P, T, kind, scores, 0, (int*)nullptr, (float*)nullptr, s);
 }
 
 bool score_shape_ok(int K, int P) { return K > 0 && P > 0 && P % 4 == 0 && (int64_t)(P + (int64_t)K) * 4 <= 150 * 1024; }
@@ -348,15 +471,5 @@
   if (B <= 0 || !score_shape_ok(K, P) || kind < 0 || kind > MCM_SCORE_VAR || !(T > 0.f) || topk < 1 ||
       topk > MCM_TOPK_MAX || !scores || !idx)
     return hipErrorInvalidValue;
-  const int lds = (P + K) * (int)sizeof(float);
-  static PerDeviceFlag attr_set;
-  if (!attr_set.get()) {
-    hipError_t e = hipFuncSetAttribute((const void*)score_kernel<true>,
-                                       hipFuncAttributeMaxDynamicSharedMemorySize, 150 * 1024);
-    if (e != hipSuccess) return e;
-    attr_set.set();
-  }
-  hipLaunchKernelGGL(score_kernel<true>, dim3(B), dim3(NWV * 64), lds, s, img, text, K, P, T, kind, scores,
-                     topk, idx, prob);
-  return hipGetLastError();
-}
+  return launch_score_any<true>(img, B, text, K, P, T, kind, scores, topk, idx, prob, s);
+}
diff --git a/mcm_amd/engine.py b/mcm_amd/engine.py
--- a/mcm_amd/engine.py
+++ b/mcm_amd/engine.py
@@ -71,6 +71,9 @@
     L.mcm_score_x2.argtypes = [vp, vp, i32, i32, vp, i32, f32, i32, vp, vp]
     if harness:
         L.mcm_debug_gemm_variant.argtypes = [i32]
+        L.mcm_debug_gemm_last_kernel.argtypes = []
+        L.mcm_debug_tail_kernels.argtypes = [i32, i32]
+        L.mcm_debug_op_linear_strided.argtypes = [vp, i32, vp, vp, vp, vp, vp, i32, i32, i32, i32, i32, i32, i32, vp]
         L.mcm_debug_op_act.argtypes = [vp, i32, vp, vp, ctypes.c_int64, vp]
         L.mcm_debug_attention_variant.argtypes = [i32]
         L.mcm_debug_attn_spin_budget.argtypes = [ctypes.c_int64]
@@ -159,7 +162,8 @@
     "mcm_neglabel_workspace_bytes", "mcm_neglabel_score_features",
     "mcm_local_workspace_bytes", "mcm_local_score_features", "mcm_encode_image_local", "mcm_score_glmcm",
 ]
-HARNESS_ONLY_SYMBOLS = ["mcm_debug_gemm_variant", "mcm_debug_attention_variant", "mcm_debug_qkv_chunks",
+HARNESS_ONLY_SYMBOLS = ["mcm_debug_gemm_variant", "mcm_debug_gemm_last_kernel", "mcm_debug_tail_kernels",
+                        "mcm_debug_op_linear_strided", "mcm_debug_attention_variant", "mcm_debug_qkv_chunks",
                         "mcm_debug_gemm_dbg", "mcm_debug_ln_fold", "mcm_debug_qkv_head_major",
                         "mcm_debug_ln_tail", "mcm_debug_ln_tail_timeouts", "mcm_debug_nsplit",
                         "mcm_debug_gemm_group_n", "mcm_debug_patch_fold", "mcm_debug_resize_fused_only",
```

Result: no change. 26220 images/sec (median of 6 runs) (+0.7%).
